# ipilter/RayTracerTest

Measured on AMD Instinct MI355X. Metric: Mray/s at 1920x1080x16spp, higher is better.
Workload: dtype f32

## Files before the change

### include/rt_mi355x.h

```cpp
#ifndef RT_MI355X_H
#define RT_MI355X_H

#include <stddef.h>
#include <stdint.h>

#ifdef __cplusplus
extern "C" {
#endif

#define RT_OK              0
#define RT_ERR_INVALID     1
#define RT_ERR_NO_DEVICE   2
#define RT_ERR_HIP         3
#define RT_ERR_STATE       4

#define RT_MATH_FMA        0u
#define RT_MATH_STRICT     1u

#define RT_FLAG_NO_FILTER  1u
#define RT_FLAG_NO_BINNING 2u

#define RT_FLAG_NEAREST_HIT 4u

#define RT_FLAG_NO_MACRO_BINS 16u
#define RT_FLAG_NO_SUPER_BINS 64u
#define RT_FLAG_NO_SURE_HIT 32u
#define RT_FLAG_SMOOTH_NORMALS 8u

#define RT_BUF_RENDER      0
#define RT_BUF_COUNTS      1
#define RT_BUF_IMAGE       2
#define RT_BUF_RNG         3
#define RT_BUF_FRAME       4
#define RT_GROUP_ID_BYTES  128

typedef struct rt_tracer rt_tracer;
typedef struct rt_float4 { float x, y, z, w; } rt_float4;

typedef void (*rt_callback_fn)(uint32_t* imageBuffer, size_t size, void* user);

typedef struct rt_options {
  uint32_t struct_size;
  int32_t  device;
  uint32_t full_height;
  uint32_t row_begin;
  uint32_t use_time_seed;
  uint32_t math_mode;
  uint64_t seed;
  uint32_t flags;
  uint32_t samples_in_flight;
  uint32_t lds_chunk;
  uint32_t bin_list;
  uint32_t transport;
} rt_options;

#define RT_TRANSPORT_RCCL  0u
#define RT_TRANSPORT_PEER  1u


int  rt_tracer_create(const uint32_t imageSize[2], const float cameraPosition[3],
                      const float cameraAngles[2], float fov, float focalLength, float aperture,
                      rt_tracer** out);
int  rt_tracer_create_ex(const uint32_t imageSize[2], const float cameraPosition[3],
                         const float cameraAngles[2], float fov, float focalLength, float aperture,
                         const rt_options* options, rt_tracer** out);
void rt_tracer_destroy(rt_tracer* t);
int  rt_tracer_trace(rt_tracer* t, uint32_t iterationCount, uint32_t samplesPerIteration,
                     uint32_t updateInterval);
void rt_tracer_stop(rt_tracer* t);
int  rt_tracer_resize(rt_tracer* t, const uint32_t size[2]);
void rt_tracer_set_camera_parameters(rt_tracer* t, float fov, float focalLength, float aperture);
void rt_tracer_rotate_camera(rt_tracer* t, const float angles[2]);
int  rt_tracer_upload_scene(rt_tracer* t, const rt_float4* hostData, size_t count);
int  rt_tracer_upload_scene_edges(rt_tracer* t, const rt_float4* hostData, size_t count);
float rt_pack_normal(const float n[3]);
void  rt_unpack_normal(float packed, float n[3]);
void rt_tracer_set_update_callback(rt_tracer* t, rt_callback_fn fn, void* user);
void rt_tracer_set_finished_callback(rt_tracer* t, rt_callback_fn fn, void* user);


int  rt_tracer_wait(rt_tracer* t);
int  rt_tracer_set_seed(rt_tracer* t, uint64_t seed);
int  rt_tracer_upload_spheres(rt_tracer* t, const rt_float4* spheres, size_t count);
int  rt_tracer_trace_enqueue(rt_tracer* t, uint32_t iterationCount, uint32_t samplesPerIteration);
int  rt_tracer_trace_enqueue_n(rt_tracer* t, uint32_t iterationCount, uint32_t samplesPerIteration, uint32_t n_steps);
int  rt_tracer_sync(rt_tracer* t);
int  rt_tracer_launch(rt_tracer* t, uint32_t samples, int clear_first, int emit_image);
int  rt_tracer_launch_iterations(rt_tracer* t, uint32_t samples, uint32_t iterations, int clear_first, int emit_image);
int  rt_tracer_fused_iterations(rt_tracer* t, uint32_t samples);
int  rt_tracer_set_list_reuse(rt_tracer* t, int across_traces);
int  rt_tracer_set_image_mirror(rt_tracer* t, void* device_visible_image);
int  rt_tracer_kernel_time(rt_tracer* t, double* total_ms, uint64_t* launches, int reset_after);
int  rt_tracer_launch_time(rt_tracer* t, double* total_ms, uint64_t* launches, int reset_after);
int  rt_tracer_trace_stats(rt_tracer* t, uint32_t samples, uint64_t out[16]);
int  rt_tracer_read_buffer(rt_tracer* t, int which, void* dst, size_t bytes);
int  rt_tracer_copy_buffer_to_device(rt_tracer* t, int which, void* dst_device, size_t bytes);
int  rt_tracer_copy_buffer_to_device_async(rt_tracer* t, int which, void* dst_device, size_t bytes);
void* rt_tracer_stream(rt_tracer* t);
void* rt_tracer_stream_b(rt_tracer* t);
void* rt_tracer_device_pointer(rt_tracer* t, int which);
size_t rt_tracer_buffer_bytes(rt_tracer* t, int which);
int  rt_tracer_info(rt_tracer* t, uint32_t out[8]);
const char* rt_tracer_last_error(rt_tracer* t);
const char* rt_last_error(void);
int  rt_device_count(void);
const char* rt_version(void);


int  rt_tracer_create_multi(const uint32_t imageSize[2], const float cameraPosition[3],
                            const float cameraAngles[2], float fov, float focalLength, float aperture,
                            const rt_options* options, const int32_t* devices, uint32_t n_bands,
                            rt_tracer** out);
int  rt_group_unique_id(uint8_t id[RT_GROUP_ID_BYTES]);
int  rt_tracer_join_group(rt_tracer* t, uint32_t n_ranks, uint32_t rank, const uint8_t id[RT_GROUP_ID_BYTES]);
int  rt_tracer_leave_group(rt_tracer* t);
int  rt_tracer_join_group_bands(rt_tracer* t, uint32_t n_ranks, uint32_t rank, const uint8_t id[RT_GROUP_ID_BYTES],
                                const uint32_t* row_begin);
int  rt_balance_rows(uint32_t n_bands, const uint32_t* row_begin, const double* cost, uint32_t granule,
                     uint32_t* new_row_begin);
int  rt_tracer_rebalance(rt_tracer* t);
int  rt_tracer_set_band(rt_tracer* t, uint32_t row_begin, uint32_t rows);
int  rt_tracer_gather_time(rt_tracer* t, double* total_ms, uint64_t* gathers, int reset_after);
int  rt_tracer_gather_only(rt_tracer* t);
int  rt_tracer_group_info(rt_tracer* t, char* json, size_t capacity);
int  rt_tracer_band_count(rt_tracer* t);
int  rt_tracer_band_info(rt_tracer* t, uint32_t band, uint32_t out[4]);

int rt_dbg_hit_triangle(int device, uint32_t math_mode, uint32_t n, const float* rays,
                        const float* tris, int eps_mode, int32_t* hit, float* tuv, float* normal,
                        float* point);
int rt_dbg_sincos(int device, uint32_t n, const float* x, float* s, float* c);
int rt_dbg_trace_occupancy(int device, int samples_in_flight, uint32_t lds_bytes);
int rt_dbg_valu_peak(int device, double* lane_fma_per_s, double* clock_ghz);
int rt_dbg_check_midrange(int device, uint64_t out[4]);
int rt_dbg_wave_list_counts(rt_tracer* t, int half, uint32_t* dst, size_t capacity_tiles, uint32_t* n_tiles, uint32_t* capacity_per_tile);
int rt_dbg_read_tile_lists(rt_tracer* t, uint32_t* dst, size_t capacity_words, uint32_t* words_per_tile);
int rt_dbg_focal_boxes(rt_tracer* t, float curv_scale, float* boxes, size_t boxes_capacity, float* focal, size_t focal_capacity);
int rt_dbg_classify(rt_tracer* t, uint32_t level, uint32_t forms, uint32_t slack_milli, const uint32_t* regions, uint32_t n_regions,
                    float* out, size_t capacity_floats);
int rt_dbg_uniform(int device, uint32_t n, uint32_t m, uint32_t* states, float* out);
int rt_dbg_get_ray(rt_tracer* t, uint32_t n, const uint32_t* pixels, uint32_t* states, float* rays);
void rt_dbg_rng_init_host(uint64_t seed, uint64_t subsequence, uint32_t state[6]);

#ifdef __cplusplus
}
#endif
#endif
```

### raytracertest_amd/api.py

```python
import ctypes as C
import os
import threading
import weakref

import numpy as np

_HERE = os.path.dirname(os.path.abspath(__file__))
_LIB_PATH = os.environ.get("RT_MI355X_LIB") or os.path.join(_HERE, "lib", "librt_mi355x.so")

MATH_FMA, MATH_STRICT = 0, 1
FLAG_NO_FILTER = 1
FLAG_NO_BINNING = 2
FLAG_NEAREST_HIT = 4
FLAG_SMOOTH_NORMALS = 8
FLAG_NO_MACRO_BINS = 16
FLAG_NO_SUPER_BINS = 64
FLAG_NO_SURE_HIT = 32
BUF_RENDER, BUF_COUNTS, BUF_IMAGE, BUF_RNG, BUF_FRAME = 0, 1, 2, 3, 4
GROUP_ID_BYTES = 128
TRANSPORT_RCCL, TRANSPORT_PEER = 0, 1

ABI_SYMBOLS = [
    "rt_tracer_create", "rt_tracer_create_ex", "rt_tracer_destroy", "rt_tracer_trace",
    "rt_tracer_stop", "rt_tracer_resize", "rt_tracer_set_camera_parameters",
    "rt_tracer_rotate_camera", "rt_tracer_upload_scene", "rt_tracer_set_update_callback",
    "rt_tracer_set_finished_callback", "rt_tracer_wait", "rt_tracer_set_seed",
    "rt_tracer_upload_spheres", "rt_tracer_trace_enqueue", "rt_tracer_trace_enqueue_n", "rt_tracer_sync", "rt_tracer_trace_stats", "rt_tracer_launch", "rt_tracer_launch_iterations", "rt_tracer_fused_iterations", "rt_tracer_set_image_mirror", "rt_tracer_set_list_reuse", "rt_tracer_stream_b", "rt_tracer_upload_scene_edges", "rt_pack_normal",
    "rt_unpack_normal",
    "rt_tracer_kernel_time", "rt_tracer_launch_time", "rt_tracer_read_buffer", "rt_tracer_copy_buffer_to_device", "rt_tracer_copy_buffer_to_device_async",
    "rt_tracer_stream",
    "rt_tracer_device_pointer", "rt_tracer_buffer_bytes", "rt_tracer_info",
    "rt_tracer_last_error", "rt_last_error", "rt_device_count", "rt_version",
    "rt_dbg_hit_triangle", "rt_dbg_sincos", "rt_dbg_valu_peak", "rt_dbg_check_midrange", "rt_dbg_trace_occupancy", "rt_dbg_uniform", "rt_dbg_get_ray",
    "rt_dbg_rng_init_host",
    "rt_tracer_create_multi", "rt_group_unique_id", "rt_tracer_join_group", "rt_tracer_leave_group",
    "rt_tracer_gather_time", "rt_tracer_band_count", "rt_tracer_band_info",
    "rt_tracer_join_group_bands", "rt_balance_rows", "rt_tracer_rebalance", "rt_tracer_set_band", "rt_dbg_read_tile_lists", "rt_dbg_wave_list_counts", "rt_dbg_focal_boxes", "rt_dbg_classify",
    "rt_tracer_gather_only", "rt_tracer_group_info",
]


class RtError(RuntimeError):
    pass


class Options(C.Structure):
    _fields_ = [("struct_size", C.c_uint32), ("device", C.c_int32), ("full_height", C.c_uint32),
                ("row_begin", C.c_uint32), ("use_time_seed", C.c_uint32), ("math_mode", C.c_uint32),
                ("seed", C.c_uint64), ("flags", C.c_uint32), ("samples_in_flight", C.c_uint32),
                ("lds_chunk", C.c_uint32), ("bin_list", C.c_uint32), ("transport", C.c_uint32)]


CALLBACK = C.CFUNCTYPE(None, C.POINTER(C.c_uint32), C.c_size_t, C.c_void_p)

_lib = None
_lib_lock = threading.Lock()


def library_path():
    return _LIB_PATH


def _share_hip_runtime_with_torch():
    if os.environ.get("RT_MI355X_HIP_RUNTIME", "") == "system":
        return None
    try:
        import importlib.util
        spec = importlib.util.find_spec("torch")
        if spec is None or not spec.submodule_search_locations:
            return None
        cand = os.path.join(list(spec.submodule_search_locations)[0], "lib", "libamdhip64.so")
        if os.path.exists(cand):
            C.CDLL(cand, mode=C.RTLD_GLOBAL)
            return cand
    except (ImportError, OSError, ValueError):
        pass
    return None


HIP_RUNTIME = None


def load_library():
    global _lib, HIP_RUNTIME
    with _lib_lock:
        if _lib is not None:
            return _lib
        if not os.path.exists(_LIB_PATH):
            raise RtError("HIP extension not built: %s is missing (run `python -m raytracertest_amd.build` "
                          "or __graft_entry__.build()); there is no CPU fallback" % _LIB_PATH)
        HIP_RUNTIME = _share_hip_runtime_with_torch()
        L = C.CDLL(_LIB_PATH)
        vp, u32p, f32p = C.c_void_p, C.POINTER(C.c_uint32), C.POINTER(C.c_float)
        L.rt_tracer_create.argtypes = [u32p, f32p, f32p, C.c_float, C.c_float, C.c_float, C.POINTER(vp)]
        L.rt_tracer_create_ex.argtypes = [u32p, f32p, f32p, C.c_float, C.c_float, C.c_float,
                                          C.POINTER(Options), C.POINTER(vp)]
        L.rt_tracer_destroy.argtypes = [vp]
        L.rt_tracer_destroy.restype = None
        L.rt_tracer_trace.argtypes = [vp, C.c_uint32, C.c_uint32, C.c_uint32]
        L.rt_tracer_stop.argtypes = [vp]
        L.rt_tracer_stop.restype = None
        L.rt_tracer_resize.argtypes = [vp, u32p]
        L.rt_tracer_set_camera_parameters.argtypes = [vp, C.c_float, C.c_float, C.c_float]
        L.rt_tracer_set_camera_parameters.restype = None
        L.rt_tracer_rotate_camera.argtypes = [vp, f32p]
        L.rt_tracer_rotate_camera.restype = None
        L.rt_tracer_upload_scene.argtypes = [vp, vp, C.c_size_t]
        L.rt_tracer_upload_scene_edges.argtypes = [vp, vp, C.c_size_t]
        L.rt_pack_normal.argtypes = [f32p]
        L.rt_pack_normal.restype = C.c_float
        L.rt_unpack_normal.argtypes = [C.c_float, f32p]
        L.rt_unpack_normal.restype = None
        L.rt_tracer_set_update_callback.argtypes = [vp, CALLBACK, vp]
        L.rt_tracer_set_update_callback.restype = None
        L.rt_tracer_set_finished_callback.argtypes = [vp, CALLBACK, vp]
        L.rt_tracer_set_finished_callback.restype = None
        L.rt_tracer_wait.argtypes = [vp]
        L.rt_tracer_set_seed.argtypes = [vp, C.c_uint64]
        L.rt_tracer_upload_spheres.argtypes = [vp, vp, C.c_size_t]
        L.rt_tracer_trace_enqueue.argtypes = [vp, C.c_uint32, C.c_uint32]
        L.rt_tracer_trace_enqueue_n.argtypes = [vp, C.c_uint32, C.c_uint32, C.c_uint32]
        L.rt_tracer_sync.argtypes = [vp]
        L.rt_tracer_launch.argtypes = [vp, C.c_uint32, C.c_int, C.c_int]
        L.rt_tracer_launch_iterations.argtypes = [vp, C.c_uint32, C.c_uint32, C.c_int, C.c_int]
        L.rt_tracer_fused_iterations.argtypes = [vp, C.c_uint32]
        L.rt_tracer_set_image_mirror.argtypes = [vp, vp]
        L.rt_tracer_set_list_reuse.argtypes = [vp, C.c_int]
        L.rt_tracer_trace_stats.argtypes = [vp, C.c_uint32, C.POINTER(C.c_uint64)]
        L.rt_tracer_kernel_time.argtypes = [vp, C.POINTER(C.c_double), C.POINTER(C.c_uint64), C.c_int]
        L.rt_tracer_launch_time.argtypes = [vp, C.POINTER(C.c_double), C.POINTER(C.c_uint64), C.c_int]
        L.rt_tracer_read_buffer.argtypes = [vp, C.c_int, vp, C.c_size_t]
        L.rt_tracer_copy_buffer_to_device.argtypes = [vp, C.c_int, vp, C.c_size_t]
        L.rt_tracer_copy_buffer_to_device_async.argtypes = [vp, C.c_int, vp, C.c_size_t]
        L.rt_tracer_stream.argtypes = [vp]
        L.rt_tracer_stream.restype = vp
        L.rt_tracer_stream_b.argtypes = [vp]
        L.rt_tracer_stream_b.restype = vp
        L.rt_tracer_device_pointer.argtypes = [vp, C.c_int]
        L.rt_tracer_device_pointer.restype = vp
        L.rt_tracer_buffer_bytes.argtypes = [vp, C.c_int]
        L.rt_tracer_buffer_bytes.restype = C.c_size_t
        L.rt_tracer_info.argtypes = [vp, u32p]
        L.rt_tracer_last_error.argtypes = [vp]
        L.rt_tracer_last_error.restype = C.c_char_p
        L.rt_last_error.restype = C.c_char_p
        L.rt_device_count.restype = C.c_int
        L.rt_version.restype = C.c_char_p
        L.rt_dbg_hit_triangle.argtypes = [C.c_int, C.c_uint32, C.c_uint32, f32p, f32p, C.c_int,
                                          C.POINTER(C.c_int32), f32p, f32p, f32p]
        L.rt_dbg_sincos.argtypes = [C.c_int, C.c_uint32, f32p, f32p, f32p]
        L.rt_dbg_uniform.argtypes = [C.c_int, C.c_uint32, C.c_uint32, u32p, f32p]
        L.rt_dbg_valu_peak.argtypes = [C.c_int, C.POINTER(C.c_double), C.POINTER(C.c_double)]
        L.rt_dbg_trace_occupancy.argtypes = [C.c_int, C.c_int, C.c_uint32]
        L.rt_dbg_get_ray.argtypes = [vp, C.c_uint32, u32p, u32p, f32p]
        L.rt_dbg_rng_init_host.argtypes = [C.c_uint64, C.c_uint64, u32p]
        L.rt_dbg_rng_init_host.restype = None
        L.rt_tracer_create_multi.argtypes = [u32p, f32p, f32p, C.c_float, C.c_float, C.c_float, C.POINTER(Options),
                                             C.POINTER(C.c_int32), C.c_uint32, C.POINTER(vp)]
        L.rt_group_unique_id.argtypes = [C.c_char_p]
        L.rt_tracer_join_group.argtypes = [vp, C.c_uint32, C.c_uint32, C.c_char_p]
        L.rt_tracer_leave_group.argtypes = [vp]
        L.rt_tracer_gather_time.argtypes = [vp, C.POINTER(C.c_double), C.POINTER(C.c_uint64), C.c_int]
        L.rt_tracer_band_count.argtypes = [vp]
        L.rt_tracer_band_info.argtypes = [vp, C.c_uint32, u32p]
        L.rt_tracer_join_group_bands.argtypes = [vp, C.c_uint32, C.c_uint32, C.c_char_p, u32p]
        L.rt_balance_rows.argtypes = [C.c_uint32, u32p, C.POINTER(C.c_double), C.c_uint32, u32p]
        L.rt_tracer_rebalance.argtypes = [vp]
        L.rt_tracer_set_band.argtypes = [vp, C.c_uint32, C.c_uint32]
        L.rt_dbg_read_tile_lists.argtypes = [vp, u32p, C.c_size_t, u32p]
        L.rt_dbg_wave_list_counts.argtypes = [vp, C.c_int, u32p, C.c_size_t, u32p, u32p]
        L.rt_dbg_focal_boxes.argtypes = [vp, C.c_float, f32p, C.c_size_t, f32p, C.c_size_t]
        L.rt_tracer_gather_only.argtypes = [vp]
        L.rt_tracer_group_info.argtypes = [vp, C.c_char_p, C.c_size_t]
        L.rt_dbg_classify.argtypes = [vp, C.c_uint32, C.c_uint32, C.c_uint32, u32p, C.c_uint32, f32p, C.c_size_t]
        _lib = L
        return _lib


def device_count():
    return int(load_library().rt_device_count())


def balance_rows(row_begin, cost, granule=8):
    b = np.ascontiguousarray(row_begin, np.uint32)
    c = np.ascontiguousarray(cost, np.float64)
    out = np.zeros_like(b)
    rc = load_library().rt_balance_rows(c.size, _u32p(b), c.ctypes.data_as(C.POINTER(C.c_double)), granule, _u32p(out))
    if rc != 0:
        raise RtError("rt_balance_rows: invalid partition")
    return [int(x) for x in out]


def group_unique_id():
    buf = C.create_string_buffer(GROUP_ID_BYTES)
    rc = load_library().rt_group_unique_id(buf)
    if rc != 0:
        raise RtError("rt_group_unique_id failed (%d): %s" % (rc, load_library().rt_last_error().decode()))
    return buf.raw


def _f32p(a):
    return a.ctypes.data_as(C.POINTER(C.c_float))


def _u32p(a):
    return a.ctypes.data_as(C.POINTER(C.c_uint32))


class RayTracer:

    def __init__(self, imageSize, cameraPosition=(0.0, 0.0, 0.0), cameraAngles=(0.0, 0.0), fov=70.0,
                 focalLength=10.0, aperture=4.0, *, seed=None, device=0, math_mode=MATH_FMA,
                 full_height=0, row_begin=0, no_filter=False, no_binning=False, nearest_hit=False, smooth_normals=False, no_macro_bins=False, no_super_bins=False, samples_in_flight=0,
                 lds_chunk=0, bin_list=0, devices=None, no_sure_hit=False, transport="rccl"):
        self._lib = load_library()
        self._h = C.c_void_p()
        self._cbs = {}
        self._retired = []
        size = np.array(imageSize, np.uint32)
        opt = Options()
        opt.struct_size = C.sizeof(Options)
        opt.device = device
        opt.full_height, opt.row_begin = full_height, row_begin
        opt.use_time_seed = 1 if seed is None else 0
        opt.seed = 0 if seed is None else int(seed)
        opt.math_mode = math_mode
        opt.flags = ((FLAG_NO_FILTER if no_filter else 0) | (FLAG_NO_BINNING if no_binning else 0) |
                     (FLAG_NEAREST_HIT if nearest_hit else 0) | (FLAG_SMOOTH_NORMALS if smooth_normals else 0) | (FLAG_NO_MACRO_BINS if no_macro_bins else 0) | (FLAG_NO_SUPER_BINS if no_super_bins else 0) |
                     (FLAG_NO_SURE_HIT if no_sure_hit else 0))
        opt.samples_in_flight, opt.lds_chunk, opt.bin_list = samples_in_flight, lds_chunk, bin_list
        opt.transport = {"rccl": TRANSPORT_RCCL, "peer": TRANSPORT_PEER}[transport]
        if devices is not None:
            devs = np.ascontiguousarray(devices, np.int32)
            rc = self._lib.rt_tracer_create_multi(_u32p(size), _f32p(np.array(cameraPosition, np.float32)),
                                                  _f32p(np.array(cameraAngles, np.float32)), fov, focalLength, aperture,
                                                  C.byref(opt), devs.ctypes.data_as(C.POINTER(C.c_int32)), devs.size,
                                                  C.byref(self._h))
        else:
            rc = self._lib.rt_tracer_create_ex(_u32p(size), _f32p(np.array(cameraPosition, np.float32)),
                                               _f32p(np.array(cameraAngles, np.float32)), fov, focalLength,
                                               aperture, C.byref(opt), C.byref(self._h))
        if rc != 0 or not self._h:
            raise RtError("rt_tracer_create failed (%d): %s" % (rc, self._lib.rt_last_error().decode()))
        self.full_height = int(full_height) if full_height else int(size[1])
        self._band = bool(full_height) and devices is None
        self.width = int(size[0])
        self.rows = int(size[1])

    def Trace(self, iterationCount, samplesPerIteration, updateInterval):
        self._check(self._lib.rt_tracer_trace(self._h, iterationCount, samplesPerIteration, updateInterval))

    def Stop(self):
        self._lib.rt_tracer_stop(self._h)

    def Resize(self, size):
        s = np.array(size, np.uint32)
        self._check(self._lib.rt_tracer_resize(self._h, _u32p(s)))
        self.width, self.rows = int(s[0]), int(s[1])
        if not self._band:
            self.full_height = self.rows

    def SetCameraParameters(self, fov, focalLength, aperture):
        self._lib.rt_tracer_set_camera_parameters(self._h, fov, focalLength, aperture)

    def RotateCamera(self, angles):
        self._lib.rt_tracer_rotate_camera(self._h, _f32p(np.array(angles, np.float32)))

    def UploadScene(self, hostData):
        a = np.ascontiguousarray(hostData, np.float32).reshape(-1, 4)
        rc = self._lib.rt_tracer_upload_scene(self._h, a.ctypes.data, a.shape[0])
        if rc == 1:
            return False
        self._check(rc)
        return True

    def UploadSceneEdges(self, hostData):
        a = np.ascontiguousarray(hostData, np.float32).reshape(-1, 4)
        rc = self._lib.rt_tracer_upload_scene_edges(self._h, a.ctypes.data, a.shape[0])
        if rc == 1:
            return False
        self._check(rc)
        return True

    def SetUpdateCallback(self, callback):
        self._set_cb("update", callback, self._lib.rt_tracer_set_update_callback)

    def SetFinishedCallback(self, callback):
        self._set_cb("finished", callback, self._lib.rt_tracer_set_finished_callback)

    def Wait(self):
        ok = bool(self._lib.rt_tracer_wait(self._h))
        self._retired.clear()
        return ok

    def SetSeed(self, seed):
        self._check(self._lib.rt_tracer_set_seed(self._h, int(seed)))

    def UploadSpheres(self, spheres):
        a = np.ascontiguousarray(spheres, np.float32).reshape(-1, 4)
        self._check(self._lib.rt_tracer_upload_spheres(self._h, a.ctypes.data, a.shape[0]))

    def TraceEnqueue(self, iterationCount, samplesPerIteration):
        self._check(self._lib.rt_tracer_trace_enqueue(self._h, iterationCount, samplesPerIteration))

    def TraceEnqueueN(self, iterationCount, samplesPerIteration, n_steps):
        self._check(self._lib.rt_tracer_trace_enqueue_n(self._h, iterationCount, samplesPerIteration, n_steps))

    def Launch(self, samples, clear_first=False, emit_image=False, iterations=1):
        if iterations == 1:
            self._check(self._lib.rt_tracer_launch(self._h, samples, int(clear_first), int(emit_image)))
        else:
            self._check(self._lib.rt_tracer_launch_iterations(self._h, samples, iterations, int(clear_first), int(emit_image)))

    def SetListReuse(self, across_traces=True):
        self._check(self._lib.rt_tracer_set_list_reuse(self._h, 1 if across_traces else 0))

    def SetImageMirror(self, device_visible_ptr):
        self._check(self._lib.rt_tracer_set_image_mirror(self._h, C.c_void_p(device_visible_ptr or 0)))

    def FusedIterations(self, samples):
        return max(1, int(self._lib.rt_tracer_fused_iterations(self._h, samples)))

    def Sync(self):
        self._check(self._lib.rt_tracer_sync(self._h))

    def TraceStats(self, samples):
        out = (C.c_uint64 * 16)()
        self._check(self._lib.rt_tracer_trace_stats(self._h, samples, out))
        v = [int(x) for x in out]
        return {"exit_det": v[0], "exit_u": v[1], "exit_v": v[2], "exit_hit": v[3],
                "skip_a": v[4], "skip_b": v[5], "skip_c": v[6], "reach_d": v[7],
                "bin_candidates": v[8], "bin_rounds": v[9], "pretest_skips": v[10],
                "tiles_by_list": {"0": v[11], "1": v[12], "sure": v[13], "2": v[14], "more": v[15]}}

    def KernelTime(self, reset=True):
        ms, n = C.c_double(), C.c_uint64()
        self._lib.rt_tracer_kernel_time(self._h, C.byref(ms), C.byref(n), 1 if reset else 0)
        return ms.value, n.value

    def LaunchTime(self, reset=True):
        ms, n = C.c_double(), C.c_uint64()
        self._lib.rt_tracer_launch_time(self._h, C.byref(ms), C.byref(n), 1 if reset else 0)
        return ms.value, n.value

    def _read(self, which, dtype, shape):
        out = np.empty(shape, dtype)
        self._check(self._lib.rt_tracer_read_buffer(self._h, which, out.ctypes.data, out.nbytes))
        return out

    def RenderBuffer(self):
        return self._read(BUF_RENDER, np.float32, (self.rows, self.width, 4))

    def SampleCounts(self):
        return self._read(BUF_COUNTS, np.uint32, (self.rows, self.width))

    def Image(self):
        return self._read(BUF_IMAGE, np.uint32, (self.rows, self.width))

    def RngStates(self):
        planes = self._read(BUF_RNG, np.uint32, (6, self.rows, self.width))
        return np.ascontiguousarray(np.moveaxis(planes, 0, -1))

    def JoinGroup(self, n_ranks, rank, unique_id=None, row_begin=None):
        if row_begin is None:
            self._check(self._lib.rt_tracer_join_group(self._h, n_ranks, rank, unique_id))
        else:
            b = np.ascontiguousarray(row_begin, np.uint32)
            self._check(self._lib.rt_tracer_join_group_bands(self._h, n_ranks, rank, unique_id, _u32p(b)))

    def SetBand(self, row_begin, rows):
        self._check(self._lib.rt_tracer_set_band(self._h, row_begin, rows))
        self.rows = int(rows)

    def Rebalance(self):
        self._check(self._lib.rt_tracer_rebalance(self._h))

    def LeaveGroup(self):
        self._check(self._lib.rt_tracer_leave_group(self._h))

    def Frame(self):
        return self._read(BUF_FRAME, np.uint32, (self.full_height, self.width))

    def GatherTime(self, reset=True):
        ms, n = C.c_double(), C.c_uint64()
        self._lib.rt_tracer_gather_time(self._h, C.byref(ms), C.byref(n), 1 if reset else 0)
        return ms.value, n.value

    def GatherOnly(self):
        self._check(self._lib.rt_tracer_gather_only(self._h))

    def GroupInfo(self):
        import json
        buf = C.create_string_buffer(8192)
        self._check(self._lib.rt_tracer_group_info(self._h, buf, len(buf)))
        return json.loads(buf.value.decode())

    def Bands(self):
        out = []
        for k in range(int(self._lib.rt_tracer_band_count(self._h))):
            v = np.zeros(4, np.uint32)
            self._check(self._lib.rt_tracer_band_info(self._h, k, _u32p(v)))
            out.append({"device": int(v[0]), "row0": int(v[1]), "rows": int(v[2]), "rank": int(v[3])})
        return out

    def DevicePointer(self, which):
        return self._lib.rt_tracer_device_pointer(self._h, which)

    def CopyToDevice(self, which, dst_ptr, nbytes):
        self._check(self._lib.rt_tracer_copy_buffer_to_device(self._h, which, dst_ptr, nbytes))

    def CopyToDeviceAsync(self, which, dst_ptr, nbytes):
        self._check(self._lib.rt_tracer_copy_buffer_to_device_async(self._h, which, dst_ptr, nbytes))

    def Stream(self):
        return int(self._lib.rt_tracer_stream(self._h) or 0)

    def StreamB(self):
        return int(self._lib.rt_tracer_stream_b(self._h) or 0)

    def Info(self):
        out = np.zeros(8, np.uint32)
        self._lib.rt_tracer_info(self._h, _u32p(out))
        keys = ("samples_in_flight", "lds_chunk", "lds_bytes", "grid_x", "grid_y", "n_tris", "n_spheres", "device")
        return dict(zip(keys, (int(v) for v in out)))

    def LastError(self):
        return self._lib.rt_tracer_last_error(self._h).decode()

    def DebugTileLists(self):
        bx, by = (self.width + 31) // 32, (self.rows + 7) // 8
        wpt = np.zeros(1, np.uint32)
        buf = np.zeros(bx * (by + 1) * 4 * 1025, np.uint32)
        self._check(self._lib.rt_dbg_read_tile_lists(self._h, _u32p(buf), buf.size, _u32p(wpt)))
        w = int(wpt[0])
        words = buf[:bx * by * 4 * w].reshape(by, bx * 4, w)[:, :, 0]
        return (words & 0x3FF).astype(np.int32), ((words >> 10) & 0x3FF).astype(np.int32), (words >> 31).astype(bool)

    def DebugWaveListCounts(self, half=0):
        n, cap = np.zeros(1, np.uint32), np.zeros(1, np.uint32)
        buf = np.zeros(((self.width + 31) // 32) * ((self.rows + 7) // 8 + 1) * 4, np.uint32)
        self._check(self._lib.rt_dbg_wave_list_counts(self._h, half, _u32p(buf), buf.size, _u32p(n), _u32p(cap)))
        return buf[:int(n[0])].copy(), int(cap[0])

    def DebugTileListWords(self):
        bx, by = (self.width + 31) // 32, (self.rows + 7) // 8
        wpt = np.zeros(1, np.uint32)
        buf = np.zeros(bx * (by + 1) * 4 * 1025, np.uint32)
        self._check(self._lib.rt_dbg_read_tile_lists(self._h, _u32p(buf), buf.size, _u32p(wpt)))
        w = int(wpt[0])
        return buf[:bx * by * 4 * w].reshape(by, bx * 4, w).copy()

    def DebugFocalBoxes(self, curv_scale=1.0):
        bx, by = (self.width + 31) // 32, (self.rows + 7) // 8
        boxes = np.zeros((by, bx * 4, 8), np.float32)
        focal = np.zeros((self.rows, self.width, 3), np.float32)
        self._check(self._lib.rt_dbg_focal_boxes(self._h, float(curv_scale), _f32p(boxes), boxes.size, _f32p(focal), focal.size))
        return boxes, focal

    def DebugClassify(self, regions, level=0, forms=False, slack_milli=1000):
        reg = np.ascontiguousarray(regions, np.uint32).reshape(-1, 2)
        n_tris = self.Info()["n_tris"]
        per = 16 + n_tris * (32 if forms else 12)
        out = np.zeros((reg.shape[0], per), np.float32)
        self._check(self._lib.rt_dbg_classify(self._h, level, 1 if forms else 0, slack_milli, _u32p(reg), reg.shape[0], _f32p(out), out.size))
        return out[:, :16], out[:, 16:].reshape(reg.shape[0], n_tris, 32 if forms else 12)

    def DebugGetRay(self, pixels, states):
        pix = np.ascontiguousarray(pixels, np.uint32).reshape(-1, 2)
        st = np.ascontiguousarray(states, np.uint32).reshape(-1, 6).copy()
        rays = np.zeros((pix.shape[0], 6), np.float32)
        self._check(self._lib.rt_dbg_get_ray(self._h, pix.shape[0], _u32p(pix), _u32p(st), _f32p(rays)))
        return rays, st

    def close(self):
        if self._h:
            self._lib.rt_tracer_destroy(self._h)
            self._h = C.c_void_p()
            self._retired.clear()

    def __del__(self):
        try:
            self.close()
        except Exception:
            pass

    def __enter__(self):
        return self

    def __exit__(self, *a):
        self.close()

    def _check(self, rc):
        if rc != 0:
            raise RtError("librt_mi355x error %d: %s" % (rc, self.LastError()))

    def _set_cb(self, key, callback, setter):
        old = self._cbs.get(key)
        if old is not None:
            self._retired.append(old)
        if callback is None:
            self._cbs[key] = CALLBACK()
            setter(self._h, self._cbs[key], None)
            return

        me = weakref.ref(self)

        def tramp(ptr, size, _user):
            n = size // 4
            img = np.ctypeslib.as_array(ptr, shape=(n,))
            owner = me()
            rows, width = (owner.rows, owner.width) if owner is not None else (0, 0)
            callback(img.reshape(rows, width) if n == rows * width and n else img, size)
        self._cbs[key] = CALLBACK(tramp)
        setter(self._h, self._cbs[key], None)


def dbg_hit_triangle(rays, tris, math_mode=MATH_FMA, eps_mode=0, device=0):
    L = load_library()
    r = np.ascontiguousarray(rays, np.float32).reshape(-1, 6)
    t = np.ascontiguousarray(tris, np.float32).reshape(-1, 9)
    n = r.shape[0]
    hit = np.zeros(n, np.int32)
    tuv, nrm, pt = (np.zeros((n, 3), np.float32) for _ in range(3))
    rc = L.rt_dbg_hit_triangle(device, math_mode, n, _f32p(r), _f32p(t), eps_mode,
                               hit.ctypes.data_as(C.POINTER(C.c_int32)), _f32p(tuv), _f32p(nrm), _f32p(pt))
    if rc != 0:
        raise RtError("rt_dbg_hit_triangle failed (%d): %s" % (rc, L.rt_last_error().decode()))
    return hit.astype(bool), tuv, nrm, pt


def dbg_sincos(x, device=0):
    L = load_library()
    a = np.ascontiguousarray(x, np.float32).ravel()
    s, c = np.zeros_like(a), np.zeros_like(a)
    rc = L.rt_dbg_sincos(device, a.size, _f32p(a), _f32p(s), _f32p(c))
    if rc != 0:
        raise RtError("rt_dbg_sincos failed (%d): %s" % (rc, L.rt_last_error().decode()))
    return s, c


def dbg_valu_peak(device=0):
    L = load_library()
    r, g = C.c_double(), C.c_double()
    rc = L.rt_dbg_valu_peak(device, C.byref(r), C.byref(g))
    if rc != 0:
        raise RtError("rt_dbg_valu_peak failed (%d): %s" % (rc, L.rt_last_error().decode()))
    return r.value, g.value


def dbg_check_midrange(device=0):
    L = load_library()
    out = (C.c_uint64 * 4)()
    L.rt_dbg_check_midrange.argtypes = [C.c_int, C.POINTER(C.c_uint64)]
    rc = L.rt_dbg_check_midrange(device, out)
    if rc != 0:
        raise RtError("rt_dbg_check_midrange failed (%d): %s" % (rc, L.rt_last_error().decode()))
    return tuple(int(x) for x in out)


def dbg_uniform(states, m, device=0):
    L = load_library()
    st = np.ascontiguousarray(states, np.uint32).reshape(-1, 6).copy()
    out = np.zeros((st.shape[0], m), np.float32)
    rc = L.rt_dbg_uniform(device, st.shape[0], m, _u32p(st), _f32p(out))
    if rc != 0:
        raise RtError("rt_dbg_uniform failed (%d): %s" % (rc, L.rt_last_error().decode()))
    return out, st


def dbg_rng_init_host(seed, subsequence):
    s = np.zeros(6, np.uint32)
    load_library().rt_dbg_rng_init_host(int(seed), int(subsequence), _u32p(s))
    return s
```

### raytracertest_amd/csrc/rt_kernels.hpp

```cpp
#pragma once
#include <hip/hip_runtime.h>
#include <stdint.h>

namespace rtk {

constexpr uint32_t kSuperChunk = 1024u, kSuperMaxChunks = 64u;

struct TraceParams {
  float4*   render;
  uint32_t* counts;
  uint32_t* rng;
  uint32_t  W, H;
  uint32_t  row0, rows;
  uint32_t  npix;
  uint32_t  samples;
  float     cam[12];
  float     half_height, aspect, focal, aperture;
  float     tile_curv, tile_round;
  const float4* tri_a;
  const float*  tri_b;
  const float4* tri_color;
  uint32_t  n_tris;
  const float4* spheres;
  uint32_t  n_spheres;
  uint32_t  chunk;
  uint32_t  bin_list;
  uint32_t  block_list;
  unsigned long long* stats;
  uint32_t* image;
  const float4* tri_n;
#ifdef RT_TIMELINE
  unsigned long long* timeline;
#endif
  uint32_t* image_host;
  uint32_t  pretest_on;
  uint32_t  iters;
  uint32_t* macro_lists;
  uint32_t  macro_cap, macro_w, macro_h, macro_nx;
  uint32_t* super_lists;
  uint32_t  super_chunks, super_f, super_nx;
  float*    macro_bounds;
  uint32_t* tile_lists;
  uint32_t  row_il, row_phase;
  uint32_t* half_cost;
  uint32_t  cost_split_brow;
  const float4* sure_table;
  uint32_t* wave_lists;
  uint32_t  wave_cap;
  uint32_t  flags;
};

constexpr uint32_t TRACE_ZERO_ACC = 1u;
constexpr uint32_t TRACE_EMIT_IMAGE = 2u;
constexpr uint32_t TRACE_NEAREST_HIT = 4u;
constexpr uint32_t TRACE_PRETEST = 32u;
constexpr uint32_t TRACE_NO_SURE_HIT = 64u;

hipError_t launch_rng_init(uint32_t* rng, uint32_t npix, uint32_t p0, const uint32_t seeded[6],
                           const uint32_t* jump, const uint32_t* win, hipStream_t st);
hipError_t launch_prep_triangles(bool fma, bool edges, const float4* verts, uint32_t n, float4* tri_a, float* tri_b,
                                 float4* color, float4* normals, hipStream_t st);
uint32_t trace_lds_bytes(const TraceParams& p, bool bin);
hipError_t launch_trace(const TraceParams& p, bool fma, bool filter, bool bin, int K, hipStream_t st);
int trace_occupancy(int K, size_t lds);
hipError_t launch_convert(const float4* render, const uint32_t* counts, uint32_t* image, uint32_t npix,
                          hipStream_t st);

hipError_t launch_dbg_hit_triangle(bool fma, uint32_t n, const float* rays, const float* tris, int eps_mode,
                                   int* hit, float* tuv, float* normal, float* point, hipStream_t st);
bool trace_can_fuse(bool filter, bool bin);
hipError_t launch_macro_bin(const TraceParams& p, bool fma, hipStream_t st);
hipError_t launch_super_bin(const TraceParams& p, bool fma, hipStream_t st);
hipError_t launch_wave_lists(const TraceParams& p, bool fma, hipStream_t st);
hipError_t launch_delay(uint32_t us, hipStream_t st);
hipError_t launch_publish_half_cost(uint32_t* half_cost, unsigned long long* host_word, hipStream_t st);
hipError_t launch_sure_table(const float4* colors, uint32_t n_tris, uint32_t samples, float4* out, hipStream_t st);
hipError_t launch_tile_lists(const TraceParams& p, bool fma, hipStream_t st);
hipError_t launch_dbg_check_midrange(unsigned long long* out, hipStream_t st);
hipError_t launch_dbg_focal_boxes(bool fma, const TraceParams& p, float* boxes, float* focal, hipStream_t st);
hipError_t launch_dbg_classify(bool fma, bool forms, uint32_t slack_milli, const TraceParams& p, uint32_t level, uint32_t n_regions,
                               const uint32_t* regions, float* out, hipStream_t st);
hipError_t launch_dbg_valu_peak(uint32_t blocks, int iters, float* out, unsigned long long* clk, hipStream_t st);
hipError_t launch_dbg_sincos(uint32_t n, const float* x, float* s, float* c, hipStream_t st);
hipError_t launch_dbg_uniform(uint32_t n, uint32_t m, uint32_t* states, float* out, hipStream_t st);
hipError_t launch_dbg_get_ray(bool fma, const TraceParams& p, uint32_t n, const uint32_t* pixels,
                              uint32_t* states, float* rays, hipStream_t st);

}
```

### raytracertest_amd/csrc/rt_lists.hpp

```cpp
#pragma once
#include "rt_classify.hpp"

namespace rtk {

template <bool FMA, int WAVES>
__device__ __forceinline__ FocalBounds rect_focal_bounds(const TraceParams& p, uint32_t x0, uint32_t y0, uint32_t rw, uint32_t rh, float (*s_box)[8]) {
  const uint32_t lane = threadIdx.x & 63u, wave = threadIdx.x >> 6;
  const uint32_t x1 = (x0 + rw < p.W) ? x0 + rw : p.W;
  const uint32_t y1 = (y0 + rh < p.rows) ? y0 + rh : p.rows;
  const uint32_t w = x1 - x0, count_px = w * (y1 - y0);
  float lo[3] = {FLT_MAX, FLT_MAX, FLT_MAX}, hi[3] = {-FLT_MAX, -FLT_MAX, -FLT_MAX};
  bool finite = true;
  for (uint32_t i = threadIdx.x; i < count_px; i += 64u * WAVES) {
    const uint32_t px = x0 + i % w, ly = y0 + i / w;
    V3 po, pd;
    pinhole<FMA>(p, px, p.row0 + ly, po, pd);
    const V3 f = focal_point<FMA>(p, pd);
    const float fl[3] = {f.x, f.y, f.z};
#pragma unroll
    for (int c = 0; c < 3; ++c) {
      finite = finite && (__builtin_fabsf(fl[c]) <= FLT_MAX);
      lo[c] = fminf(lo[c], fl[c]);
      hi[c] = fmaxf(hi[c], fl[c]);
    }
  }
#pragma unroll
  for (int c = 0; c < 3; ++c) { lo[c] = uniform(wave_min(lo[c])); hi[c] = uniform(wave_max(hi[c])); }
  const bool wave_ok = __builtin_amdgcn_ballot_w64(!finite) == 0ull;
  if (lane == 0u) {
#pragma unroll
    for (int c = 0; c < 3; ++c) { s_box[wave][c] = lo[c]; s_box[wave][3 + c] = hi[c]; }
    s_box[wave][6] = wave_ok ? 1.0f : 0.0f;
  }
  __syncthreads();
  FocalBounds bb;
  bb.ok = true; bb.any = count_px != 0u;
#pragma unroll
  for (int c = 0; c < 3; ++c) { bb.lo[c] = FLT_MAX; bb.hi[c] = -FLT_MAX; }
  for (uint32_t v = 0; v < static_cast<uint32_t>(WAVES); ++v) {
#pragma unroll
    for (int c = 0; c < 3; ++c) {
      bb.lo[c] = fminf(bb.lo[c], s_box[v][c]);
      bb.hi[c] = fmaxf(bb.hi[c], s_box[v][3 + c]);
    }
    bb.ok = bb.ok && (s_box[v][6] != 0.0f);
  }
  return bb;
}

template <class Src>
__device__ __forceinline__ void bin_pass(const TraceParams& p, const TileFamily& fam, Src tri_of, uint32_t n, uint32_t* out, uint32_t cap,
                                         uint32_t (*s_cnt)[4]) {
  const uint32_t lane = threadIdx.x & 63u, wave = threadIdx.x >> 6;
  uint32_t total = 0, step = 0;
  bool overflow = false;
  for (uint32_t base = 0; base < n; base += 256u, ++step) {
    const uint32_t e = base + threadIdx.x;
    const bool valid = e < n;
    const uint32_t tri = tri_of(valid ? e : (n - 1u));
    const float4 A0 = p.tri_a[2u * tri], A1 = p.tri_a[2u * tri + 1u];
    const float bz = p.tri_b[tri];
    bool keep = valid;
    if (fam.usable)
      keep = valid && !tile_misses_triangle(fam, {A1.z, A1.w, bz}, {A0.w, A1.x, A1.y}, {A0.x, A0.y, A0.z});
    const unsigned long long m = __builtin_amdgcn_ballot_w64(keep);
    uint32_t* const slot = s_cnt[step & 1u];
    if (lane == 0u) slot[wave] = static_cast<uint32_t>(__builtin_popcountll(m));
    __syncthreads();
    const uint32_t c0 = slot[0], c1 = slot[1], c2 = slot[2], c3 = slot[3];
    const uint32_t before = (wave > 0u ? c0 : 0u) + (wave > 1u ? c1 : 0u) + (wave > 2u ? c2 : 0u);
    const uint32_t step_total = c0 + c1 + c2 + c3;
    if (total + step_total > cap) { overflow = true; break; }
    const uint32_t pos = total + before + __builtin_amdgcn_mbcnt_hi(static_cast<uint32_t>(m >> 32),
                                                                __builtin_amdgcn_mbcnt_lo(static_cast<uint32_t>(m), 0u));
    if (keep) out[1u + pos] = tri;
    total += step_total;
  }
  if (threadIdx.x == 0u) out[0] = overflow ? 0xFFFFFFFFu : total;
}


__device__ __forceinline__ FocalBounds load_bounds(const float* b) {
  FocalBounds r;
#pragma unroll
  for (int c = 0; c < 3; ++c) { r.lo[c] = uniform(b[c]); r.hi[c] = uniform(b[3 + c]); }
  r.ok = uniform(b[6]) != 0.0f; r.any = uniform(b[7]) != 0.0f;
  return r;
}

template <bool FMA>
__global__ __launch_bounds__(256) void macro_bounds_kernel(TraceParams p) {
  __shared__ float s_box[4][8];
  const FocalBounds bb = rect_focal_bounds<FMA, 4>(p, blockIdx.x * p.macro_w, blockIdx.y * p.macro_h, p.macro_w, p.macro_h, s_box);
  if (threadIdx.x == 0u) {
    float* const o = p.macro_bounds + (static_cast<size_t>(blockIdx.y) * gridDim.x + blockIdx.x) * 8u;
#pragma unroll
    for (int c = 0; c < 3; ++c) { o[c] = bb.lo[c]; o[3 + c] = bb.hi[c]; }
    o[6] = bb.ok ? 1.0f : 0.0f; o[7] = bb.any ? 1.0f : 0.0f;
  }
}

template <bool FMA>
__global__ __launch_bounds__(256) void super_bin_kernel(TraceParams p) {
  __shared__ uint32_t s_cnt[2][4];
  const uint32_t sx = blockIdx.x % p.super_nx, sy = blockIdx.x / p.super_nx;
  const uint32_t macro_ny = (p.rows + p.macro_h - 1u) / p.macro_h;
  FocalBounds bb;
  bb.ok = true; bb.any = false;
#pragma unroll
  for (int c = 0; c < 3; ++c) { bb.lo[c] = FLT_MAX; bb.hi[c] = -FLT_MAX; }
  for (uint32_t j = 0; j < p.super_f; ++j) {
    for (uint32_t i = 0; i < p.super_f; ++i) {
      const uint32_t mx = sx * p.super_f + i, my = sy * p.super_f + j;
      if (mx >= p.macro_nx || my >= macro_ny) continue;
      const FocalBounds mb = load_bounds(p.macro_bounds + (static_cast<size_t>(my) * p.macro_nx + mx) * 8u);
#pragma unroll
      for (int c = 0; c < 3; ++c) { bb.lo[c] = fminf(bb.lo[c], mb.lo[c]); bb.hi[c] = fmaxf(bb.hi[c], mb.hi[c]); }
      bb.ok = bb.ok && mb.ok; bb.any = bb.any || mb.any;
    }
  }
  const TileFamily fam = make_family(p, bb);
  const uint32_t first = blockIdx.y * kSuperChunk;
  const uint32_t n = p.n_tris - first < kSuperChunk ? p.n_tris - first : kSuperChunk;
  uint32_t* const out = p.super_lists + (static_cast<size_t>(blockIdx.x) * gridDim.y + blockIdx.y) * (kSuperChunk + 1u);
  bin_pass(p, fam, [&](uint32_t e) { return first + e; }, n, out, kSuperChunk, s_cnt);
}

template <bool FMA>
__global__ __launch_bounds__(256) void macro_bin_kernel(TraceParams p) {
  __shared__ float s_box[4][8];
  __shared__ uint32_t s_cnt[2][4];
  __shared__ uint32_t s_first[kSuperMaxChunks + 1u];
  FocalBounds bb;
  if (p.macro_bounds != nullptr) bb = load_bounds(p.macro_bounds + (static_cast<size_t>(blockIdx.y) * gridDim.x + blockIdx.x) * 8u);
  else bb = rect_focal_bounds<FMA, 4>(p, blockIdx.x * p.macro_w, blockIdx.y * p.macro_h, p.macro_w, p.macro_h, s_box);
  const TileFamily fam = make_family(p, bb);
  uint32_t* const out = p.macro_lists + (static_cast<size_t>(blockIdx.y) * gridDim.x + blockIdx.x) * (p.macro_cap + 1u);
  if (p.super_lists == nullptr) {
    bin_pass(p, fam, [](uint32_t e) { return e; }, p.n_tris, out, p.macro_cap, s_cnt);
    return;
  }
  const uint32_t S = p.super_chunks;
  const uint32_t* const sl = p.super_lists + static_cast<size_t>((blockIdx.y / p.super_f) * p.super_nx + blockIdx.x / p.super_f) * S * (kSuperChunk + 1u);
  if (threadIdx.x == 0u) {
    uint32_t acc = 0;
    for (uint32_t c = 0; c < S; ++c) { s_first[c] = acc; acc += sl[static_cast<size_t>(c) * (kSuperChunk + 1u)]; }
    s_first[S] = acc;
  }
  __syncthreads();
  const uint32_t n = s_first[S];
  bin_pass(p, fam, [&](uint32_t e) {
    uint32_t c = 0;
    for (uint32_t k = 1; k < S; ++k) c += (e >= s_first[k]) ? 1u : 0u;
    return sl[static_cast<size_t>(c) * (kSuperChunk + 1u) + 1u + (e - s_first[c])];
  }, n, out, p.macro_cap, s_cnt);
}

template <int CTRL>
__device__ __forceinline__ float dpp_f(float v) {
  return __builtin_bit_cast(float, __builtin_amdgcn_update_dpp(0, __builtin_bit_cast(int, v), CTRL, 0xF, 0xF, true));
}
#define RT_ROW_REDUCE(OP, v)                 \
  v = OP(v, dpp_f<0xB1>(v));                 \
  v = OP(v, dpp_f<0x4E>(v));                 \
  v = OP(v, dpp_f<0x124>(v));                \
  v = OP(v, dpp_f<0x128>(v));
template <int G>
__device__ __forceinline__ float group_max(float v) {
  RT_ROW_REDUCE(fmaxf, v)
#pragma unroll
  for (int off = G / 2; off >= 16; off >>= 1) v = fmaxf(v, __shfl_xor(v, off, 64));
  return v;
}
template <int G>
__device__ __forceinline__ float group_min(float v) {
  RT_ROW_REDUCE(fminf, v)
#pragma unroll
  for (int off = G / 2; off >= 16; off >>= 1) v = fminf(v, __shfl_xor(v, off, 64));
  return v;
}
#undef RT_ROW_REDUCE

template <bool FMA, int G, class SL>
__device__ __forceinline__ FocalBounds group_focal_bounds(const TraceParams& p, uint32_t x0, uint32_t y0, bool in_image, uint32_t gl, uint32_t gbase) {
  constexpr uint32_t T = 64u / G;
  const bool full = in_image && x0 + 8u <= p.W && y0 + 8u <= p.rows;
  FocalBounds b;
  const bool corners = p.tile_curv > 0.0f && full;
  const unsigned long long need_range = __builtin_amdgcn_ballot_w64(in_image && !corners);
  {
    const uint32_t cx = x0 + ((gl & 1u) ? 7u : 0u), cy = y0 + ((gl & 2u) ? 7u : 0u);
    V3 po, pd;
    pinhole<FMA>(p, cx < p.W ? cx : 0u, p.row0 + (cy < p.rows ? cy : 0u), po, pd);
    const V3 f = focal_point<FMA>(p, pd);
    const float fl[3] = {f.x, f.y, f.z};
    const float dev = p.tile_curv + RT_SLK(4e-6f) * p.tile_round;
    bool finite = true;
#pragma unroll
    for (int i = 0; i < 3; ++i) {
      const float c0 = __shfl(fl[i], static_cast<int>(gbase), 64), c1 = __shfl(fl[i], static_cast<int>(gbase + 1u), 64);
      const float c2 = __shfl(fl[i], static_cast<int>(gbase + 2u), 64), c3 = __shfl(fl[i], static_cast<int>(gbase + 3u), 64);
      b.lo[i] = fminf(fminf(c0, c1), fminf(c2, c3)) - dev;
      b.hi[i] = fmaxf(fmaxf(c0, c1), fmaxf(c2, c3)) + dev;
      finite = finite && (__builtin_fabsf(b.lo[i]) <= FLT_MAX) && (__builtin_fabsf(b.hi[i]) <= FLT_MAX);
    }
    b.ok = finite; b.any = true;
  }
  if (need_range != 0ull) {
    float lo[3] = {FLT_MAX, FLT_MAX, FLT_MAX}, hi[3] = {-FLT_MAX, -FLT_MAX, -FLT_MAX};
    bool finite = true, any = false;
#pragma unroll
    for (uint32_t i = 0; i < T; ++i) {
      const uint32_t pi = gl + i * G;
      const uint32_t px = x0 + (pi & 7u), py = y0 + (pi >> 3);
      const bool inside = in_image && px < p.W && py < p.rows;
      V3 po, pd;
      pinhole<FMA>(p, inside ? px : 0u, p.row0 + (inside ? py : 0u), po, pd);
      const V3 f = focal_point<FMA>(p, pd);
      const float fl[3] = {f.x, f.y, f.z};
#pragma unroll
      for (int c = 0; c < 3; ++c) {
        if (inside) { lo[c] = fminf(lo[c], fl[c]); hi[c] = fmaxf(hi[c], fl[c]); finite = finite && (__builtin_fabsf(fl[c]) <= FLT_MAX); }
      }
      any = any || inside;
    }
    const unsigned long long gmask = G == 64 ? ~0ull : (0xFFFFFFFFull << gbase);
    const bool g_ok = (__builtin_amdgcn_ballot_w64(!finite) & gmask) == 0ull;
    const bool g_any = (__builtin_amdgcn_ballot_w64(any) & gmask) != 0ull;
#pragma unroll
    for (int c = 0; c < 3; ++c) { lo[c] = group_min<G>(lo[c]); hi[c] = group_max<G>(hi[c]); }
    if (!corners) {
#pragma unroll
      for (int c = 0; c < 3; ++c) { b.lo[c] = lo[c]; b.hi[c] = hi[c]; }
      b.ok = g_ok; b.any = g_any;
    }
  }
  return b;
}

template <bool FMA, int G, class SL = SlackProduct>
__global__ __launch_bounds__(256, 5) void tile_lists_kernel(const TraceParams p) {
  static_assert(G == 32 || G == 64, "lanes per tile");
  constexpr uint32_t T = 64u / G;
  const uint32_t lane = threadIdx.x & 63u, wave = threadIdx.x >> 6;
  const uint32_t gl = lane & (G - 1u), gbase = lane & ~(G - 1u);
  const uint32_t gx = (p.W + 31u) / 32u, gy = (p.rows + 7u) / 8u;
  const uint32_t slots = gx * gy * 4u;
  const uint32_t slot = (blockIdx.x * 4u + wave) * T + lane / G;
  const bool live = slot < slots;
  const uint32_t sl = live ? slot : 0u;
  const uint32_t x0 = ((sl / 4u) % gx) * 32u + (sl % 4u) * 8u, y0 = ((sl / 4u) / gx) * 8u;
  const bool in_image = live && x0 < p.W;

  const FocalBounds b = group_focal_bounds<FMA, G, SL>(p, x0, y0, in_image, gl, gbase);
  const TileFamily fam = make_family<SL>(p, b);

  uint32_t* const saved = p.tile_lists + static_cast<size_t>(sl) * (1u + p.bin_list);
  const uint32_t n = p.n_tris;
  uint32_t count = 0;
  const float NEG = -__builtin_inff();
  bool haveA = false;
  float Q = NEG, M1 = NEG, M2 = NEG;
  uint32_t A = 0, I1 = 0xFFFFFFFFu;
  for (uint32_t base = 0; base < n; base += G) {
    const uint32_t tri = base + gl;
    const bool valid = in_image && tri < n;
    const uint32_t ti = tri < n ? tri : n - 1u;
    const float4 A0 = p.tri_a[2u * ti], A1 = p.tri_a[2u * ti + 1u];
    const float bz = p.tri_b[ti];
    bool keep = valid, sure = false;
    float q[2] = {0.0f, 0.0f};
    if (fam.usable) {
      const bool miss = tile_misses_triangle<false, true, SL>(fam, {A1.z, A1.w, bz}, {A0.w, A1.x, A1.y}, {A0.x, A0.y, A0.z}, nullptr, &sure, q);
      keep = valid && !miss;
    } else {
      sure = false;
    }
    const unsigned long long m = __builtin_amdgcn_ballot_w64(keep);
    const unsigned long long gm = G == 64 ? m : ((m >> gbase) & 0xFFFFFFFFull);
    const uint32_t pos = count + static_cast<uint32_t>(__builtin_popcountll(gm & ((1ull << gl) - 1ull)));
    if (keep) saved[1u + pos] = tri;
    count += static_cast<uint32_t>(__builtin_popcountll(gm));
    const bool cand = keep && sure && fam.usable;
    const float Qs = group_max<G>(cand ? q[0] : NEG);
    const unsigned long long bm = __builtin_amdgcn_ballot_w64(cand && q[0] == Qs);
    const unsigned long long gbm = G == 64 ? bm : ((bm >> gbase) & 0xFFFFFFFFull);
    if (gbm != 0ull && (!haveA || Qs > Q)) { haveA = true; Q = Qs; A = base + static_cast<uint32_t>(__builtin_ctzll(gbm)); }
    const float qh = keep ? ((q[1] == q[1]) ? q[1] : __builtin_inff()) : NEG;
    if (n <= G) {
      const uint32_t la = gbm != 0ull ? static_cast<uint32_t>(__builtin_ctzll(gbm)) : 0xFFFFFFFFu;
      M1 = group_max<G>((keep && gl != la) ? qh : NEG);
      I1 = 0xFFFFFFFEu;
      break;
    }
    const float m1s = group_max<G>(qh);
    const unsigned long long tm = __builtin_amdgcn_ballot_w64(keep && qh == m1s);
    const unsigned long long gtm = G == 64 ? tm : ((tm >> gbase) & 0xFFFFFFFFull);
    const uint32_t l1 = gtm != 0ull ? static_cast<uint32_t>(__builtin_ctzll(gtm)) : 0xFFFFFFFFu;
    const float m2s = group_max<G>((keep && gl != l1) ? qh : NEG);
    if (gtm != 0ull) {
      if (m1s > M1) { M2 = fmaxf(M1, m2s); M1 = m1s; I1 = base + l1; }
      else { M2 = fmaxf(M2, m1s); }
    }
  }
  bool sure_one = false;
  if (haveA) {
    const float R = (I1 == A) ? M2 : M1;
    sure_one = count <= 1u || (R < Q - 1e-4f * (__builtin_fabsf(R) + __builtin_fabsf(Q)));
  }
  if (live && gl == 0u) saved[0] = count | (A << 10) | (sure_one ? 0x80000000u : 0u);
}

template <class SL>
__device__ __forceinline__ float tile_dev(const TraceParams& p) { return p.tile_curv + RT_SLK(4e-6f) * p.tile_round; }

__device__ __forceinline__ void region_corner_pixel(const TraceParams& p, uint32_t rx, uint32_t ry, uint32_t tile, uint32_t corner,
                                                    uint32_t& px, uint32_t& py, bool& valid) {
  const uint32_t x0 = rx * 32u + (tile & 3u) * 8u, y0 = (ry * 2u + (tile >> 2)) * 8u;
  valid = x0 < p.W && y0 < p.rows;
  const uint32_t x1 = (x0 + 7u < p.W) ? x0 + 7u : p.W - 1u, y1 = (y0 + 7u < p.rows) ? y0 + 7u : p.rows - 1u;
  px = valid ? ((corner & 1u) ? x1 : x0) : 0u;
  py = valid ? ((corner & 2u) ? y1 : y0) : 0u;
}

template <bool FMA, class SL, bool PACK = false>
__device__ __forceinline__ void region_focal_bounds(const TraceParams& p, uint32_t rx, uint32_t ry, uint32_t lane,
                                                    FocalBounds& tile_b, FocalBounds& region_b) {
  const uint32_t l32 = lane & 31u;
  uint32_t px, py;
  bool valid;
  region_corner_pixel(p, rx, ry, l32 >> 2, l32 & 3u, px, py, valid);
  V3 po, pd;
  pinhole<FMA>(p, px, p.row0 + py, po, pd);
  const V3 f = focal_point<FMA>(p, pd);
  const float fl[3] = {f.x, f.y, f.z};
  const float dev = tile_dev<SL>(p);
  bool fin = true;
  float rlo[3], rhi[3];
#pragma unroll
  for (int i = 0; i < 3; ++i) {
    float lo = fl[i], hi = fl[i];
    lo = fminf(lo, dpp_f<0xB1>(lo)); lo = fminf(lo, dpp_f<0x4E>(lo));
    hi = fmaxf(hi, dpp_f<0xB1>(hi)); hi = fmaxf(hi, dpp_f<0x4E>(hi));
    tile_b.lo[i] = lo - dev;
    tile_b.hi[i] = hi + dev;
    fin = fin && (__builtin_fabsf(tile_b.lo[i]) <= FLT_MAX) && (__builtin_fabsf(tile_b.hi[i]) <= FLT_MAX) && (fl[i] == fl[i]);
    rlo[i] = valid ? tile_b.lo[i] : FLT_MAX;
    rhi[i] = valid ? tile_b.hi[i] : -FLT_MAX;
  }
  const unsigned long long badm = __builtin_amdgcn_ballot_w64(!fin);
  const uint32_t quad_bad = (static_cast<uint32_t>(badm >> (lane & (PACK ? 60u : 28u))) & 0xFu);
  tile_b.ok = quad_bad == 0u;
  tile_b.any = valid;
  const unsigned long long vm = __builtin_amdgcn_ballot_w64(valid);
  const uint32_t hs = PACK ? (lane & 32u) : 0u;
  region_b.any = ((vm >> hs) & 0xFFFFFFFFull) != 0ull;
  region_b.ok = (((badm & vm) >> hs) & 0xFFFFFFFFull) == 0ull;
#pragma unroll
  for (int i = 0; i < 3; ++i) {
    region_b.lo[i] = group_min<32>(rlo[i]);
    region_b.hi[i] = group_max<32>(rhi[i]);
  }
}


template <int G>
__device__ __forceinline__ float max_group(float v) {
  v = fmaxf(v, dpp_f<0xB1>(v));
  v = fmaxf(v, dpp_f<0x4E>(v));
  if constexpr (G == 8) v = fmaxf(v, dpp_f<0x141>(v));
  return v;
}

template <class SL, int G2>
__device__ __forceinline__ void region_level2(const TraceParams& p, uint32_t lane, const FocalBounds& mine, const uint32_t* cand, uint32_t cnt,
                                              uint32_t cnt_max, uint32_t tslot, bool slot_live, bool lower) {
  constexpr uint32_t GM = (1u << G2) - 1u;
  const uint32_t j = lane & (G2 - 1u), gsh = lane & ~static_cast<uint32_t>(G2 - 1);
  const bool tile_valid = mine.any;
  const TileFamily fam = make_family<SL>(p, mine);
  uint32_t* const saved = p.tile_lists + static_cast<size_t>(tile_valid ? tslot : 0u) * (1u + p.bin_list);
  const float NEG = -__builtin_inff();
  uint32_t count = 0;
  bool haveA = false;
  float Q = NEG, M1 = NEG, M2 = NEG;
  uint32_t A = 0, I1 = 0xFFFFFFFFu;
  const bool one_pass = cnt_max <= static_cast<uint32_t>(G2);
  bool others_ok = true;
  for (uint32_t c0 = 0; c0 < cnt_max; c0 += G2) {
    const bool has = tile_valid && c0 + j < cnt;
    const uint32_t tri = (c0 + j < cnt) ? cand[c0 + j] : 0u;
    const float4 A0 = p.tri_a[2u * tri], A1 = p.tri_a[2u * tri + 1u];
    const float bz = p.tri_b[tri];
    bool keep = has, sure = false;
    float q[2] = {0.0f, 0.0f};
    float pr[9] = {0.0f, 0.0f, 0.0f, 0.0f, 0.0f, 0.0f, 0.0f, 0.0f, 0.0f};
    if (fam.usable) {
      const bool miss = tile_misses_triangle<false, true, SL>(fam, {A1.z, A1.w, bz}, {A0.w, A1.x, A1.y}, {A0.x, A0.y, A0.z}, nullptr, &sure, q,
                                                              nullptr, pr);
      keep = has && !miss;
    }
    const uint32_t gm = static_cast<uint32_t>(__builtin_amdgcn_ballot_w64(keep) >> gsh) & GM;
    const uint32_t pos = count + static_cast<uint32_t>(__builtin_popcount(gm & ((1u << j) - 1u)));
    if (keep) saved[1u + pos] = tri;
    count += static_cast<uint32_t>(__builtin_popcount(gm));
    const bool cd = keep && sure && fam.usable;
    const float Qs = max_group<G2>(cd ? q[0] : NEG);
    const uint32_t gbm = static_cast<uint32_t>(__builtin_amdgcn_ballot_w64(cd && q[0] == Qs) >> gsh) & GM;
    if (gbm != 0u && (!haveA || Qs > Q)) { haveA = true; Q = Qs; A = cand[c0 + static_cast<uint32_t>(__builtin_ctz(gbm))]; }
    const float qh = keep ? ((q[1] == q[1]) ? q[1] : __builtin_inff()) : NEG;
    if (one_pass) {
      const uint32_t la = gbm != 0u ? static_cast<uint32_t>(__builtin_ctz(gbm)) : 0xFFFFFFFFu;
      bool lane_ok = !keep || j == la || (gbm != 0u && qh < Qs - 1e-4f * (__builtin_fabsf(qh) + __builtin_fabsf(Qs)));
      const bool need = gbm != 0u && !lane_ok;
      if (__builtin_amdgcn_ballot_w64(need) != 0ull) {
        float pa[9];
        const int src = static_cast<int>(gsh + (la & (G2 - 1u)));
#pragma unroll
        for (int i = 0; i < 9; ++i) pa[i] = __shfl(pr[i], src, 64);
        lane_ok = lane_ok || (need && pair_farther<SL>(fam, pa, pr));
      }
      others_ok = (static_cast<uint32_t>(__builtin_amdgcn_ballot_w64(!lane_ok) >> gsh) & GM) == 0u;
    }
    const float m1s = max_group<G2>(qh);
    const uint32_t gtm = static_cast<uint32_t>(__builtin_amdgcn_ballot_w64(keep && qh == m1s) >> gsh) & GM;
    const uint32_t l1 = gtm != 0u ? static_cast<uint32_t>(__builtin_ctz(gtm)) : 0xFFFFFFFFu;
    const float m2s = max_group<G2>((keep && j != l1) ? qh : NEG);
    if (gtm != 0u) {
      const uint32_t i1s = cand[c0 + l1];
      if (m1s > M1) { M2 = fmaxf(M1, m2s); M1 = m1s; I1 = i1s; }
      else { M2 = fmaxf(M2, m1s); }
    }
  }
  bool sure_one = false;
  if (haveA) {
    const float R = (I1 == A) ? M2 : M1;
    sure_one = count <= 1u || (R < Q - 1e-4f * (__builtin_fabsf(R) + __builtin_fabsf(Q)));
    if (one_pass) sure_one = sure_one || others_ok;
  }
  if (j == 0u) {
    if (tile_valid) saved[0] = count | (A << 10) | (sure_one ? 0x80000000u : 0u);
    else if (slot_live) p.tile_lists[static_cast<size_t>(tslot) * (1u + p.bin_list)] = 0u;
  }
  if (p.half_cost != nullptr) {
    const bool rays = j == 0u && tile_valid && !sure_one;
    const uint32_t nu = static_cast<uint32_t>(__builtin_popcountll(__builtin_amdgcn_ballot_w64(rays && !lower)));
    const uint32_t nl = static_cast<uint32_t>(__builtin_popcountll(__builtin_amdgcn_ballot_w64(rays && lower)));
    if (lane == 0u) {
      if (nu != 0u) atomicAdd(p.half_cost, nu);
      if (nl != 0u) atomicAdd(p.half_cost + 1, nl);
    }
  }
}

template <bool FMA, class SL = SlackProduct>
__global__ __launch_bounds__(256, RT_LISTS_WAVES) void region_lists_kernel(const TraceParams p) {
  __shared__ uint32_t s_cand[4][256];
  const uint32_t lane = threadIdx.x & 63u, wave = threadIdx.x >> 6;
  const uint32_t gx = (p.W + 31u) / 32u, gy = (p.rows + 7u) / 8u, gry = (gy + 1u) / 2u;
  const uint32_t region = blockIdx.x * 4u + wave;
  if (region >= gx * gry) return;
  const uint32_t rx = region % gx, ry = region / gx;
  FocalBounds tb, rb;
  region_focal_bounds<FMA, SL>(p, rx, ry, lane, tb, rb);
  const uint32_t n = p.n_tris;
  uint32_t* const cand = s_cand[wave];

  uint32_t cnt = 0;
  {
    const TileFamily rf = make_family<SL>(p, rb);
    for (uint32_t base = 0; base < n; base += 64u) {
      const uint32_t tri = base + lane;
      const bool valid = tri < n;
      const uint32_t ti = valid ? tri : n - 1u;
      const float4 A0 = p.tri_a[2u * ti], A1 = p.tri_a[2u * ti + 1u];
      const float bz = p.tri_b[ti];
      bool keep = valid;
      if (rf.usable) keep = valid && !tile_misses_triangle<false, false, SL>(rf, {A1.z, A1.w, bz}, {A0.w, A1.x, A1.y}, {A0.x, A0.y, A0.z});
      const unsigned long long m = __builtin_amdgcn_ballot_w64(keep);
      const uint32_t pos = cnt + __builtin_amdgcn_mbcnt_hi(static_cast<uint32_t>(m >> 32), __builtin_amdgcn_mbcnt_lo(static_cast<uint32_t>(m), 0u));
      if (keep) cand[pos] = tri;
      cnt += static_cast<uint32_t>(__builtin_popcountll(m));
    }
    __builtin_amdgcn_fence(__ATOMIC_RELEASE, "wavefront");
    __builtin_amdgcn_wave_barrier();
  }

  const uint32_t t8 = lane >> 3;
  FocalBounds mine;
#pragma unroll
  for (int i = 0; i < 3; ++i) {
    mine.lo[i] = __shfl(tb.lo[i], static_cast<int>(4u * t8), 64);
    mine.hi[i] = __shfl(tb.hi[i], static_cast<int>(4u * t8), 64);
  }
  const unsigned long long okm = __builtin_amdgcn_ballot_w64(tb.ok), anym = __builtin_amdgcn_ballot_w64(tb.any);
  mine.ok = ((okm >> (4u * t8)) & 1ull) != 0ull;
  mine.any = ((anym >> (4u * t8)) & 1ull) != 0ull;
  const uint32_t brow = ry * 2u + (t8 >> 2);
  region_level2<SL, 8>(p, lane, mine, cand, cnt, cnt, (brow * gx + rx) * 4u + (t8 & 3u), brow < gy, brow >= p.cost_split_brow);
}

template <bool FMA, class SL = SlackProduct>
__global__ __launch_bounds__(256, 4) void region_pair_lists_kernel(const TraceParams p) {
  __shared__ uint32_t s_cand[4][2][32];
  const uint32_t lane = threadIdx.x & 63u, wave = threadIdx.x >> 6, half = lane >> 5;
  const uint32_t gx = (p.W + 31u) / 32u, gy = (p.rows + 7u) / 8u, gry = (gy + 1u) / 2u, regions = gx * gry;
  const uint32_t first = (blockIdx.x * 4u + wave) * 2u;
  if (first >= regions) return;
  const bool live = first + half < regions;
  const uint32_t region = live ? first + half : first;
  const uint32_t rx = region % gx, ry = region / gx;
  FocalBounds tb, rb;
  region_focal_bounds<FMA, SL, true>(p, rx, ry, lane, tb, rb);
  const uint32_t n = p.n_tris;
  uint32_t* const cand = s_cand[wave][half];

  uint32_t cnt;
  {
    const TileFamily rf = make_family<SL>(p, rb);
    const uint32_t tri = lane & 31u;
    const bool valid = tri < n;
    const uint32_t ti = valid ? tri : n - 1u;
    const float4 A0 = p.tri_a[2u * ti], A1 = p.tri_a[2u * ti + 1u];
    const float bz = p.tri_b[ti];
    bool keep = valid;
    if (rf.usable) keep = valid && !tile_misses_triangle<false, false, SL>(rf, {A1.z, A1.w, bz}, {A0.w, A1.x, A1.y}, {A0.x, A0.y, A0.z});
    const uint32_t hm = static_cast<uint32_t>(__builtin_amdgcn_ballot_w64(keep) >> (lane & 32u));
    if (keep) cand[__builtin_popcount(hm & ((1u << tri) - 1u))] = tri;
    cnt = static_cast<uint32_t>(__builtin_popcount(hm));
    __builtin_amdgcn_fence(__ATOMIC_RELEASE, "wavefront");
    __builtin_amdgcn_wave_barrier();
  }
  const uint32_t cnt_a = static_cast<uint32_t>(__builtin_amdgcn_readlane(static_cast<int>(cnt), 0));
  const uint32_t cnt_b = static_cast<uint32_t>(__builtin_amdgcn_readlane(static_cast<int>(cnt), 32));
  const unsigned long long okm = __builtin_amdgcn_ballot_w64(tb.ok), anym = __builtin_amdgcn_ballot_w64(tb.any && live);

  if (cnt_a <= 4u && cnt_b <= 4u) {
    const uint32_t t8 = (lane >> 2) & 7u;
    FocalBounds mine = tb;
    mine.ok = ((okm >> (lane & 60u)) & 1ull) != 0ull;
    mine.any = ((anym >> (lane & 60u)) & 1ull) != 0ull;
    const uint32_t brow = ry * 2u + (t8 >> 2);
    region_level2<SL, 4>(p, lane, mine, cand, cnt, cnt_a > cnt_b ? cnt_a : cnt_b, (brow * gx + rx) * 4u + (t8 & 3u), live && brow < gy,
                         brow >= p.cost_split_brow);
  } else {
#pragma nounroll
    for (uint32_t h = 0; h < 2u; ++h) {
      if (first + h >= regions) break;
      const uint32_t t8 = lane >> 3, src = h * 32u + 4u * t8;
      FocalBounds mine;
#pragma unroll
      for (int i = 0; i < 3; ++i) {
        mine.lo[i] = __shfl(tb.lo[i], static_cast<int>(src), 64);
        mine.hi[i] = __shfl(tb.hi[i], static_cast<int>(src), 64);
      }
      mine.ok = ((okm >> src) & 1ull) != 0ull;
      mine.any = ((anym >> src) & 1ull) != 0ull;
      const uint32_t hrx = (first + h) % gx, hry = (first + h) / gx, brow = hry * 2u + (t8 >> 2);
      const uint32_t hc = h == 0u ? cnt_a : cnt_b;
      region_level2<SL, 8>(p, lane, mine, s_cand[wave][h], hc, hc, (brow * gx + hrx) * 4u + (t8 & 3u), brow < gy, brow >= p.cost_split_brow);
    }
  }
}


}
```

### raytracertest_amd/csrc/rt_trace.hpp

```cpp
#pragma once
#include "rt_lists.hpp"

namespace rtk {

#ifndef RT_TRACE_MIN_WAVES
#define RT_TRACE_MIN_WAVES 4
#endif
#ifndef RT_TRACE_WAVES
#define RT_TRACE_WAVES(K) RT_TRACE_MIN_WAVES
#endif
#ifndef RT_HBM_WAVES
#define RT_HBM_WAVES 4
#endif
#ifndef RT_SMALL_WG_WAVES
#define RT_SMALL_WG_WAVES 4
#endif

template <bool FMA, int K, bool FILTER, bool STATS, class GetB>
__device__ __forceinline__ void test_triangle(const float4 A0, const float4 A1, GetB get_v0z, int tri_index,
                                              const V3 (&o)[K], const V3 (&d)[K], float (&best_t)[K],
                                              int (&best_i)[K], bool nearest, bool counted_lane, uint32_t valid_k,
                                              unsigned long long (&st_exit)[4],
                                              unsigned long long (&st_skip)[4]) {
  using M = Math<FMA>;
  const V3 e2 = {A0.x, A0.y, A0.z}, e1 = {A0.w, A1.x, A1.y};

  if constexpr (!FILTER) {
    const V3 v0 = {A1.z, A1.w, get_v0z()};
#pragma unroll
    for (int k = 0; k < K; ++k) {
      float t = 0.0f, u = 0.0f, v = 0.0f;
      int stage;
      const bool h = hit_triangle_exact<FMA>(o[k], d[k], v0, e1, e2, RT_EPS, t, u, v, stage);
      if (h && (nearest ? (t > 0.0f && t < best_t[k]) : best_t[k] < t)) {
        best_t[k] = t;
        best_i[k] = tri_index;
      }
      if constexpr (STATS) {
        const bool counted = counted_lane && (static_cast<uint32_t>(k) < valid_k);
#pragma unroll
        for (int e = 0; e < 4; ++e)
          st_exit[e] += __builtin_popcountll(__builtin_amdgcn_ballot_w64(counted && stage == e));
      }
    }
  } else {
    V3 pv[K];
    float det[K];
    unsigned long long mk[K];
    unsigned long long live = 0ull;
#pragma unroll
    for (int k = 0; k < K; ++k) {
      pv[k] = M::cross(d[k], e2);
      det[k] = M::dot(e1, pv[k]);
      mk[k] = __builtin_amdgcn_ballot_w64(!(det[k] < RT_EPS));
      live |= mk[k];
    }
    if (live == 0ull) { if constexpr (STATS) st_skip[0]++; return; }

    const V3 v0 = {A1.z, A1.w, get_v0z()};
    V3 tv[K];
    float U[K], thi[K], tlo[K];
    live = 0ull;
#pragma unroll
    for (int k = 0; k < K; ++k) {
      tv[k] = rtd::sub(o[k], v0);
      U[k] = M::dot(tv[k], pv[k]);
      thi[k] = det[k] * 1.0001f;
      tlo[k] = det[k] * -1e-6f;
      mk[k] &= __builtin_amdgcn_ballot_w64(!(U[k] > thi[k])) & __builtin_amdgcn_ballot_w64(!(U[k] < tlo[k]));
      live |= mk[k];
    }
    if (live == 0ull) { if constexpr (STATS) st_skip[1]++; return; }

    V3 qv[K];
    float V[K];
    live = 0ull;
#pragma unroll
    for (int k = 0; k < K; ++k) {
      qv[k] = M::cross(tv[k], e1);
      V[k] = M::dot(d[k], qv[k]);
      mk[k] &= __builtin_amdgcn_ballot_w64(!(V[k] < tlo[k])) &
               __builtin_amdgcn_ballot_w64(!((U[k] + V[k]) > thi[k]));
      live |= mk[k];
    }
    if (live == 0ull) { if constexpr (STATS) st_skip[2]++; return; }
    if constexpr (STATS) st_skip[3]++;

#pragma unroll
    for (int k = 0; k < K; ++k) {
      if (mk[k] != 0ull) {
        const float inv = 1.0f / det[k];
        const float u = U[k] * inv;
        const float v = V[k] * inv;
        const float t = M::dot(e2, qv[k]) * inv;
        const bool miss = (det[k] < RT_EPS) | (u < 0.0f) | (u > 1.0f) | (v < 0.0f) | (u + v > 1.0f);
        const bool closer = nearest ? ((t > 0.0f) & (t < best_t[k])) : (best_t[k] < t);
        const bool upd = (!miss) & closer;
        best_t[k] = upd ? t : best_t[k];
        best_i[k] = upd ? tri_index : best_i[k];
      }
    }
  }
}


constexpr uint32_t kWaveRec = 16u;
constexpr uint32_t kWaveOverflow = 0xFFFFFFFFu;
template <bool FMA, int K, bool FILTER, bool STATS, bool BIN, bool ONEPASS, bool FUSE = false, bool PRE = false, bool HBM = false>
__global__ __launch_bounds__((BIN && ONEPASS) ? 64 * RT_SMALL_WG_WAVES : 256, (ONEPASS && K == 2) ? 5 : HBM ? RT_HBM_WAVES : RT_TRACE_WAVES(K)) void trace_kernel(const TraceParams p) {
  static_assert(!HBM || (PRE && BIN && !ONEPASS && FILTER && !STATS), "lists from HBM: the default dense-scene kernels only");
  using M = Math<FMA>;
  extern __shared__ float4 s_mem[];
  constexpr uint32_t WGW = (BIN && ONEPASS) ? RT_SMALL_WG_WAVES : 4u, WGS = 4u / WGW;

  const uint32_t lane = threadIdx.x & 63u, wl = threadIdx.x >> 6;
  const uint32_t wave = (blockIdx.x % WGS) * WGW + wl;
  const uint32_t bx = blockIdx.x / WGS;
  uint32_t by = blockIdx.y;
  const uint32_t gxb = gridDim.x / WGS;
  if constexpr (BIN && ONEPASS) {
    if (p.row_il != 0u) by = (blockIdx.y / p.row_il) * (2u * p.row_il) + p.row_phase * p.row_il + blockIdx.y % p.row_il;
  }
  const uint32_t px = bx * 32u + wave * 8u + (lane & 7u);
  const uint32_t ly = by * 8u + (lane >> 3);
  const bool inside = px < p.W && ly < p.rows;
  const uint32_t cxp = inside ? px : 0u, cyp = inside ? ly : 0u;
  const size_t pix = static_cast<size_t>(cxp) + static_cast<size_t>(cyp) * p.W;

#ifdef RT_TIMELINE
  const size_t tl_slot = ((static_cast<size_t>(by) * gxb + bx) * 4u + wave) * 16u;
  auto tl_mark = [&](uint32_t i) {
    __builtin_amdgcn_sched_barrier(0);
    if (p.timeline != nullptr && lane == 0u) p.timeline[tl_slot + i] = __builtin_amdgcn_s_memrealtime();
    __builtin_amdgcn_sched_barrier(0);
  };
  if (p.timeline != nullptr && lane == 0u) {
    uint32_t hw, xcc;
    asm volatile("s_getreg_b32 %0, hwreg(HW_REG_HW_ID)" : "=s"(hw));
    asm volatile("s_getreg_b32 %0, hwreg(HW_REG_XCC_ID)" : "=s"(xcc));
    p.timeline[tl_slot + 6] = hw;
    p.timeline[tl_slot + 7] = (static_cast<unsigned long long>(xcc) << 32) | (__builtin_amdgcn_s_memrealtime() & 0xffffffffull);
  }
  tl_mark(0);
#else
  auto tl_mark = [](uint32_t) {};
#endif
  Rng rng;
  auto load_rng = [&] {
    rng.d = p.rng[0 * static_cast<size_t>(p.npix) + pix];
    rng.v0 = p.rng[1 * static_cast<size_t>(p.npix) + pix];
    rng.v1 = p.rng[2 * static_cast<size_t>(p.npix) + pix];
    rng.v2 = p.rng[3 * static_cast<size_t>(p.npix) + pix];
    rng.v3 = p.rng[4 * static_cast<size_t>(p.npix) + pix];
    rng.v4 = p.rng[5 * static_cast<size_t>(p.npix) + pix];
  };
  constexpr bool RNG_LATE = PRE && BIN && !ONEPASS;
  constexpr bool THIRD_BLOCK = RT_TRACE_THIRD_BLOCK, THIRD_WAVE = RT_TRACE_THIRD_WAVE;
  if constexpr (!RNG_LATE) load_rng();


  const bool sure_ok = BIN && ONEPASS && (p.flags & (TRACE_NEAREST_HIT | TRACE_NO_SURE_HIT)) == 0u && p.n_spheres == 0u && p.tri_n == nullptr;
  bool loaded_sure = false;
  uint32_t list_word = 0u;
  if constexpr (BIN && ONEPASS) {
    if (p.tile_lists != nullptr) {
      const size_t slot0 = (static_cast<size_t>(by) * gxb + bx) * 4u + wave;
      list_word = static_cast<uint32_t>(__builtin_amdgcn_readfirstlane(static_cast<int>(p.tile_lists[slot0 * (1u + p.bin_list)])));
      loaded_sure = sure_ok && (list_word >> 31) != 0u;
    }
  }
  V3 po = {0.0f, 0.0f, 0.0f}, pd = {0.0f, 0.0f, 0.0f}, focal = {0.0f, 0.0f, 0.0f};
  if (!loaded_sure) {
    pinhole<FMA>(p, cxp, p.row0 + cyp, po, pd);
    focal = focal_point<FMA>(p, pd);
  }

  const uint32_t n = p.n_tris;
  const bool nearest = (p.flags & TRACE_NEAREST_HIT) != 0u;
  float ax = 0.0f, ay = 0.0f, az = 0.0f;
  unsigned long long st_exit[4] = {0, 0, 0, 0};
  unsigned long long st_skip[4] = {0, 0, 0, 0};
  unsigned long long st_bin[2] = {0, 0};
  unsigned long long st_pre = 0;

  const uint32_t cap = n < p.chunk ? n : p.chunk;
  float4* const sA = s_mem;
  float* const sB = reinterpret_cast<float*>(s_mem + 2u * cap);
  const bool single_chunk = n <= p.chunk;
  if constexpr (!BIN) {
    if (single_chunk) {
      for (uint32_t i = threadIdx.x; i < 2u * n; i += 256u) sA[i] = p.tri_a[i];
      for (uint32_t i = threadIdx.x; i < n; i += 256u) sB[i] = p.tri_b[i];
      __syncthreads();
    }
  }

  const uint32_t L = p.bin_list;
  float4* const cA = s_mem + static_cast<size_t>(wl) * (2u * L);
  float* const cB = reinterpret_cast<float*>(s_mem + WGW * 2u * L) + wl * L;
  int* const cI = reinterpret_cast<int*>(s_mem + WGW * 2u * L) + WGW * L + wl * L;
  constexpr bool PRETEST = PRE && BIN && !ONEPASS;
  const bool pretest = PRETEST && (p.flags & TRACE_PRETEST) != 0u;
  float4* const cP = s_mem + 4u * 2u * L + 2u * L + static_cast<size_t>(wave) * (4u * L);
  const uint32_t list_floats4 = pretest ? (4u * 2u * L + 2u * L + 16u * L) : (4u * 2u * L + 2u * L);
  float* const cC = reinterpret_cast<float*>(s_mem + list_floats4) + wave * (3u * L);

  TileFamily fam;
  bool list_complete = false;
  uint32_t list_count = 0;
  bool sure_hit_tile = false;
  uint32_t sure_winner = 0;
  const uint32_t Lb = p.block_list;
  uint32_t* const bI = reinterpret_cast<uint32_t*>(s_mem + list_floats4);
  uint32_t* const bcnt = bI + Lb;
  float* const bbox = reinterpret_cast<float*>(bcnt + 8);
  uint32_t src_count = n;
  bool src_is_block_list = false;
  const uint32_t* mI = nullptr;
  if constexpr (BIN && !ONEPASS) {
    if (p.macro_lists != nullptr) {
      const uint32_t mt = (blockIdx.y * 8u / p.macro_h) * p.macro_nx + (blockIdx.x * 32u / p.macro_w);
      const uint32_t* const ml = p.macro_lists + static_cast<size_t>(mt) * (p.macro_cap + 1u);
      const uint32_t mc = static_cast<uint32_t>(__builtin_amdgcn_readfirstlane(static_cast<int>(ml[0])));
      if (mc != 0xFFFFFFFFu) { mI = ml + 1; src_count = mc; }
    }
  }
  const uint32_t n_src = src_count;
  if constexpr (BIN && ONEPASS) fam.usable = false;
  bool hbm_overflow = false;
  if constexpr (HBM) {
    const size_t slot = (static_cast<size_t>(by) * gxb + bx) * 4u + wave;
    const float4* const rec = reinterpret_cast<const float4*>(p.wave_lists) + slot * (1u + p.wave_cap) * (kWaveRec / 4u);
    const float4 hdr = rec[0];
    const uint32_t count = static_cast<uint32_t>(__builtin_amdgcn_readfirstlane(__builtin_bit_cast(int, hdr.x)));
    hbm_overflow = count == kWaveOverflow;
    fam.usable = true;
    fam.fc[0] = uniform(hdr.y); fam.fc[1] = uniform(hdr.z); fam.fc[2] = uniform(hdr.w);
    list_count = hbm_overflow ? 0u : count;
    for (uint32_t e = lane; e < list_count; e += 64u) {
      const float4* const r = rec + (1u + e) * (kWaveRec / 4u);
      const float4 f0 = r[0], f1 = r[1], f2 = r[2], f3 = r[3];
      const uint32_t tri = __builtin_bit_cast(uint32_t, f3.z);
      const float4 a0 = p.tri_a[2u * tri], a1 = p.tri_a[2u * tri + 1u], c0 = p.tri_color[tri];
      const float bz = p.tri_b[tri];
      cP[4u * e] = f0; cP[4u * e + 1u] = f1; cP[4u * e + 2u] = f2; cP[4u * e + 3u] = make_float4(f3.x, f3.y, 0.0f, 0.0f);
      cA[2u * e] = a0; cA[2u * e + 1u] = a1;
      cB[e] = bz;
      cI[e] = static_cast<int>(tri);
      cC[3u * e] = c0.x; cC[3u * e + 1u] = c0.y; cC[3u * e + 2u] = c0.z;
    }
    __builtin_amdgcn_fence(__ATOMIC_RELEASE, "wavefront");
    __builtin_amdgcn_wave_barrier();
    list_complete = true;
  }
  if constexpr (BIN && !ONEPASS && !HBM) {
    tl_mark(8);
    const FocalBounds wb = focal_bounds(p, focal, inside);
    tl_mark(9);
    fam = make_family(p, wb);
    tl_mark(10);
    {
      if (Lb != 0u) {
        const FocalBounds bb = block_focal_union(wb, bbox, wave, lane);
        const TileFamily bfam = make_family(p, bb);
        uint32_t total = 0;
        bool overflow = false;
        uint32_t step = 0;
        for (uint32_t base = 0; base < n_src; base += 256u, ++step) {
          const uint32_t e = base + threadIdx.x;
          const bool valid = e < n_src;
          const uint32_t ei = valid ? e : (n_src - 1u);
          const uint32_t tri = mI != nullptr ? mI[ei] : ei;
          const uint32_t ti = tri;
          const float4 A0 = p.tri_a[2u * ti], A1 = p.tri_a[2u * ti + 1u];
          const float bz = p.tri_b[ti];
          bool keep = valid;
          if (bfam.usable)
            keep = valid && !tile_misses_triangle<false, false, SlackProduct, THIRD_BLOCK>(bfam, {A1.z, A1.w, bz}, {A0.w, A1.x, A1.y}, {A0.x, A0.y, A0.z});
          const unsigned long long m = __builtin_amdgcn_ballot_w64(keep);
          uint32_t* const slot = bcnt + (step & 1u) * 4u;
          if (lane == 0u) slot[wave] = static_cast<uint32_t>(__builtin_popcountll(m));
          __syncthreads();
          const uint32_t c0 = slot[0], c1 = slot[1], c2 = slot[2], c3 = slot[3];
          const uint32_t before = (wave > 0u ? c0 : 0u) + (wave > 1u ? c1 : 0u) + (wave > 2u ? c2 : 0u);
          const uint32_t step_total = c0 + c1 + c2 + c3;
          if (total + step_total > Lb) { overflow = true; break; }
          const uint32_t pos = total + before + __builtin_amdgcn_mbcnt_hi(static_cast<uint32_t>(m >> 32),
                                                                      __builtin_amdgcn_mbcnt_lo(static_cast<uint32_t>(m), 0u));
          if (keep) bI[pos] = tri;
          total += step_total;
        }
        __syncthreads();
        if (!overflow) { src_count = total; src_is_block_list = true; }
      }
    }
  }

  auto classify = [&](uint32_t from, auto with_forms) -> uint32_t {
    constexpr bool WF = decltype(with_forms)::value;
    uint32_t count = 0, base = from;
    while (base < src_count && count < L) {
      const uint32_t e = base + lane;
      const bool valid = e < src_count;
      const uint32_t ei = valid ? e : (src_count - 1u);
      const uint32_t tri = src_is_block_list ? bI[ei] : (mI != nullptr ? mI[ei] : ei);
      const uint32_t ti = tri;
      float4 A0, A1;
      float bz;
      A0 = p.tri_a[2u * ti]; A1 = p.tri_a[2u * ti + 1u];
      bz = p.tri_b[ti];
      bool keep = valid;
      float forms[18] = {0.0f, 0.0f, 0.0f, 0.0f, 0.0f, 0.0f, 0.0f, 0.0f, 0.0f,
                         0.0f, 0.0f, 0.0f, 0.0f, 0.0f, 0.0f, 0.0f, 0.0f, 0.0f};
      if (fam.usable) {
        if constexpr (PRETEST && WF) {
          if (pretest) {
            const bool miss3 = tile_misses_triangle<false, false, SlackProduct, true>(fam, {A1.z, A1.w, bz}, {A0.w, A1.x, A1.y}, {A0.x, A0.y, A0.z});
            asm volatile("" : "+v"(A0.x), "+v"(A0.y), "+v"(A0.z), "+v"(A0.w), "+v"(A1.x), "+v"(A1.y), "+v"(A1.z), "+v"(A1.w), "+v"(bz));
            keep = valid && !miss3 && !tile_misses_triangle<true>(fam, {A1.z, A1.w, bz}, {A0.w, A1.x, A1.y}, {A0.x, A0.y, A0.z}, forms);
          }
          else keep = valid && !tile_misses_triangle<false, false, SlackProduct, THIRD_WAVE>(fam, {A1.z, A1.w, bz}, {A0.w, A1.x, A1.y}, {A0.x, A0.y, A0.z});
        } else {
          keep = valid && !tile_misses_triangle<false, false, SlackProduct, THIRD_WAVE>(fam, {A1.z, A1.w, bz}, {A0.w, A1.x, A1.y}, {A0.x, A0.y, A0.z});
        }
      }
      const unsigned long long m = __builtin_amdgcn_ballot_w64(keep);
      if (count + static_cast<uint32_t>(__builtin_popcountll(m)) > L) break;
      const uint32_t pos = count + __builtin_amdgcn_mbcnt_hi(static_cast<uint32_t>(m >> 32),
                                                             __builtin_amdgcn_mbcnt_lo(static_cast<uint32_t>(m), 0u));
      if (keep) {
        cA[2u * pos] = A0;
        cA[2u * pos + 1u] = A1;
        cB[pos] = bz;
        cI[pos] = static_cast<int>(tri);
        if constexpr (PRETEST && WF) {
          if (pretest) {
            auto pk = [&](float hi, float lo) {
              const uint32_t h = __builtin_bit_cast(uint16_t, static_cast<_Float16>(hi)), l = __builtin_bit_cast(uint16_t, static_cast<_Float16>(lo));
              return __builtin_bit_cast(float, (h << 16) | l);
            };
            cP[4u * pos] = make_float4(forms[0], forms[1], forms[2], forms[3]);
            cP[4u * pos + 1u] = make_float4(forms[4], forms[5], forms[6], forms[7]);
            cP[4u * pos + 2u] = make_float4(forms[8], pk(forms[9], forms[10]), pk(forms[11], forms[12]), pk(forms[13], forms[14]));
            cP[4u * pos + 3u] = make_float4(pk(forms[15], forms[16]), pk(forms[17], 0.0f), 0.0f, 0.0f);
          }
        }
      }
      count += static_cast<uint32_t>(__builtin_popcountll(m));
      base += 64u;
    }
    __builtin_amdgcn_fence(__ATOMIC_RELEASE, "wavefront");
    __builtin_amdgcn_wave_barrier();
    list_count = count;
    if constexpr (STATS) { st_bin[0] += count; st_bin[1] += 1; }
    return base < src_count ? base : src_count;
  };

  if constexpr (BIN && ONEPASS) {
    const size_t slot = (static_cast<size_t>(by) * gxb + bx) * 4u + wave;
    const uint32_t count = list_word & 0x3FFu;
    sure_hit_tile = loaded_sure;
    sure_winner = (list_word >> 10) & 0x3FFu;
    if (p.tile_lists != nullptr) {
      const uint32_t* const saved = p.tile_lists + slot * (1u + L);
      for (uint32_t base = 0; base < (sure_hit_tile ? 0u : count); base += 64u) {
        const uint32_t e = base + lane;
        if (e < count) {
          const uint32_t tri = saved[1u + e];
          cA[2u * e] = p.tri_a[2u * tri];
          cA[2u * e + 1u] = p.tri_a[2u * tri + 1u];
          cB[e] = p.tri_b[tri];
          cI[e] = static_cast<int>(tri);
        }
      }
    }
    __builtin_amdgcn_fence(__ATOMIC_RELEASE, "wavefront");
    __builtin_amdgcn_wave_barrier();
    list_count = count;
    if constexpr (STATS) { st_bin[0] += count; st_bin[1] += 1; }
    list_complete = true;
  }
  bool forms_ready = false;
  if constexpr (PRETEST && !HBM) {
    const uint32_t next0 = classify(0u, std::true_type{});
    list_complete = next0 >= src_count;
    forms_ready = pretest && list_complete;
  }
  if constexpr (HBM) forms_ready = true;
  if constexpr (RNG_LATE) load_rng();
  tl_mark(1);
  float4 sure_col = make_float4(0.0f, 0.0f, 0.0f, 0.0f);
  const bool sure_sums = BIN && ONEPASS && p.sure_table != nullptr;
  if constexpr (BIN && ONEPASS) { if (sure_hit_tile) sure_col = sure_sums ? p.sure_table[sure_winner] : p.tri_color[sure_winner]; }
  if constexpr (STATS && BIN && ONEPASS) {
    if (lane == 0u && p.stats != nullptr)
      atomicAdd(p.stats + (sure_hit_tile ? 13 : list_count == 0u ? 11 : list_count == 1u ? 12 : list_count == 2u ? 14 : 15), 1ull);
  }
  const uint32_t iters = FUSE ? p.iters : 1u;
  float rx = 0.0f, ry = 0.0f, rz = 0.0f, rw = 0.0f;
  uint32_t cnt_first = 0u;
  for (uint32_t it = 0; it < iters; ++it) {
  if constexpr (FUSE) { ax = 0.0f; ay = 0.0f; az = 0.0f; }
  uint32_t traced_samples = p.samples;
  if constexpr (BIN && ONEPASS) {
    if (sure_hit_tile) {
      rtd::rng_discard(rng, 3u * p.samples);
      if (sure_sums) { ax = sure_col.x; ay = sure_col.y; az = sure_col.z; }
      else for (uint32_t s = 0; s < p.samples; ++s) { ax += sure_col.x; ay += sure_col.y; az += sure_col.z; }
      if constexpr (STATS) st_pre += (p.samples + static_cast<uint32_t>(K) - 1u) / static_cast<uint32_t>(K);
      traced_samples = 0u;
    }
  }
  for (uint32_t s0 = 0; s0 < traced_samples; s0 += K) {
    if (s0 == static_cast<uint32_t>(K)) tl_mark(2);
    const uint32_t valid_k = (p.samples - s0 < static_cast<uint32_t>(K)) ? p.samples - s0 : static_cast<uint32_t>(K);
    V3 o[K], d[K];
    float best_t[K];
    int best_i[K];
#pragma unroll
    for (int k = 0; k < K; ++k) {
      if (static_cast<uint32_t>(k) < valid_k) get_ray<FMA>(p, focal, rng, o[k], d[k]);
      else { o[k] = {0.0f, 0.0f, 0.0f}; d[k] = {0.0f, 0.0f, -1.0f}; }
      best_t[k] = nearest ? FLT_MAX : -FLT_MAX;
      best_i[k] = -1;
    }

    const unsigned long long lanes_in = __builtin_amdgcn_ballot_w64(inside);
    unsigned long long pad_mask[K];
#pragma unroll
    for (int k = 0; k < K; ++k) pad_mask[k] = (static_cast<uint32_t>(k) < valid_k) ? 0ull : ~0ull;
    float dox[K], doy[K];
    float dFx = 0.0f, dFy = 0.0f, dFz = 0.0f;
    if constexpr (PRETEST) {
#pragma unroll
      for (int k = 0; k < K; ++k) { dox[k] = o[k].x - p.cam[9]; doy[k] = o[k].y - p.cam[10]; }
      dFx = focal.x - fam.fc[0]; dFy = focal.y - fam.fc[1]; dFz = focal.z - fam.fc[2];
    }
    if constexpr (BIN && ONEPASS) {
      for (uint32_t j = 0; j < list_count; ++j) {
        const float4 A0 = cA[2u * j], A1 = cA[2u * j + 1u];
        test_triangle<FMA, K, FILTER, STATS>(A0, A1, [&] { return cB[j]; }, cI[j], o, d, best_t, best_i,
                                             nearest, inside, valid_k, st_exit, st_skip);
      }
    } else if constexpr (BIN) {
      uint32_t base = 0;
      do {
        uint32_t next = src_count;
        if constexpr (!HBM) {
          if (!list_complete) {
            next = classify(base, std::false_type{});
            if (base == 0u && next >= src_count) list_complete = true;
          }
        }
        auto forms_eval = [&](const float4 f0, const float4 f1, const float4 q2, const float4 q3) -> bool {
          const float f2 = q2.x;
          typedef _Float16 h2 __attribute__((ext_vector_type(2)));
          const h2 w0 = __builtin_bit_cast(h2, q2.y), w1 = __builtin_bit_cast(h2, q2.z), w2 = __builtin_bit_cast(h2, q2.w),
                   w3 = __builtin_bit_cast(h2, q3.x), w4 = __builtin_bit_cast(h2, q3.y);
          const float b1 = __builtin_fmaf(static_cast<float>(w1.y), dFz, __builtin_fmaf(static_cast<float>(w0.x), dFy, __builtin_fmaf(static_cast<float>(w0.y), dFx, f0.x)));
          const float b2 = __builtin_fmaf(static_cast<float>(w2.x), dFz, __builtin_fmaf(static_cast<float>(w2.y), dFy, __builtin_fmaf(static_cast<float>(w1.x), dFx, f0.w)));
          const float b3 = __builtin_fmaf(static_cast<float>(w4.y), dFz, __builtin_fmaf(static_cast<float>(w3.x), dFy, __builtin_fmaf(static_cast<float>(w3.y), dFx, f1.z)));
          unsigned long long all_neg = ~0ull;
#pragma unroll
          for (int k = 0; k < K; ++k) {
            const float F1 = __builtin_fmaf(f0.z, doy[k], __builtin_fmaf(f0.y, dox[k], b1));
            const float F2 = __builtin_fmaf(f1.y, doy[k], __builtin_fmaf(f1.x, dox[k], b2));
            const float F3 = __builtin_fmaf(f2, doy[k], __builtin_fmaf(f1.w, dox[k], b3));
            const float worst = __builtin_fminf(__builtin_fminf(F1, F2), F3);
            all_neg &= __builtin_amdgcn_ballot_w64(worst < 0.0f) | pad_mask[k];
          }
          const bool alive = (~all_neg & lanes_in) != 0ull;
          if constexpr (STATS) { if (!alive) st_pre += 1; }
          return alive;
        };
        auto forms_alive = [&](uint32_t j) -> bool { return forms_eval(cP[4u * j], cP[4u * j + 1u], cP[4u * j + 2u], cP[4u * j + 3u]); };
        auto run_tests = [&](uint32_t j) {
          const float4 A0 = cA[2u * j], A1 = cA[2u * j + 1u];
          test_triangle<FMA, K, FILTER, STATS>(A0, A1, [&] { return cB[j]; }, HBM ? static_cast<int>(j) : cI[j], o, d, best_t, best_i,
                                               nearest, inside, valid_k, st_exit, st_skip);
        };
        if (forms_ready) {
          uint32_t j = 0;
          for (; j + 1u < list_count; j += 2u) {
            const bool a0 = forms_alive(j), a1 = forms_alive(j + 1u);
            if (a0) run_tests(j);
            if (a1) run_tests(j + 1u);
          }
          if (j < list_count && forms_alive(j)) run_tests(j);
        } else {
          for (uint32_t j = 0; j < list_count; ++j) run_tests(j);
        }
        base = next;
        if (!list_complete) __builtin_amdgcn_wave_barrier();
      } while (!list_complete && base < src_count);
      if constexpr (HBM) {
        if (hbm_overflow) {
          for (uint32_t e = 0; e < n_src; ++e) {
            const uint32_t tri = mI != nullptr ? static_cast<uint32_t>(__builtin_amdgcn_readfirstlane(static_cast<int>(mI[e]))) : e;
            const float4 A0 = p.tri_a[2u * tri], A1 = p.tri_a[2u * tri + 1u];
            const float bz = p.tri_b[tri];
            test_triangle<FMA, K, FILTER, STATS>(A0, A1, [&] { return bz; }, static_cast<int>(tri), o, d, best_t, best_i,
                                                 nearest, inside, valid_k, st_exit, st_skip);
          }
        }
      }
    } else {
      for (uint32_t c0 = 0; c0 < n; c0 += p.chunk) {
        const uint32_t cn = (n - c0 < p.chunk) ? n - c0 : p.chunk;
        if (!single_chunk) {
          __syncthreads();
          for (uint32_t i = threadIdx.x; i < 2u * cn; i += 256u) sA[i] = p.tri_a[2u * c0 + i];
          for (uint32_t i = threadIdx.x; i < cn; i += 256u) sB[i] = p.tri_b[c0 + i];
          __syncthreads();
        }
        for (uint32_t j = 0; j < cn; ++j) {
          const float4 A0 = sA[2u * j], A1 = sA[2u * j + 1u];
          test_triangle<FMA, K, FILTER, STATS>(A0, A1, [&] { return sB[j]; }, static_cast<int>(c0 + j), o, d,
                                               best_t, best_i, nearest, inside, valid_k, st_exit, st_skip);
        }
      }
    }
// ... 132 lines not shown
```

### raytracertest_amd/csrc/rt_tracer.hip

```cpp
#include <hip/hip_runtime.h>

#include <atomic>
#include <chrono>
#include <condition_variable>
#include <functional>
#include <cmath>
#include <cstdarg>
#include <cstdio>
#include <cstring>
#include <ctime>
#include <map>
#include <mutex>
#include <string>
#include <thread>
#include <vector>

#include "../../include/rt_mi355x.h"
#include "rt_device_math.hpp"
#include "rt_kernels.hpp"
#include "rt_rng_host.hpp"

namespace {

std::mutex g_err_mu;
std::string g_last_error;

struct Env {
  bool log;
  bool no_split;
  bool no_pretest;
  bool no_sure_table;
  int row_interleave;
  long macro_cap;
  static bool on(const char* name) { const char* e = getenv(name); return e && e[0] == '1'; }
  Env() {
    log = getenv("RT_MI355X_LOG") != nullptr;
    no_split = on("RT_MI355X_NO_SPLIT");
    no_pretest = on("RT_MI355X_NO_PRETEST");
    no_sure_table = on("RT_MI355X_NO_SURE_TABLE");
    const char* ri = getenv("RT_MI355X_ROW_INTERLEAVE");
    row_interleave = (ri && (ri[0] == '0' || ri[0] == '1') && ri[1] == 0) ? ri[0] - '0' : -1;
    const char* mc = getenv("RT_MI355X_MACRO_CAP");
    macro_cap = mc ? strtol(mc, nullptr, 10) : 0;
  }
};
inline Env read_env() { return Env(); }

void set_global_error(const std::string& s) {
  std::lock_guard<std::mutex> lk(g_err_mu);
  g_last_error = s;
  static const bool log = getenv("RT_MI355X_LOG") != nullptr;
  if (log) fprintf(stderr, "[rt_mi355x] %s\n", s.c_str());
}

std::string fmt(const char* f, ...) {
  char buf[512];
  va_list ap;
  va_start(ap, f);
  vsnprintf(buf, sizeof buf, f, ap);
  va_end(ap);
  return buf;
}

struct HipFail { std::string what; };
#define HIP_CHECK(expr)                                                                   \
  do {                                                                                    \
    hipError_t e_ = (expr);                                                               \
    if (e_ != hipSuccess) throw HipFail{fmt("%s failed: %s", #expr, hipGetErrorString(e_))}; \
  } while (0)

std::mutex g_jump_mu;
std::vector<uint32_t> g_jump_host;
std::map<int, uint32_t*> g_jump_dev;

const std::vector<uint32_t>& jump_host() {
  std::lock_guard<std::mutex> lk(g_jump_mu);
  if (g_jump_host.empty()) g_jump_host = rth::build_jump_table();
  return g_jump_host;
}

constexpr size_t kJumpWords = 32u * 160u * 8u;

uint32_t* jump_device(int device) {
  const std::vector<uint32_t>& h = jump_host();
  std::lock_guard<std::mutex> lk(g_jump_mu);
  auto it = g_jump_dev.find(device);
  if (it != g_jump_dev.end()) return it->second;
  static const std::vector<uint32_t> win = rth::build_window_tables(h);
  uint32_t* d = nullptr;
  HIP_CHECK(hipMalloc(&d, (h.size() + win.size()) * sizeof(uint32_t)));
  HIP_CHECK(hipMemcpy(d, h.data(), h.size() * sizeof(uint32_t), hipMemcpyHostToDevice));
  HIP_CHECK(hipMemcpy(d + h.size(), win.data(), win.size() * sizeof(uint32_t), hipMemcpyHostToDevice));
  g_jump_dev[device] = d;
  return d;
}

struct Camera {
  float position[3];
  float angles[2];
  float fov;
  float focal, aperture;
  float M[16];

  static float radians(float deg) { return deg * 0.01745329251994329576923690768489f; }

  void transform() {
    float sx, cx, sy, cy;
    rtd::sincos_spec(angles[0] * 0.5f, sx, cx);
    rtd::sincos_spec(angles[1] * 0.5f, sy, cy);
    const float Xw = cx, Xx = 1.0f * sx, Xy = 0.0f * sx, Xz = 0.0f * sx;
    const float Yw = cy, Yx = 0.0f * sy, Yy = 1.0f * sy, Yz = 0.0f * sy;
    const float w = Yw * Xw - Yx * Xx - Yy * Xy - Yz * Xz;
    const float x = Yw * Xx + Yx * Xw + Yy * Xz - Yz * Xy;
    const float y = Yw * Xy + Yy * Xw + Yz * Xx - Yx * Xz;
    const float z = Yw * Xz + Yz * Xw + Yx * Xy - Yy * Xx;
    const float qxx = x * x, qyy = y * y, qzz = z * z, qxz = x * z, qxy = x * y, qyz = y * z;
    const float qwx = w * x, qwy = w * y, qwz = w * z;
    memset(M, 0, sizeof M);
    M[0] = 1.0f - 2.0f * (qyy + qzz); M[1] = 2.0f * (qxy + qwz);        M[2] = 2.0f * (qxz - qwy);
    M[4] = 2.0f * (qxy - qwz);        M[5] = 1.0f - 2.0f * (qxx + qzz); M[6] = 2.0f * (qyz + qwx);
    M[8] = 2.0f * (qxz + qwy);        M[9] = 2.0f * (qyz - qwx);        M[10] = 1.0f - 2.0f * (qxx + qyy);
    M[15] = 1.0f;
  }
  float tan_half_fov() const {
    float s, c;
    rtd::sincos_spec(fov / 2.0f, s, c);
    return s / c;
  }
};

#ifndef RT_EVENT_STRIDE
#define RT_EVENT_STRIDE 16
#endif
#ifndef RT_PRETEST_LIST
#define RT_PRETEST_LIST 84u
#endif
struct EventPair { hipEvent_t a, b, c; uint32_t launches; bool split; uint64_t seq; };

class RenderThread {
 public:
  ~RenderThread() { shutdown(); }
  bool busy() const { return busy_.load(std::memory_order_acquire); }
  void run(std::function<void()> job) {
    std::unique_lock<std::mutex> lk(mu_);
    done_cv_.wait(lk, [&] { return !busy_.load(); });
    if (!th_.joinable()) th_ = std::thread([this] { loop(); });
    job_ = std::move(job);
    busy_.store(true, std::memory_order_release);
    posted_.store(true, std::memory_order_release);
    lk.unlock();
    cv_.notify_one();
  }
  void wait_idle() {
    if (!busy()) return;
    for (int i = 0; i < 2000 && busy(); ++i) spin_pause();
    std::unique_lock<std::mutex> lk(mu_);
    done_cv_.wait(lk, [&] { return !busy_.load(); });
  }
  void shutdown() {
    {
      std::unique_lock<std::mutex> lk(mu_);
      done_cv_.wait(lk, [&] { return !busy_.load(); });
      quit_ = true;
    }
    cv_.notify_one();
    if (th_.joinable()) th_.join();
  }

 private:
  static void spin_pause() {
#if defined(__x86_64__) || defined(__i386__)
    __builtin_ia32_pause();
#endif
  }
  void loop() {
    for (;;) {
      const auto t0 = std::chrono::steady_clock::now();
      while (!posted_.load(std::memory_order_acquire) &&
             std::chrono::steady_clock::now() - t0 < std::chrono::microseconds(50)) spin_pause();
      std::function<void()> job;
      {
        std::unique_lock<std::mutex> lk(mu_);
        cv_.wait(lk, [&] { return posted_.load() || quit_; });
        if (!posted_.load()) return;
        posted_.store(false);
        job = std::move(job_);
        job_ = nullptr;
      }
      job();
      {
        std::lock_guard<std::mutex> lk(mu_);
        busy_.store(false, std::memory_order_release);
      }
      done_cv_.notify_all();
    }
  }
// ... 50 lines not shown
    a_dirty = false;
  }
  void mark_b_dirty() { std::lock_guard<std::mutex> lk(order_mu); b_dirty = true; }
  float4* d_render = nullptr;
  uint32_t* d_counts = nullptr;
  uint32_t* d_image = nullptr;
  uint32_t* d_rng = nullptr;
  uint32_t* h_image = nullptr;
  uint32_t* h_image_alt = nullptr;
  uint32_t* image_mirror = nullptr;
  hipEvent_t handoff_event = nullptr;
  int handoff_next = 0;
  float4* d_tri = nullptr;
  float* d_tri_b = nullptr;
  float4* d_tri_color = nullptr;
  uint32_t n_tris = 0;
  float4* d_spheres = nullptr;
  uint32_t n_spheres = 0;

  std::mutex state_mu;
  Camera cam;
  rt_callback_fn update_cb = nullptr; void* update_user = nullptr;
  rt_callback_fn finished_cb = nullptr; void* finished_user = nullptr;

  std::mutex api_mu;
  RenderThread render;
  std::atomic<bool> stopped{false};
  std::atomic<bool> completed{false};

  std::mutex time_mu;
  std::vector<EventPair> pending;
  std::vector<EventPair> free_events;
  uint64_t next_event_seq = 0;
  double kernel_ms = 0.0;
  double span_ms = 0.0;
  uint64_t kernel_launches = 0;

  std::mutex err_mu;
  std::string last_error;
  uint32_t last_k = 0, last_chunk = 0, last_lds = 0;

  void set_error(const std::string& s) {
    { std::lock_guard<std::mutex> lk(err_mu); last_error = s; }
    set_global_error(s);
  }
  uint32_t npix() const { return W * rows; }
  void use_device() { HIP_CHECK(hipSetDevice(device)); }

  void cancel_and_join() {
    if (render.busy()) {
      stopped = true;
      render.wait_idle();
      stopped = false;
    }
  }

  void release_buffers() {
    if (d_render) (void)hipFree(d_render);
    if (d_counts) (void)hipFree(d_counts);
    if (d_image) (void)hipFree(d_image);
    if (d_rng) (void)hipFree(d_rng);
    if (h_image) (void)hipHostFree(h_image);
    if (h_image_alt) (void)hipHostFree(h_image_alt);
    h_image_alt = nullptr;
    d_render = nullptr; d_counts = nullptr; d_image = nullptr; d_rng = nullptr; h_image = nullptr;
  }

  void create_states() {
    uint32_t seeded[6];
    rth::seed_state(seed, seeded);
    const uint32_t p0 = row0 * W;
    if (static_cast<uint64_t>(W) * H > 0xFFFFFFFFull) throw HipFail{"frames above 2^32 pixels are not supported (32-bit pixel index, Kernels.cuh:128)"};
    uint32_t* const tables = jump_device(device);
    HIP_CHECK(rtk::launch_rng_init(d_rng, npix(), p0, seeded, tables, tables + kJumpWords, main_stream()));
  }

  void create_buffers() {
    const size_t n = npix();
    if (n == 0) throw HipFail{"image has no pixels"};
    HIP_CHECK(hipMalloc(&d_rng, n * 6 * sizeof(uint32_t)));
    HIP_CHECK(hipMalloc(&d_render, n * sizeof(float4)));
    HIP_CHECK(hipMalloc(&d_counts, n * sizeof(uint32_t)));
    HIP_CHECK(hipMalloc(&d_image, n * sizeof(uint32_t)));
    HIP_CHECK(hipHostMalloc(&h_image, n * sizeof(uint32_t), hipHostMallocDefault));
    HIP_CHECK(hipHostMalloc(&h_image_alt, n * sizeof(uint32_t), hipHostMallocDefault));
    memset(h_image, 0, n * sizeof(uint32_t));
    memset(h_image_alt, 0, n * sizeof(uint32_t));
    HIP_CHECK(hipMemsetAsync(d_render, 0, n * sizeof(float4), main_stream()));
    HIP_CHECK(hipMemsetAsync(d_counts, 0, n * sizeof(uint32_t), main_stream()));
    HIP_CHECK(hipMemsetAsync(d_image, 0, n * sizeof(uint32_t), main_stream()));
    create_states();
    HIP_CHECK(hipStreamSynchronize(main_stream()));
  }

  void reshape(uint32_t w, uint32_t h, uint32_t r0, uint32_t n) {
    HIP_CHECK(hipStreamSynchronize(main_stream()));
    sync_list_stream();
    release_buffers();
    W = w; H = h; row0 = r0; rows = n;
    list_key_valid = false;
    create_buffers();
  }

  void copy_image_to(uint32_t* target) {
    HIP_CHECK(hipMemcpyAsync(target, d_image, static_cast<size_t>(npix()) * sizeof(uint32_t), hipMemcpyDeviceToDevice, main_stream()));
  }

  void tile_corner_bound(rtk::TraceParams& p) const {
    p.tile_curv = -1.0f; p.tile_round = 0.0f;
    double G[3][3];
    for (int i = 0; i < 3; ++i)
      for (int j = 0; j < 3; ++j) {
        G[i][j] = 0.0;
        for (int r = 0; r < 3; ++r) G[i][j] += static_cast<double>(p.cam[i * 3 + r]) * static_cast<double>(p.cam[j * 3 + r]);
      }
    double lmax = 0.0, lmin = 1e300;
    for (int i = 0; i < 3; ++i) {
      const double off = std::fabs(G[i][(i + 1) % 3]) + std::fabs(G[i][(i + 2) % 3]);
      lmax = std::max(lmax, G[i][i] + off);
      lmin = std::min(lmin, G[i][i] - off);
    }
    if (!(lmin > 0.25) || !(lmax < 4.0)) return;
    const double hh = std::fabs(static_cast<double>(p.half_height)), asp = std::fabs(static_cast<double>(p.aspect));
    const double a = 7.0 * 2.0 * hh * asp / static_cast<double>(W), b = 7.0 * 2.0 * hh / static_cast<double>(H);
    if (!(0.5 * (a * a + b * b) * (lmax / lmin) <= 0.1 * std::min(a, b))) return;
    const double foc = std::fabs(static_cast<double>(p.focal));
#ifndef RT_TILE_CURV_SCALE
#define RT_TILE_CURV_SCALE 1.0
#endif
    const double curv = foc * 0.5 * (a * a + b * b) * (lmax / lmin) * 1.001 * RT_TILE_CURV_SCALE + 1e-30;
    const double pos = std::max(std::fabs(p.cam[9]), std::max(std::fabs(p.cam[10]), std::fabs(p.cam[11])));
    const double round = foc * (1.0 + hh * asp + hh) + pos;
    if (!(curv <= 1e30) || !(round <= 1e30)) return;
    p.tile_curv = std::nextafter(static_cast<float>(curv), 3.0e38f);
    p.tile_round = std::nextafter(static_cast<float>(round), 3.0e38f);
  }

  rtk::TraceParams params(uint32_t samples) {
    rtk::TraceParams p;
    memset(&p, 0, sizeof p);
    Camera c;
    { std::lock_guard<std::mutex> lk(state_mu); c = cam; }
    p.render = d_render; p.counts = d_counts; p.rng = d_rng;
    p.W = W; p.H = H; p.row0 = row0; p.rows = rows; p.npix = npix(); p.samples = samples;
    for (int col = 0; col < 4; ++col)
      for (int r = 0; r < 3; ++r) p.cam[col * 3 + r] = c.M[col * 4 + r];
    p.half_height = c.tan_half_fov();
    p.aspect = static_cast<float>(W) / static_cast<float>(H);
    p.focal = c.focal; p.aperture = c.aperture;
    tile_corner_bound(p);
    p.tri_a = d_tri; p.tri_b = d_tri_b; p.tri_color = d_tri_color; p.n_tris = n_tris;
    p.tri_n = smooth_normals ? d_tri_n : nullptr;
    p.stats = nullptr;
    p.spheres = d_spheres; p.n_spheres = n_spheres;
    p.chunk = chunk_req ? chunk_req : 1024u;
    if (p.chunk > 4096u) p.chunk = 4096u;
    uint32_t want = bin_list_req ? bin_list_req : ((n_tris + 31u) / 32u) * 32u;
    want = ((want + 31u) / 32u) * 32u;
    p.bin_list = want < 32u ? 32u : want > (bin_list_req ? 960u : 256u) ? (bin_list_req ? 960u : 256u) : want;
    p.block_list = n_tris > p.bin_list ? 1024u : 0u;
    if (p.block_list != 0u && !bin_list_req) p.bin_list = 192u;
    if (pretest && filter && bin && n_tris >= kPretestMinTris && n_tris <= 50000u) {
      p.pretest_on = 1u;
      if (!bin_list_req) p.bin_list = RT_PRETEST_LIST;
      else p.bin_list = (p.bin_list + 1u) & ~1u;
      if (p.block_list != 0u) p.block_list = 448u;
    }
    return p;
  }

  uint32_t mode_flags(const rtk::TraceParams& p) const {
    return (nearest_hit ? rtk::TRACE_NEAREST_HIT : 0u) | (p.pretest_on ? rtk::TRACE_PRETEST : 0u) |
           (sure_hit ? 0u : rtk::TRACE_NO_SURE_HIT);
  }

  int pick_k(uint32_t samples) const {
    if (k_req == 1 || k_req == 2 || k_req == 4) return static_cast<int>(k_req);
    const uint32_t want = (n_tris <= 128u) ? 2u : 4u;
    return samples >= want ? static_cast<int>(want) : samples >= 2 ? 2 : 1;
  }

  EventPair take_events() {
    std::lock_guard<std::mutex> lk(time_mu);
    if (!free_events.empty()) { EventPair e = free_events.back(); free_events.pop_back(); return e; }
    EventPair e{};
    HIP_CHECK(hipEventCreate(&e.a));
    HIP_CHECK(hipEventCreate(&e.b));
    HIP_CHECK(hipEventCreate(&e.c));
    return e;
  }

  void enqueue_trace_launch(uint32_t samples, uint32_t flags, int sync_after, uint32_t iters = 1,
                            uint32_t* host_image = nullptr, bool allow_split = true) {
    const int K = pick_k(samples);
    rtk::TraceParams p = params(samples);
    p.iters = iters;
    p.image_host = host_image;
    p.flags = flags | mode_flags(p);
    p.image = d_image;
    bool have_lists = false;
    const bool build_lists = prepare_tile_lists(p, (flags & rtk::TRACE_ZERO_ACC) != 0u, have_lists);
    attach_sure_table(p, have_lists);
    last_k = K; last_chunk = p.chunk;
    last_lds = rtk::trace_lds_bytes(p, bin);
    const bool timed = sync_after == 1 || (launch_counter++ % kEventStride) == 0u;
    const uint32_t r0 = allow_split ? split_row(p.rows) : 0u;
    EventPair e{};
    if (timed) { e = take_events(); e.launches = 1; e.split = r0 != 0u; }
    if (r0 == 0u) {
      (void)main_stream();
      if (build_lists) build_tile_lists_ahead(p);
      attach_tile_lists(p, have_lists);
      if (timed) HIP_CHECK(hipEventRecord(e.a, stream));
      if (have_lists) wait_for_lists(stream, list_waited_a);
      attach_macro_lists(p, 0, stream, (flags & rtk::TRACE_ZERO_ACC) != 0u);
      HIP_CHECK(rtk::launch_trace(p, fma, filter, bin, K, stream));
      if (timed) HIP_CHECK(hipEventRecord(e.b, stream));
    } else {
      fork_b();
      if (build_lists) build_tile_lists_ahead(p);
      const bool stagger = stagger_next.exchange(false);
      const bool interleave = have_lists && want_interleave();
      if (have_lists && interleave != rows_interleaved) {
        (void)main_stream();
        fork_b();
        rows_interleaved = interleave;
        if (env.log) fprintf(stderr, "[rt_mi355x] split launches: halves by %s\n", interleave ? "even / odd block rows" : "rows");
      }
      rtk::TraceParams half[2] = {sub_band(p, 0u, r0), sub_band(p, r0, p.rows - r0)};
      if (interleave) { half[0] = p; half[1] = p; half[0].row_il = half[1].row_il = 1u; half[1].row_phase = 1u; }
      hipStream_t st[2] = {stream, stream_b};
      if (timed) HIP_CHECK(hipEventRecord(e.a, stream));
      for (int h = 0; h < 2; ++h) {
        attach_tile_lists(half[h], have_lists);
        if (have_lists) wait_for_lists(st[h], h == 0 ? list_waited_a : list_waited_b);
        if (h == 1 && stagger) {
          const uint32_t us = static_cast<uint32_t>(last_half_ms.load() * 450.0f);
          if (us >= 5u) HIP_CHECK(rtk::launch_delay(us, stream_b));
          else HIP_CHECK(hipStreamWaitEvent(stream_b, stagger_event, 0));
        }
        attach_macro_lists(half[h], h, st[h], (flags & rtk::TRACE_ZERO_ACC) != 0u);
        HIP_CHECK(rtk::launch_trace(half[h], fma, filter, bin, K, st[h]));
        if (h == 0 && stagger) HIP_CHECK(hipEventRecord(stagger_event, stream));
      }
      if (timed) { HIP_CHECK(hipEventRecord(e.b, stream)); HIP_CHECK(hipEventRecord(e.c, stream_b)); }
      mark_b_dirty();
    }
    if (!timed) return;
    const EventPair* wait_for = nullptr;
    EventPair waited{};
    size_t back = 2;
    {
      std::lock_guard<std::mutex> lk(time_mu);
      if (sync_after == 0) reap_finished_locked();
      e.seq = next_event_seq++;
      pending.push_back(e);
      const size_t stride = kEventStride;
      back = (static_cast<size_t>(sync_after > 1 ? sync_after : 2) + stride - 1u) / stride;
      if (back < 2u) back = 2u;
      if (sync_after == 1) { waited = e; wait_for = &waited; }
      else if (sync_after > 1 && pending.size() >= back) { waited = pending[pending.size() - back]; wait_for = &waited; }
    }
    if (wait_for) {
      HIP_CHECK(hipEventSynchronize(wait_for->b));
      if (wait_for->split) HIP_CHECK(hipEventSynchronize(wait_for->c));
      if (sync_after > 1) drain_events(back - 1u);
    }
  }

  static rtk::TraceParams sub_band(const rtk::TraceParams& p, uint32_t off, uint32_t n) {
    rtk::TraceParams q = p;
    const size_t px = static_cast<size_t>(off) * p.W;
    q.row0 = p.row0 + off; q.rows = n;
    q.render = p.render + px; q.counts = p.counts + px; q.rng = p.rng + px;
    q.image = p.image + px;
    if (p.image_host != nullptr) q.image_host = p.image_host + px;
    return q;
  }

  void recycle_locked(size_t n_done) {
    for (size_t i = 0; i < n_done; ++i) {
      EventPair& e = pending[i];
      float ms = 0.0f;
      if (hipEventElapsedTime(&ms, e.a, e.b) == hipSuccess) {
        kernel_ms += ms; kernel_launches += e.launches;
        if (e.split && e.launches == 1) last_half_ms = ms;
        float lower = 0.0f;
        if (e.split && hipEventElapsedTime(&lower, e.a, e.c) == hipSuccess && lower > ms) ms = lower;
        span_ms += ms;
      }
      free_events.push_back(e);
    }
    pending.erase(pending.begin(), pending.begin() + static_cast<std::ptrdiff_t>(n_done));
  }
  void drain_events(size_t keep_last = 0) {
    std::lock_guard<std::mutex> lk(time_mu);
    if (pending.size() > keep_last) recycle_locked(pending.size() - keep_last);
  }
  void drain_events_before(uint64_t seq_end) {
    std::lock_guard<std::mutex> lk(time_mu);
    size_t n = 0;
    while (n < pending.size() && pending[n].seq < seq_end) ++n;
    recycle_locked(n);
  }
  void reap_finished_locked() {
    size_t n = 0;
    while (n < pending.size() && hipEventQuery(pending[n].b) == hipSuccess &&
           (!pending[n].split || hipEventQuery(pending[n].c) == hipSuccess)) ++n;
    (void)hipGetLastError();
    recycle_locked(n);
  }
  uint64_t event_seq_now() { std::lock_guard<std::mutex> lk(time_mu); return next_event_seq; }

  void clear_accumulators() {
    HIP_CHECK(hipMemsetAsync(d_render, 0, static_cast<size_t>(npix()) * sizeof(float4), main_stream()));
    HIP_CHECK(hipMemsetAsync(d_counts, 0, static_cast<size_t>(npix()) * sizeof(uint32_t), main_stream()));
  }

  void convert() {
    HIP_CHECK(rtk::launch_convert(d_render, d_counts, d_image, npix(), main_stream()));
  }

  static void sync_polling(hipStream_t st) {
    const auto t0 = std::chrono::steady_clock::now();
    for (;;) {
      const hipError_t e = hipStreamQuery(st);
      if (e == hipSuccess) return;
      if (e != hipErrorNotReady) HIP_CHECK(e);
      if (std::chrono::steady_clock::now() - t0 > std::chrono::milliseconds(2)) break;
    }
    (void)hipGetLastError();
    HIP_CHECK(hipStreamSynchronize(st));
  }

  void fetch_image() {
    HIP_CHECK(hipMemcpyAsync(h_image, d_image, static_cast<size_t>(npix()) * sizeof(uint32_t),
                             hipMemcpyDeviceToHost, main_stream()));
    HIP_CHECK(hipStreamSynchronize(main_stream()));
  }

  struct ListKey {
    float cam[12], half_height, aspect, focal, aperture;
    uint32_t W, H, row0, rows, bin_list, n_tris, scene_generation;
    bool fma;
  };
  static constexpr int kListRing = 8, kFreeEvents = 10;
  int ring_n = 8, kFreeStride = 4;
  uint32_t* d_list_ring[kListRing] = {};
  hipEvent_t list_ready[kListRing] = {};
  hipEvent_t list_free_a[kFreeEvents] = {}, list_free_b[kFreeEvents] = {};
  uint64_t list_free_build[kFreeEvents] = {};
  uint64_t list_alloc_build = 0;
  uint64_t list_free_waited = 0;
  int list_cur = 0;
  uint64_t list_builds = 0;
  uint64_t list_waited_a = 0, list_waited_b = 0;
  hipStream_t stream_l = nullptr;
  std::atomic<bool> stagger_next{true};
  hipEvent_t stagger_event = nullptr;
  std::atomic<float> last_half_ms{0.0f};
  size_t tile_lists_words = 0;
  uint32_t* tile_lists_now() const { return d_list_ring[list_cur]; }
  uint32_t* d_half_cost = nullptr;
  unsigned long long* h_half_cost = nullptr;
  bool rows_interleaved = false;
  bool want_interleave() {
    if (env.row_interleave >= 0) return env.row_interleave != 0;
    if (h_half_cost == nullptr) return false;
    const unsigned long long w = *reinterpret_cast<volatile unsigned long long*>(h_half_cost);
    const double u = static_cast<double>(w & 0xFFFFFFFFull), l = static_cast<double>(w >> 32);
    if (u + l < 16.0) return rows_interleaved;
    const double ratio = (u > l ? u : l) / ((u > l ? l : u) + 1.0);
    return rows_interleaved ? ratio > 1.15 : ratio > 1.25;
  }
  uint32_t split_row(uint32_t band_rows) const {
    return (split_launches && band_rows >= 128u) ? ((band_rows / 2u + 7u) / 8u) * 8u : 0u;
  }
  void release_tile_lists() {
    for (int r = 0; r < kListRing; ++r) { if (d_list_ring[r]) (void)hipFree(d_list_ring[r]); d_list_ring[r] = nullptr; }
    tile_lists_words = 0; list_key_valid = false; list_cur = 0; list_alloc_build = list_builds;
  }
  void sync_list_stream() { if (stream_l) HIP_CHECK(hipStreamSynchronize(stream_l)); }
  ListKey list_key{};
  bool list_key_valid = false;
  uint32_t scene_generation = 0;

  bool prepare_tile_lists(const rtk::TraceParams& p, bool first_launch_of_trace, bool& have) {
    have = false;
    if (!bin || p.n_tris == 0u || p.n_tris > p.bin_list) return false;
    have = true;
    const size_t tiles = static_cast<size_t>((W + 31u) / 32u) * ((rows + 7u) / 8u + 1u) * 4u;
    const size_t words = tiles * (1u + p.bin_list);
    if (words > tile_lists_words) {
      HIP_CHECK(hipStreamSynchronize(main_stream()));
      sync_list_stream();
      release_tile_lists();
      {
        const bool big = words * sizeof(uint32_t) > (size_t(128) << 20);
        ring_n = big ? 4 : 8; kFreeStride = big ? 2 : 4;
      }
      for (int r = 0; r < ring_n; ++r) {
        HIP_CHECK(hipMalloc(&d_list_ring[r], words * sizeof(uint32_t)));
        HIP_CHECK(hipMemsetAsync(d_list_ring[r], 0, words * sizeof(uint32_t), stream_l));
      }
      tile_lists_words = words;
    }
    ListKey k;
    memset(&k, 0, sizeof k);
    memcpy(k.cam, p.cam, sizeof k.cam);
    k.half_height = p.half_height; k.aspect = p.aspect; k.focal = p.focal; k.aperture = p.aperture;
    k.W = p.W; k.H = p.H; k.row0 = p.row0; k.rows = p.rows; k.bin_list = p.bin_list; k.n_tris = p.n_tris;
    k.scene_generation = scene_generation; k.fma = fma;
    const bool same = list_key_valid && memcmp(&k, &list_key, sizeof k) == 0 && !(first_launch_of_trace && !reuse_across_traces);
    if (same) return false;
    list_key = k;
    list_key_valid = true;
    return true;
  }

  void attach_tile_lists(rtk::TraceParams& p, bool have) {
    p.tile_lists = nullptr;
    if (!have) return;
    const size_t slot_base = static_cast<size_t>((W + 31u) / 32u) * ((p.row0 - row0) / 8u) * 4u;
    p.tile_lists = tile_lists_now() + slot_base * (1u + p.bin_list);
  }

  float4* d_sure_table = nullptr;
  uint32_t sure_table_cap = 0, sure_table_samples = 0;
  uint64_t sure_table_scene = ~0ull;
  void attach_sure_table(rtk::TraceParams& p, bool have) {
    p.sure_table = nullptr;
    if (!have || env.no_sure_table || p.n_tris == 0u) return;
    if (sure_table_samples != p.samples || sure_table_scene != scene_generation || sure_table_cap < p.n_tris) {
      hipStream_t st = main_stream();
      if (sure_table_cap < p.n_tris) {
        HIP_CHECK(hipStreamSynchronize(st));
        if (d_sure_table) { HIP_CHECK(hipFree(d_sure_table)); d_sure_table = nullptr; }
        HIP_CHECK(hipMalloc(&d_sure_table, static_cast<size_t>(p.n_tris) * sizeof(float4)));
        sure_table_cap = p.n_tris;
      }
      HIP_CHECK(rtk::launch_sure_table(p.tri_color, p.n_tris, p.samples, d_sure_table, st));
      sure_table_samples = p.samples; sure_table_scene = scene_generation;
    }
    p.sure_table = d_sure_table;
  }

  void build_tile_lists_ahead(const rtk::TraceParams& p_band) {
    const uint64_t m = list_builds;
    if (m > 0 && m % kFreeStride == 0) {
      const int i = static_cast<int>((m / kFreeStride) % kFreeEvents);
      HIP_CHECK(hipEventRecord(list_free_a[i], stream));
      HIP_CHECK(hipEventRecord(list_free_b[i], stream_b));
      list_free_build[i] = m;
    }
    const int r = static_cast<int>(m % ring_n);
    if (m >= list_alloc_build + ring_n) {
      const uint64_t e = ((m - ring_n + 1 + kFreeStride - 1) / kFreeStride) * kFreeStride;
      const int i = static_cast<int>((e / kFreeStride) % kFreeEvents);
      if (list_free_build[i] != e) throw HipFail{"list ring: the free event of the slot's readers is missing"};
      if (e != list_free_waited) {
        HIP_CHECK(hipStreamWaitEvent(stream_l, list_free_a[i], 0));
        HIP_CHECK(hipStreamWaitEvent(stream_l, list_free_b[i], 0));
        list_free_waited = e;
      }
    }
    list_cur = r;
    rtk::TraceParams q = p_band;
    attach_tile_lists(q, true);
    const uint32_t sr = split_row(rows);
    if (sr != 0u && d_half_cost != nullptr && env.row_interleave < 0 && (m % 32u) == 0u) { q.half_cost = d_half_cost; q.cost_split_brow = sr / 8u; }
    HIP_CHECK(rtk::launch_tile_lists(q, fma, stream_l));
    HIP_CHECK(hipEventRecord(list_ready[r], stream_l));
    if (q.half_cost != nullptr) HIP_CHECK(rtk::launch_publish_half_cost(d_half_cost, h_half_cost, stream_l));
    ++list_builds;
  }
  void wait_for_lists(hipStream_t st, uint64_t& waited) {
    if (waited == list_builds) return;
    HIP_CHECK(hipStreamWaitEvent(st, list_ready[list_cur], 0));
    waited = list_builds;
  }

  static constexpr uint32_t kEventStride = RT_EVENT_STRIDE;
  std::atomic<uint32_t> launch_counter{0};
  uint32_t* d_macro_lists[2] = {nullptr, nullptr};
  size_t macro_lists_words[2] = {0, 0};
  bool macro = true;
  bool pretest = true;
  bool sure_hit = true;
  bool reuse_across_traces = true;
  static constexpr uint32_t kPretestMinTris = 4096;
  static constexpr uint32_t kMacroW = 128, kMacroH = 64, kMacroCapMax = 65536;
#ifndef RT_SUPER_F
#define RT_SUPER_F 4
#endif
  static constexpr uint32_t kSuperF = RT_SUPER_F, kSuperMinTris = 2048;
  bool super_level = true;
  uint32_t* d_super_lists[2] = {nullptr, nullptr};
  size_t super_lists_words[2] = {0, 0};

  ListKey macro_key[2] = {};
  bool macro_key_valid[2] = {false, false};
  void attach_macro_lists(rtk::TraceParams& p, int half, hipStream_t st, bool first_launch_of_trace = true) {
    p.macro_lists = nullptr;
    if (!bin || !macro || p.n_tris <= p.bin_list) return;
    p.macro_w = kMacroW; p.macro_h = kMacroH;
    p.macro_nx = (p.W + p.macro_w - 1u) / p.macro_w;
    const uint32_t ny = (p.rows + p.macro_h - 1u) / p.macro_h;
    p.macro_cap = p.n_tris < kMacroCapMax ? p.n_tris : kMacroCapMax;
    if (env.macro_cap > 0 && static_cast<uint32_t>(env.macro_cap) < p.macro_cap) p.macro_cap = static_cast<uint32_t>(env.macro_cap);
    const size_t words = static_cast<size_t>(p.macro_nx) * ny * (p.macro_cap + 1u);
    if (words > macro_lists_words[half]) {
      if (d_macro_lists[half]) (void)hipFree(d_macro_lists[half]);
      d_macro_lists[half] = nullptr; macro_lists_words[half] = 0; macro_key_valid[half] = false;
      HIP_CHECK(hipMalloc(&d_macro_lists[half], words * sizeof(uint32_t)));
      macro_lists_words[half] = words;
    }
    p.macro_lists = d_macro_lists[half];
    p.super_lists = nullptr; p.macro_bounds = nullptr; p.super_f = 0u; p.super_chunks = 0u; p.super_nx = 0u;
    const uint32_t chunks = (p.n_tris + rtk::kSuperChunk - 1u) / rtk::kSuperChunk;
    if (super_level && p.n_tris >= kSuperMinTris && chunks <= rtk::kSuperMaxChunks && p.macro_nx * ny > kSuperF * kSuperF) {
      p.super_f = kSuperF; p.super_chunks = chunks;
      p.super_nx = (p.macro_nx + kSuperF - 1u) / kSuperF;
      const size_t sw = static_cast<size_t>(p.super_nx) * ((ny + kSuperF - 1u) / kSuperF) * chunks * (rtk::kSuperChunk + 1u) +
                        static_cast<size_t>(p.macro_nx) * ny * 8u;
      if (sw > super_lists_words[half]) {
        if (d_super_lists[half]) (void)hipFree(d_super_lists[half]);
        d_super_lists[half] = nullptr; super_lists_words[half] = 0; macro_key_valid[half] = false;
        HIP_CHECK(hipMalloc(&d_super_lists[half], sw * sizeof(uint32_t)));
        super_lists_words[half] = sw;
      }
      p.super_lists = d_super_lists[half];
      p.macro_bounds = reinterpret_cast<float*>(d_super_lists[half] + (sw - static_cast<size_t>(p.macro_nx) * ny * 8u));
    }
    ListKey k;
    memset(&k, 0, sizeof k);
    memcpy(k.cam, p.cam, sizeof k.cam);
    k.half_height = p.half_height; k.aspect = p.aspect; k.focal = p.focal; k.aperture = p.aperture;
    k.W = p.W; k.H = p.H; k.row0 = p.row0; k.rows = p.rows; k.bin_list = p.macro_cap * 65536u + p.macro_w * 256u + p.macro_h; k.n_tris = p.n_tris;
    k.scene_generation = scene_generation; k.fma = fma;
    const bool same = macro_key_valid[half] && memcmp(&k, &macro_key[half], sizeof k) == 0 && !(first_launch_of_trace && !reuse_across_traces);
    if (!same) {
      macro_key[half] = k;
      macro_key_valid[half] = true;
      if (p.super_lists != nullptr) HIP_CHECK(rtk::launch_super_bin(p, fma, st));
      HIP_CHECK(rtk::launch_macro_bin(p, fma, st));
    }
    attach_wave_lists(p, half, st, !same);
  }

  static constexpr size_t kWaveListsMaxBytes = size_t(6) << 30;
  uint32_t* d_wave_lists[2] = {nullptr, nullptr};
  size_t wave_lists_words[2] = {0, 0};
  bool wave_lists_valid[2] = {false, false};
  void attach_wave_lists(rtk::TraceParams& p, int half, hipStream_t st, bool macro_rebuilt) {
    p.wave_lists = nullptr; p.wave_cap = 0u;
    if (macro_rebuilt) wave_lists_valid[half] = false;
    if (!p.pretest_on || p.stats != nullptr || p.macro_lists == nullptr) return;
    const size_t tiles = static_cast<size_t>((p.W + 31u) / 32u) * ((p.rows + 7u) / 8u) * 4u;
    const size_t words = tiles * (1u + p.bin_list) * 16u;
    if (words * sizeof(uint32_t) > kWaveListsMaxBytes) return;
    if (words > wave_lists_words[half]) {
      if (d_wave_lists[half]) (void)hipFree(d_wave_lists[half]);
      d_wave_lists[half] = nullptr; wave_lists_words[half] = 0; wave_lists_valid[half] = false;
      HIP_CHECK(hipMalloc(&d_wave_lists[half], words * sizeof(uint32_t)));
      wave_lists_words[half] = words;
    }
    p.wave_lists = d_wave_lists[half]; p.wave_cap = p.bin_list;
    if (!wave_lists_valid[half]) {
      HIP_CHECK(rtk::launch_wave_lists(p, fma, st));
      wave_lists_valid[half] = true;
    }
  }

  static constexpr int kWindow = 4;

  void trace_enqueue_body(uint32_t iterationCount, uint32_t samplesPerIteration, uint32_t* target) {
    use_device();
    if (iterationCount == 0) {
      clear_accumulators();
      convert();
      if (target) copy_image_to(target);
      return;
    }
    const uint32_t group = fused_iterations(samplesPerIteration);
    for (uint32_t i = 0; i < iterationCount;) {
      const uint32_t n = iterationCount - i < group ? iterationCount - i : group;
      const bool last = i + n == iterationCount;
      enqueue_trace_launch(samplesPerIteration, (i == 0 ? rtk::TRACE_ZERO_ACC : 0u) | (last ? rtk::TRACE_EMIT_IMAGE : 0u),
                           0, n, last ? target : nullptr);
      i += n;
    }
  }

  uint32_t fused_iterations(uint32_t samplesPerIteration) const {
    if (!rtk::trace_can_fuse(filter, bin) || samplesPerIteration == 0u) return 1u;
    const uint32_t n = 64u / samplesPerIteration;
    return n < 1u ? 1u : n;
  }

  void trace_funct(uint32_t iterationCount, uint32_t samplesPerIteration, uint32_t updateInterval) {
    try {
      use_device();
      bool cleared = false;
      struct { bool due = false; uint32_t* image = nullptr; rt_callback_fn cb = nullptr; void* user = nullptr; } pend;
      auto deliver = [&] {
        if (!pend.due) return;
        HIP_CHECK(hipEventSynchronize(handoff_event));
        pend.cb(pend.image, static_cast<size_t>(npix()) * sizeof(uint32_t), pend.user);
        pend.due = false;
      };
      uint32_t* final_image = h_image;
      uint32_t i = 0;
      while (!stopped && i < iterationCount) {
        rt_callback_fn cb; void* user;
        { std::lock_guard<std::mutex> lk(state_mu); cb = update_cb; user = update_user; }
        auto is_update = [&](uint32_t k) { return cb != nullptr && k > 0 && updateInterval > 0 && k % updateInterval == 0; };
        const uint32_t last_allowed = iterationCount - 1u - i < fused_iterations(samplesPerIteration) - 1u
                                          ? iterationCount - 1u : i + fused_iterations(samplesPerIteration) - 1u;
        uint32_t e = i;
        while (e < last_allowed && !is_update(e)) ++e;
        const bool update = is_update(e);
        const bool emit = update || e + 1 == iterationCount;
        const uint32_t flags = (cleared ? 0u : rtk::TRACE_ZERO_ACC) | (emit ? rtk::TRACE_EMIT_IMAGE : 0u);
        uint32_t* const target = emit ? (handoff_next ? h_image_alt : h_image) : nullptr;
        if (emit && pend.due && pend.image == target) deliver();
        enqueue_trace_launch(samplesPerIteration, flags, kWindow, e - i + 1u, target, false);
        cleared = true;
        deliver();
        if (emit) { final_image = target; handoff_next ^= 1; }
        if (update) {
          HIP_CHECK(hipEventRecord(handoff_event, main_stream()));
          pend.due = true; pend.image = target; pend.cb = cb; pend.user = user;
        }
        i = e + 1u;
      }
      deliver();
      drain_events();
      if (!cleared) {
        clear_accumulators();
        if (!stopped) convert();
      }
      if (stopped) { HIP_CHECK(hipStreamSynchronize(main_stream())); return; }
      if (cleared && i == iterationCount) {
        sync_polling(main_stream());
      } else {
        fetch_image();
        final_image = h_image;
      }
      completed = true;
      rt_callback_fn cb; void* user;
      { std::lock_guard<std::mutex> lk(state_mu); cb = finished_cb; user = finished_user; }
      if (cb != nullptr) cb(final_image, static_cast<size_t>(npix()) * sizeof(uint32_t), user);
    } catch (const HipFail& f) {
      set_error(f.what);
    } catch (...) {
      set_error("unknown failure in the render thread");
    }
  }
};

#include "rt_multi.hpp"

namespace {

size_t buffer_bytes(rt_tracer* t, int which) {
  const size_t n = t->npix();
  switch (which) {
    case RT_BUF_RENDER: return n * sizeof(float4);
    case RT_BUF_COUNTS: return n * sizeof(uint32_t);
    case RT_BUF_IMAGE: return n * sizeof(uint32_t);
    case RT_BUF_RNG: return n * 6 * sizeof(uint32_t);
    case RT_BUF_FRAME: {
      const Group* g = t->mg ? &t->mg->group : t->grp;
      return (g && g->has_root) ? g->frame_bytes() : 0;
    }
    default: return 0;
  }
}

void* buffer_ptr(rt_tracer* t, int which) {
  if (which == RT_BUF_FRAME || (t->mg && which == RT_BUF_IMAGE)) {
    Group* g = t->mg ? &t->mg->group : t->grp;
    return (g && g->has_root) ? g->d_frame[g->last_b < 0 ? 0 : g->last_b] : nullptr;
  }
  if (t->mg) return nullptr;
  switch (which) {
    case RT_BUF_RENDER: return t->d_render;
    case RT_BUF_COUNTS: return t->d_counts;
    case RT_BUF_IMAGE: return t->d_image;
    case RT_BUF_RNG: return t->d_rng;
    default: return nullptr;
  }
}

template <class F>
int guarded(rt_tracer* t, F&& f) {
  try {
    f();
    return RT_OK;
  } catch (const HipFail& e) {
    if (t) t->set_error(e.what); else set_global_error(e.what);
    return RT_ERR_HIP;
  } catch (const std::exception& e) {
    if (t) t->set_error(e.what()); else set_global_error(e.what());
    return RT_ERR_STATE;
  } catch (...) {
    if (t) t->set_error("unknown failure"); else set_global_error("unknown failure");
    return RT_ERR_STATE;
  }
}

struct DevBuf {
  void* p = nullptr;
  explicit DevBuf(size_t bytes) { HIP_CHECK(hipMalloc(&p, bytes ? bytes : 1)); }
  ~DevBuf() { if (p) (void)hipFree(p); }
  template <class T> T* as() { return static_cast<T*>(p); }
};

int require_device(int device) {
  int n = 0;
  hipError_t e = hipGetDeviceCount(&n);
  if (e != hipSuccess || n <= 0) {
    set_global_error(fmt("no HIP device available (%s); librt_mi355x has no CPU fallback",
                         e == hipSuccess ? "device count 0" : hipGetErrorString(e)));
    return RT_ERR_NO_DEVICE;
  }
  if (device < 0 || device >= n) {
    set_global_error(fmt("device %d out of range (%d devices)", device, n));
    return RT_ERR_INVALID;
  }
  return RT_OK;
}

}

#include "rt_multi_api.hpp"

extern "C" {

#ifndef RT_KERNEL_SOURCE_HASH
#define RT_KERNEL_SOURCE_HASH "unknown"
#endif
const char* rt_version(void) { return "rt_mi355x 0.2 (gfx950, kernels=" RT_KERNEL_SOURCE_HASH ")"; }

int rt_device_count(void) {
  int n = 0;
  if (hipGetDeviceCount(&n) != hipSuccess) return 0;
  return n;
}

const char* rt_last_error(void) {
  static thread_local std::string copy;
  std::lock_guard<std::mutex> lk(g_err_mu);
  copy = g_last_error;
  return copy.c_str();
}

const char* rt_tracer_last_error(rt_tracer* t) {
  static thread_local std::string copy;
  if (!t) return rt_last_error();
  std::lock_guard<std::mutex> lk(t->err_mu);
  copy = t->last_error;
  return copy.c_str();
}

int rt_tracer_create_ex(const uint32_t imageSize[2], const float cameraPosition[3],
                        const float cameraAngles[2], float fov, float focalLength, float aperture,
                        const rt_options* options, rt_tracer** out) {
  if (!out) return RT_ERR_INVALID;
  *out = nullptr;
  if (!imageSize || !cameraAngles || imageSize[0] == 0 || imageSize[1] == 0) {
    set_global_error("rt_tracer_create: invalid image size or camera angles");
    return RT_ERR_INVALID;
  }
  rt_options opt;
  memset(&opt, 0, sizeof opt);
  opt.use_time_seed = 1;
  if (options) {
    const size_t n = options->struct_size < sizeof(opt) ? options->struct_size : sizeof(opt);
    if (n < 8) { set_global_error("rt_options.struct_size not set"); return RT_ERR_INVALID; }
    opt.use_time_seed = 0;
    memcpy(&opt, options, n);
  }
  int rc = require_device(opt.device);
  if (rc != RT_OK) return rc;

  rt_tracer* t = new rt_tracer();
  t->device = opt.device;
  t->W = imageSize[0];
  if (opt.full_height) {
    t->band_mode = true;
    t->H = opt.full_height; t->row0 = opt.row_begin; t->rows = imageSize[1];
    if (static_cast<uint64_t>(t->row0) + t->rows > t->H) {
      delete t;
      set_global_error("row band exceeds full_height");
      return RT_ERR_INVALID;
    }
  } else {
    t->H = imageSize[1]; t->row0 = 0; t->rows = imageSize[1];
  }
  t->seed = opt.use_time_seed ? static_cast<uint64_t>(static_cast<uint32_t>(time(nullptr))) : opt.seed;
  t->fma = opt.math_mode != RT_MATH_STRICT;
  t->filter = (opt.flags & RT_FLAG_NO_FILTER) == 0;
  t->bin = (opt.flags & RT_FLAG_NO_BINNING) == 0;
  t->nearest_hit = (opt.flags & RT_FLAG_NEAREST_HIT) != 0;
  t->smooth_normals = (opt.flags & RT_FLAG_SMOOTH_NORMALS) != 0;
  t->env = read_env();
  t->pretest = !t->env.no_pretest;
  t->sure_hit = (opt.flags & RT_FLAG_NO_SURE_HIT) == 0;
  t->split_launches = !t->env.no_split;
  t->macro = (opt.flags & RT_FLAG_NO_MACRO_BINS) == 0;
  t->super_level = (opt.flags & RT_FLAG_NO_SUPER_BINS) == 0;
  t->k_req = opt.samples_in_flight;
  t->chunk_req = opt.lds_chunk;
  t->bin_list_req = opt.bin_list;
  Camera& c = t->cam;
  for (int i = 0; i < 3; ++i) c.position[i] = cameraPosition ? cameraPosition[i] : 0.0f;
  c.angles[0] = cameraAngles[0]; c.angles[1] = cameraAngles[1];
  c.fov = Camera::radians(fov);
  c.focal = focalLength; c.aperture = aperture;
  c.transform();
  rc = guarded(t, [&] {
    t->use_device();
    HIP_CHECK(hipStreamCreateWithFlags(&t->stream, hipStreamNonBlocking));
    HIP_CHECK(hipStreamCreateWithFlags(&t->stream_b, hipStreamNonBlocking));
    {
      int lo = 0, hi = 0;
      if (hipDeviceGetStreamPriorityRange(&lo, &hi) == hipSuccess && hi != lo)
        HIP_CHECK(hipStreamCreateWithPriority(&t->stream_l, hipStreamNonBlocking, hi));
      else
        HIP_CHECK(hipStreamCreateWithFlags(&t->stream_l, hipStreamNonBlocking));
      HIP_CHECK(hipEventCreateWithFlags(&t->stagger_event, hipEventDisableTiming));
      HIP_CHECK(hipMalloc(&t->d_half_cost, 2 * sizeof(uint32_t)));
      HIP_CHECK(hipMemset(t->d_half_cost, 0, 2 * sizeof(uint32_t)));
      HIP_CHECK(hipDeviceSynchronize());
      HIP_CHECK(hipHostMalloc(&t->h_half_cost, sizeof(unsigned long long), hipHostMallocDefault));
      *t->h_half_cost = 0ull;
      for (int r = 0; r < rt_tracer::kListRing; ++r) HIP_CHECK(hipEventCreateWithFlags(&t->list_ready[r], hipEventDisableTiming));
      for (int r = 0; r < rt_tracer::kFreeEvents; ++r) {
        HIP_CHECK(hipEventCreateWithFlags(&t->list_free_a[r], hipEventDisableTiming));
        HIP_CHECK(hipEventCreateWithFlags(&t->list_free_b[r], hipEventDisableTiming));
      }
    }
    HIP_CHECK(hipEventCreateWithFlags(&t->handoff_event, hipEventDisableTiming));
    HIP_CHECK(hipEventCreateWithFlags(&t->join_event, hipEventDisableTiming));
    HIP_CHECK(hipEventCreateWithFlags(&t->fork_event, hipEventDisableTiming));
    t->create_buffers();
  });
  if (rc != RT_OK) {
    std::string why = t->last_error;
    t->release_buffers();
    if (t->handoff_event) (void)hipEventDestroy(t->handoff_event);
    if (t->join_event) (void)hipEventDestroy(t->join_event);
    if (t->fork_event) (void)hipEventDestroy(t->fork_event);
    if (t->stream_b) (void)hipStreamDestroy(t->stream_b);
    if (t->stream) (void)hipStreamDestroy(t->stream);
    delete t;
    set_global_error("rt_tracer_create: " + why);
    return rc;
  }
  *out = t;
  return RT_OK;
}

int rt_tracer_create(const uint32_t imageSize[2], const float cameraPosition[3],
                     const float cameraAngles[2], float fov, float focalLength, float aperture,
                     rt_tracer** out) {
  return rt_tracer_create_ex(imageSize, cameraPosition, cameraAngles, fov, focalLength, aperture,
                             nullptr, out);
}

void rt_tracer_destroy(rt_tracer* t) {
  if (!t) return;
  t->stopped = true;
  t->render.shutdown();
  if (t->mg) {
    multi_destroy(t);
    delete t;
    return;
  }
  member_leave(t);
  (void)hipSetDevice(t->device);
  if (t->stream_b) (void)hipStreamSynchronize(t->stream_b);
  if (t->stream) (void)hipStreamSynchronize(t->stream);
  t->drain_events();
  for (EventPair& e : t->free_events) { (void)hipEventDestroy(e.a); (void)hipEventDestroy(e.b); (void)hipEventDestroy(e.c); }
  if (t->stream_l) (void)hipStreamSynchronize(t->stream_l);
  t->release_tile_lists();
  for (int r = 0; r < rt_tracer::kListRing; ++r)
    if (t->list_ready[r]) (void)hipEventDestroy(t->list_ready[r]);
  for (int r = 0; r < rt_tracer::kFreeEvents; ++r) {
    if (t->list_free_a[r]) (void)hipEventDestroy(t->list_free_a[r]);
    if (t->list_free_b[r]) (void)hipEventDestroy(t->list_free_b[r]);
  }
  if (t->stream_l) (void)hipStreamDestroy(t->stream_l);
  if (t->stagger_event) (void)hipEventDestroy(t->stagger_event);
  if (t->d_half_cost) (void)hipFree(t->d_half_cost);
  if (t->h_half_cost) (void)hipHostFree(t->h_half_cost);
  for (int h = 0; h < 2; ++h) if (t->d_macro_lists[h]) (void)hipFree(t->d_macro_lists[h]);
  for (int h = 0; h < 2; ++h) if (t->d_super_lists[h]) (void)hipFree(t->d_super_lists[h]);
  for (int h = 0; h < 2; ++h) if (t->d_wave_lists[h]) (void)hipFree(t->d_wave_lists[h]);
  if (t->d_tri_n) (void)hipFree(t->d_tri_n);
  if (t->d_tri) (void)hipFree(t->d_tri);
  if (t->d_tri_b) (void)hipFree(t->d_tri_b);
  if (t->d_tri_color) (void)hipFree(t->d_tri_color);
  if (t->d_sure_table) (void)hipFree(t->d_sure_table);
  if (t->d_spheres) (void)hipFree(t->d_spheres);
  t->release_buffers();
  if (t->handoff_event) (void)hipEventDestroy(t->handoff_event);
  if (t->join_event) (void)hipEventDestroy(t->join_event);
  if (t->fork_event) (void)hipEventDestroy(t->fork_event);
  if (t->stream_b) (void)hipStreamDestroy(t->stream_b);
  if (t->stream) (void)hipStreamDestroy(t->stream);
  delete t;
}

int rt_tracer_trace(rt_tracer* t, uint32_t iterationCount, uint32_t samplesPerIteration,
                    uint32_t updateInterval) {
  if (!t) return RT_ERR_INVALID;
  std::lock_guard<std::mutex> lk(t->api_mu);
  return guarded(t, [&] {
    t->cancel_and_join();
    t->completed = false;
    if (t->mg) t->render.run([=] { multi_trace_funct(t, iterationCount, samplesPerIteration, updateInterval); });
    else t->render.run([=] { t->trace_funct(iterationCount, samplesPerIteration, updateInterval); });
  });
}

void rt_tracer_stop(rt_tracer* t) {
  if (t) t->stopped = true;
}

int rt_tracer_wait(rt_tracer* t) {
  if (!t) return 0;
  std::lock_guard<std::mutex> lk(t->api_mu);
  t->render.wait_idle();
  t->stopped = false;
  return t->completed ? 1 : 0;
}

int rt_tracer_resize(rt_tracer* t, const uint32_t size[2]) {
  if (!t || !size || size[0] == 0 || size[1] == 0) return RT_ERR_INVALID;
  std::lock_guard<std::mutex> lk(t->api_mu);
  return guarded(t, [&] {
    t->cancel_and_join();
    if (t->mg) { multi_resize(t, size[0], size[1]); return; }
    if (t->grp) throw HipFail{"Resize: the tracer is a member of a multi-process group (leave and re-join with the new bands)"};
    t->use_device();
    HIP_CHECK(hipStreamSynchronize(t->main_stream()));
    t->release_buffers();
    t->W = size[0];
    if (t->band_mode) {
      if (static_cast<uint64_t>(t->row0) + size[1] > t->H) throw HipFail{"row band exceeds full_height"};
      t->rows = size[1];
    } else {
      t->H = size[1]; t->rows = size[1];
    }
    t->create_buffers();
  });
}

void rt_tracer_set_camera_parameters(rt_tracer* t, float fov, float focalLength, float aperture) {
  if (!t) return;
  std::lock_guard<std::mutex> lk(t->state_mu);
  t->cam.fov = Camera::radians(fov);
  t->cam.focal = focalLength;
  t->cam.aperture = aperture;
}

void rt_tracer_rotate_camera(rt_tracer* t, const float angles[2]) {
  if (!t || !angles) return;
  std::lock_guard<std::mutex> lk(t->state_mu);
  t->cam.angles[0] += angles[0];
  t->cam.angles[1] += angles[1];
  t->cam.transform();
}

static int upload_scene_impl(rt_tracer* t, const rt_float4* hostData, size_t count, bool edges) {
  if (!t) return RT_ERR_INVALID;
  if (!hostData || count < 3 || count % 3 != 0) {
    t->set_error(fmt("UploadScene got invalid triangle list. Size = %zu", count));
    return RT_ERR_INVALID;
  }
  std::lock_guard<std::mutex> lk(t->api_mu);
  if (t->mg) {
    int rc = guarded(t, [&] { t->cancel_and_join(); multi_sync_all(t); });
    for (rt_tracer* b : t->mg->bands) {
      if (rc != RT_OK) break;
      rc = upload_scene_impl(b, hostData, count, edges);
      if (rc != RT_OK) t->set_error(b->last_error);
    }
    if (rc == RT_OK) { t->n_tris = static_cast<uint32_t>(count / 3); t->scene_generation++; }
    return rc;
  }
  return guarded(t, [&] {
    t->cancel_and_join();
    t->use_device();
    HIP_CHECK(hipStreamSynchronize(t->main_stream()));
    t->sync_list_stream();
    if (t->d_tri) { (void)hipFree(t->d_tri); t->d_tri = nullptr; }
    if (t->d_tri_b) { (void)hipFree(t->d_tri_b); t->d_tri_b = nullptr; }
    if (t->d_tri_color) { (void)hipFree(t->d_tri_color); t->d_tri_color = nullptr; }
    if (t->d_tri_n) { (void)hipFree(t->d_tri_n); t->d_tri_n = nullptr; }
    t->n_tris = 0;
    const uint32_t n = static_cast<uint32_t>(count / 3);
    DevBuf verts(count * sizeof(float4));
    HIP_CHECK(hipMalloc(&t->d_tri, static_cast<size_t>(n) * 2 * sizeof(float4)));
    HIP_CHECK(hipMalloc(&t->d_tri_b, static_cast<size_t>(n) * sizeof(float)));
    HIP_CHECK(hipMalloc(&t->d_tri_color, static_cast<size_t>(n) * sizeof(float4)));
    if (edges) HIP_CHECK(hipMalloc(&t->d_tri_n, static_cast<size_t>(n) * 3 * sizeof(float4)));
    HIP_CHECK(hipMemcpyAsync(verts.p, hostData, count * sizeof(float4), hipMemcpyHostToDevice, t->main_stream()));
    HIP_CHECK(rtk::launch_prep_triangles(t->fma, edges, verts.as<float4>(), n, t->d_tri, t->d_tri_b,
                                         t->d_tri_color, t->d_tri_n, t->main_stream()));
    HIP_CHECK(hipStreamSynchronize(t->main_stream()));
    t->n_tris = n;
    t->scene_generation++;
  });
}

int rt_tracer_upload_scene(rt_tracer* t, const rt_float4* hostData, size_t count) {
  return upload_scene_impl(t, hostData, count, false);
}

int rt_tracer_upload_scene_edges(rt_tracer* t, const rt_float4* hostData, size_t count) {
  return upload_scene_impl(t, hostData, count, true);
}

float rt_pack_normal(const float n[3]) {
  return floorf(n[0] * 127.0f + 127.5f) / 256.0f + floorf(n[1] * 127.0f + 127.5f) / 65536.0f +
         floorf(n[2] * 127.0f + 127.5f) / 16777216.0f;
}

void rt_unpack_normal(float packed, float n[3]) {
  const float m[3] = {1.0f, 256.0f, 65536.0f};
  for (int i = 0; i < 3; ++i) {
    const float s = packed * m[i];
    const float frac = s - floorf(s);
    n[i] = floorf(frac * 256.0f) / 127.0f - 1.0f;
  }
}

int rt_tracer_upload_spheres(rt_tracer* t, const rt_float4* spheres, size_t count) {
  if (!t || (count && !spheres)) return RT_ERR_INVALID;
  std::lock_guard<std::mutex> lk(t->api_mu);
  if (t->mg) {
    int rc = guarded(t, [&] { t->cancel_and_join(); multi_sync_all(t); });
    for (rt_tracer* b : t->mg->bands) {
      if (rc != RT_OK) break;
      rc = rt_tracer_upload_spheres(b, spheres, count);
      if (rc != RT_OK) t->set_error(b->last_error);
// ... 26 lines not shown
  t->finished_cb = fn; t->finished_user = user;
}

int rt_tracer_set_seed(rt_tracer* t, uint64_t seed) {
  if (!t) return RT_ERR_INVALID;
  std::lock_guard<std::mutex> lk(t->api_mu);
  return guarded(t, [&] {
    t->cancel_and_join();
    t->seed = seed;
    if (t->mg) {
      t->mg->opt.seed = seed;
      for (rt_tracer* b : t->mg->bands)
        if (rt_tracer_set_seed(b, seed) != RT_OK) throw HipFail{b->last_error};
      return;
    }
    t->use_device();
    t->create_states();
    HIP_CHECK(hipStreamSynchronize(t->main_stream()));
  });
}

static void trace_enqueue_once(rt_tracer* t, uint32_t iterationCount, uint32_t samplesPerIteration) {
  if (t->mg) { multi_trace_enqueue(t, iterationCount, samplesPerIteration); return; }
  if (t->grp) {
    const size_t k = member_band_index(t);
    const int b = t->grp->begin_frame();
    t->trace_enqueue_body(iterationCount, samplesPerIteration, t->grp->tile_target(k, b));
    t->grp->tile_written(k);
    t->grp->gather(b);
    return;
  }
  t->trace_enqueue_body(iterationCount, samplesPerIteration, t->image_mirror);
}

int rt_tracer_trace_enqueue(rt_tracer* t, uint32_t iterationCount, uint32_t samplesPerIteration) {
  if (!t) return RT_ERR_INVALID;
  std::lock_guard<std::mutex> lk(t->api_mu);
  return guarded(t, [&] {
    t->cancel_and_join();
    trace_enqueue_once(t, iterationCount, samplesPerIteration);
  });
}

int rt_tracer_trace_enqueue_n(rt_tracer* t, uint32_t iterationCount, uint32_t samplesPerIteration, uint32_t n_steps) {
  if (!t) return RT_ERR_INVALID;
  std::lock_guard<std::mutex> lk(t->api_mu);
  return guarded(t, [&] {
    t->cancel_and_join();
    for (uint32_t s = 0; s < n_steps; ++s) trace_enqueue_once(t, iterationCount, samplesPerIteration);
  });
}

int rt_tracer_set_list_reuse(rt_tracer* t, int across_traces) {
  if (!t) return RT_ERR_INVALID;
  std::lock_guard<std::mutex> lk(t->api_mu);
  t->cancel_and_join();
  if (t->mg) for (rt_tracer* b : t->mg->bands) (void)rt_tracer_set_list_reuse(b, across_traces);
  t->reuse_across_traces = across_traces != 0;
  t->list_key_valid = false;
  return RT_OK;
}

int rt_tracer_set_image_mirror(rt_tracer* t, void* device_visible_image) {
  if (!t) return RT_ERR_INVALID;
  std::lock_guard<std::mutex> lk(t->api_mu);
  if (t->mg || t->grp) { t->set_error("rt_tracer_set_image_mirror: the gather owns the second image target of a sharded frame"); return RT_ERR_STATE; }
  t->image_mirror = static_cast<uint32_t*>(device_visible_image);
  return RT_OK;
}

int rt_tracer_fused_iterations(rt_tracer* t, uint32_t samples) {
  if (t && t->mg) return static_cast<int>(t->mg->bands[0]->fused_iterations(samples));
  return t ? static_cast<int>(t->fused_iterations(samples)) : 0;
}

static void launch_impl(rt_tracer* t, uint32_t samples, uint32_t iterations, bool clear_first, bool emit) {
  t->cancel_and_join();
  if (t->mg) { multi_launch(t, samples, iterations, clear_first, emit); return; }
  t->use_device();
  const uint32_t flags = (clear_first ? rtk::TRACE_ZERO_ACC : 0u) | (emit ? rtk::TRACE_EMIT_IMAGE : 0u);
  if (t->grp && emit) {
    const size_t k = member_band_index(t);
    const int b = t->grp->begin_frame();
    t->enqueue_trace_launch(samples, flags, 0, iterations, t->grp->tile_target(k, b));
    t->grp->tile_written(k);
    t->grp->gather(b);
    return;
  }
  t->enqueue_trace_launch(samples, flags, 0, iterations, emit ? t->image_mirror : nullptr);
}

int rt_tracer_launch_iterations(rt_tracer* t, uint32_t samples, uint32_t iterations, int clear_first, int emit_image) {
  if (!t || iterations == 0u) return RT_ERR_INVALID;
  if (iterations > static_cast<uint32_t>(rt_tracer_fused_iterations(t, samples))) {
    t->set_error(fmt("rt_tracer_launch_iterations: %u iterations of %u samples exceed rt_tracer_fused_iterations", iterations, samples));
    return RT_ERR_INVALID;
  }
  std::lock_guard<std::mutex> lk(t->api_mu);
  return guarded(t, [&] { launch_impl(t, samples, iterations, clear_first != 0, emit_image != 0); });
}

int rt_tracer_launch(rt_tracer* t, uint32_t samples, int clear_first, int emit_image) {
  if (!t) return RT_ERR_INVALID;
  std::lock_guard<std::mutex> lk(t->api_mu);
  return guarded(t, [&] { launch_impl(t, samples, 1u, clear_first != 0, emit_image != 0); });
}

int rt_tracer_trace_stats(rt_tracer* t, uint32_t samples, uint64_t out[16]) {
  if (!t || !out) return RT_ERR_INVALID;
  std::lock_guard<std::mutex> lk(t->api_mu);
  if (t->mg) {
    memset(out, 0, 16 * sizeof(uint64_t));
    t->cancel_and_join();
    multi_push_camera(t);
    for (rt_tracer* b : t->mg->bands) {
      uint64_t part[16];
      const int rc = rt_tracer_trace_stats(b, samples, part);
      if (rc != RT_OK) { t->set_error(b->last_error); return rc; }
      for (int i = 0; i < 16; ++i) out[i] += part[i];
    }
    return RT_OK;
  }
  return guarded(t, [&] {
    t->cancel_and_join();
    t->use_device();
    DevBuf counters(16 * sizeof(unsigned long long));
    HIP_CHECK(hipMemsetAsync(counters.p, 0, 16 * sizeof(unsigned long long), t->main_stream()));
    t->clear_accumulators();
    rtk::TraceParams p = t->params(samples);
    p.stats = counters.as<unsigned long long>();
    p.flags = t->mode_flags(p);
    bool have_lists = false;
    const bool build_lists = t->prepare_tile_lists(p, true, have_lists);
    t->sync_list_stream();
    t->attach_tile_lists(p, have_lists);
    if (have_lists) HIP_CHECK(rtk::launch_tile_lists(p, t->fma, t->main_stream()));
    (void)build_lists;
    t->attach_macro_lists(p, 0, t->main_stream());
    HIP_CHECK(rtk::launch_trace(p, t->fma, t->filter, t->bin, t->pick_k(samples), t->main_stream()));
    HIP_CHECK(hipStreamSynchronize(t->main_stream()));
    HIP_CHECK(hipMemcpy(out, counters.p, 16 * sizeof(uint64_t), hipMemcpyDeviceToHost));
  });
}

int rt_tracer_sync(rt_tracer* t) {
  if (!t) return RT_ERR_INVALID;
  if (t->mg) return guarded(t, [&] { multi_sync_all(t); });
  return guarded(t, [&] {
    t->use_device();
    const uint64_t seen = t->event_seq_now();
    HIP_CHECK(hipStreamSynchronize(t->main_stream()));
    t->sync_list_stream();
    t->stagger_next = true;
    t->drain_events_before(seen);
    if (t->grp) t->grp->sync();
  });
}

int rt_tracer_kernel_time(rt_tracer* t, double* total_ms, uint64_t* launches, int reset_after) {
  if (!t) return RT_ERR_INVALID;
  if (t->mg) {
    const int rc = rt_tracer_kernel_time(t->mg->bands[0], total_ms, launches, reset_after);
    if (reset_after) for (size_t k = 1; k < t->mg->bands.size(); ++k) (void)rt_tracer_kernel_time(t->mg->bands[k], nullptr, nullptr, 1);
    return rc;
  }
  std::lock_guard<std::mutex> lk(t->time_mu);
  if (total_ms) *total_ms = t->kernel_ms;
  if (launches) *launches = t->kernel_launches;
  if (reset_after) { t->kernel_ms = 0.0; t->span_ms = 0.0; t->kernel_launches = 0; t->launch_counter = 0; }
  return RT_OK;
}

int rt_tracer_launch_time(rt_tracer* t, double* total_ms, uint64_t* launches, int reset_after) {
  if (!t) return RT_ERR_INVALID;
  if (t->mg) {
    const int rc = rt_tracer_launch_time(t->mg->bands[0], total_ms, launches, reset_after);
    if (reset_after) for (size_t k = 1; k < t->mg->bands.size(); ++k) (void)rt_tracer_launch_time(t->mg->bands[k], nullptr, nullptr, 1);
    return rc;
  }
  std::lock_guard<std::mutex> lk(t->time_mu);
  if (total_ms) *total_ms = t->span_ms;
  if (launches) *launches = t->kernel_launches;
  if (reset_after) { t->kernel_ms = 0.0; t->span_ms = 0.0; t->kernel_launches = 0; t->launch_counter = 0; }
  return RT_OK;
}

size_t rt_tracer_buffer_bytes(rt_tracer* t, int which) { return t ? buffer_bytes(t, which) : 0; }
void* rt_tracer_device_pointer(rt_tracer* t, int which) { return t ? buffer_ptr(t, which) : nullptr; }

int rt_tracer_read_buffer(rt_tracer* t, int which, void* dst, size_t bytes) {
  if (!t || !dst) return RT_ERR_INVALID;
  if (t->mg) {
    if (bytes > buffer_bytes(t, which) || buffer_bytes(t, which) == 0) return RT_ERR_INVALID;
    return guarded(t, [&] { multi_read_buffer(t, which, dst, bytes); });
  }
  if (buffer_ptr(t, which) == nullptr || bytes > buffer_bytes(t, which)) return RT_ERR_INVALID;
  return guarded(t, [&] {
    t->use_device();
    HIP_CHECK(hipStreamSynchronize(t->main_stream()));
    if (t->grp) t->grp->sync();
    HIP_CHECK(hipMemcpy(dst, buffer_ptr(t, which), bytes, hipMemcpyDeviceToHost));
  });
}

int rt_tracer_copy_buffer_to_device(rt_tracer* t, int which, void* dst_device, size_t bytes) {
  if (!t || !dst_device || buffer_ptr(t, which) == nullptr || bytes > buffer_bytes(t, which)) return RT_ERR_INVALID;
  if (t->mg) return guarded(t, [&] {
    multi_sync_all(t);
    HIP_CHECK(hipSetDevice(t->mg->group.local[0].device));
    HIP_CHECK(hipMemcpy(dst_device, buffer_ptr(t, which), bytes, hipMemcpyDeviceToDevice));
  });
  return guarded(t, [&] {
    t->use_device();
    if (t->grp && which == RT_BUF_FRAME) t->grp->sync();
    HIP_CHECK(hipMemcpyAsync(dst_device, buffer_ptr(t, which), bytes, hipMemcpyDeviceToDevice, t->main_stream()));
    HIP_CHECK(hipStreamSynchronize(t->main_stream()));
  });
}

int rt_tracer_copy_buffer_to_device_async(rt_tracer* t, int which, void* dst_device, size_t bytes) {
  if (!t || !dst_device || buffer_ptr(t, which) == nullptr || bytes > buffer_bytes(t, which)) return RT_ERR_INVALID;
  if (t->mg || which == RT_BUF_FRAME) { t->set_error("rt_tracer_copy_buffer_to_device_async: per-stream copies are for plain tracers' own buffers"); return RT_ERR_STATE; }
  return guarded(t, [&] {
    t->use_device();
    HIP_CHECK(hipMemcpyAsync(dst_device, buffer_ptr(t, which), bytes, hipMemcpyDeviceToDevice, t->main_stream()));
  });
}

void* rt_tracer_stream(rt_tracer* t) { return (t && !t->mg) ? static_cast<void*>(t->stream) : nullptr; }
void* rt_tracer_stream_b(rt_tracer* t) { return (t && !t->mg) ? static_cast<void*>(t->stream_b) : nullptr; }

int rt_tracer_info(rt_tracer* t, uint32_t out[8]) {
  if (!t || !out) return RT_ERR_INVALID;
  if (t->mg) {
    (void)rt_tracer_info(t->mg->bands[0], out);
    out[3] = (t->W + 31) / 32; out[4] = (t->H + 7) / 8;
    out[7] = static_cast<uint32_t>(t->device);
    return RT_OK;
  }
  out[0] = t->last_k; out[1] = t->last_chunk; out[2] = t->last_lds;
  out[3] = (t->W + 31) / 32; out[4] = (t->rows + 7) / 8;
  out[5] = t->n_tris; out[6] = t->n_spheres; out[7] = static_cast<uint32_t>(t->device);
  return RT_OK;
}


int rt_tracer_create_multi(const uint32_t imageSize[2], const float cameraPosition[3], const float cameraAngles[2],
                           float fov, float focalLength, float aperture, const rt_options* options,
                           const int32_t* devices, uint32_t n_bands, rt_tracer** out) {
  return multi_create(imageSize, cameraPosition, cameraAngles, fov, focalLength, aperture, options, devices, n_bands, out);
}

int rt_group_unique_id(uint8_t id[RT_GROUP_ID_BYTES]) {
  if (!id) return RT_ERR_INVALID;
  return guarded(nullptr, [&] {
    ncclUniqueId uid;
    RCCL_CHECK(need_rccl().GetUniqueId(&uid));
    memcpy(id, uid.internal, RT_GROUP_ID_BYTES);
  });
}

int rt_tracer_join_group(rt_tracer* t, uint32_t n_ranks, uint32_t rank, const uint8_t id[RT_GROUP_ID_BYTES]) {
  if (!t || t->mg || n_ranks == 0u || rank >= n_ranks || (!id && n_ranks > 1u)) return RT_ERR_INVALID;
  static const uint8_t zero_id[RT_GROUP_ID_BYTES] = {0};
  std::lock_guard<std::mutex> lk(t->api_mu);
  return guarded(t, [&] {
    t->cancel_and_join();
    member_join(t, n_ranks, rank, id ? id : zero_id, nullptr);
  });
}

int rt_tracer_join_group_bands(rt_tracer* t, uint32_t n_ranks, uint32_t rank, const uint8_t id[RT_GROUP_ID_BYTES],
                               const uint32_t* row_begin) {
  if (!t || t->mg || n_ranks == 0u || rank >= n_ranks || (!id && n_ranks > 1u) || !row_begin) return RT_ERR_INVALID;
  static const uint8_t zero_id[RT_GROUP_ID_BYTES] = {0};
  std::lock_guard<std::mutex> lk(t->api_mu);
  return guarded(t, [&] {
    t->cancel_and_join();
    member_join(t, n_ranks, rank, id ? id : zero_id, row_begin);
  });
}

int rt_balance_rows(uint32_t n_bands, const uint32_t* row_begin, const double* cost, uint32_t granule, uint32_t* new_row_begin) {
  if (n_bands == 0u || !row_begin || !cost || !new_row_begin) return RT_ERR_INVALID;
  for (uint32_t k = 0; k < n_bands; ++k) if (row_begin[k + 1] <= row_begin[k]) return RT_ERR_INVALID;
  balance_rows(n_bands, row_begin, cost, granule, new_row_begin);
  return RT_OK;
}

int rt_tracer_set_band(rt_tracer* t, uint32_t row_begin, uint32_t rows) {
  if (!t || t->mg || rows == 0u) return RT_ERR_INVALID;
  std::lock_guard<std::mutex> lk(t->api_mu);
  return guarded(t, [&] {
    t->cancel_and_join();
    if (t->grp) throw HipFail{"rt_tracer_set_band: leave the group first"};
    if (!t->band_mode) throw HipFail{"rt_tracer_set_band: the tracer owns a whole image, not a band (rt_options.full_height)"};
    if (static_cast<uint64_t>(row_begin) + rows > t->H) throw HipFail{"row band exceeds full_height"};
    t->use_device();
    t->reshape(t->W, t->H, row_begin, rows);
  });
}

int rt_tracer_rebalance(rt_tracer* t) {
  if (!t || !t->mg) return RT_ERR_INVALID;
  std::lock_guard<std::mutex> lk(t->api_mu);
  return guarded(t, [&] {
// ... 24 lines not shown
    member_leave(t);
  });
}

int rt_tracer_gather_time(rt_tracer* t, double* total_ms, uint64_t* gathers, int reset_after) {
  if (!t) return RT_ERR_INVALID;
  Group* g = t->mg ? &t->mg->group : t->grp;
  if (total_ms) *total_ms = 0.0;
  if (gathers) *gathers = 0u;
  if (g) g->read_time(total_ms, gathers, reset_after != 0);
  return RT_OK;
}

int rt_tracer_gather_only(rt_tracer* t) {
  if (!t || (!t->mg && !t->grp)) return RT_ERR_INVALID;
  std::lock_guard<std::mutex> lk(t->api_mu);
  return guarded(t, [&] {
    t->cancel_and_join();
    group_gather_only(t);
  });
}

int rt_tracer_group_info(rt_tracer* t, char* json, size_t capacity) {
  if (!t || !json || capacity == 0) return RT_ERR_INVALID;
  const std::string s = group_info_json(t);
  if (s.size() + 1 > capacity) return RT_ERR_INVALID;
  memcpy(json, s.c_str(), s.size() + 1);
  return RT_OK;
}

int rt_tracer_band_count(rt_tracer* t) {
  if (!t) return 0;
  return t->mg ? static_cast<int>(t->mg->bands.size()) : 1;
}

int rt_tracer_band_info(rt_tracer* t, uint32_t band, uint32_t out[4]) {
  if (!t || !out) return RT_ERR_INVALID;
  if (t->mg) {
    if (band >= t->mg->bands.size()) return RT_ERR_INVALID;
    const GroupBand& b = t->mg->group.bands[band];
    out[0] = static_cast<uint32_t>(t->mg->band_device[band]); out[1] = b.row0; out[2] = b.rows; out[3] = static_cast<uint32_t>(b.rank);
    return RT_OK;
  }
  if (band != 0u) return RT_ERR_INVALID;
  out[0] = static_cast<uint32_t>(t->device); out[1] = t->row0; out[2] = t->rows;
  out[3] = t->grp ? static_cast<uint32_t>(t->grp->local[0].rank) : 0u;
  return RT_OK;
}


int rt_dbg_hit_triangle(int device, uint32_t math_mode, uint32_t n, const float* rays, const float* tris,
                        int eps_mode, int32_t* hit, float* tuv, float* normal, float* point) {
  int rc = require_device(device);
  if (rc != RT_OK) return rc;
  return guarded(nullptr, [&] {
    HIP_CHECK(hipSetDevice(device));
    DevBuf dr(n * 6 * sizeof(float)), dt(n * 9 * sizeof(float)), dh(n * sizeof(int)),
        duv(n * 3 * sizeof(float)), dn(n * 3 * sizeof(float)), dp(n * 3 * sizeof(float));
    HIP_CHECK(hipMemcpy(dr.p, rays, n * 6 * sizeof(float), hipMemcpyHostToDevice));
    HIP_CHECK(hipMemcpy(dt.p, tris, n * 9 * sizeof(float), hipMemcpyHostToDevice));
    HIP_CHECK(rtk::launch_dbg_hit_triangle(math_mode != RT_MATH_STRICT, n, dr.as<float>(), dt.as<float>(),
                                           eps_mode, dh.as<int>(), duv.as<float>(), dn.as<float>(),
                                           dp.as<float>(), nullptr));
    HIP_CHECK(hipDeviceSynchronize());
    HIP_CHECK(hipMemcpy(hit, dh.p, n * sizeof(int), hipMemcpyDeviceToHost));
    HIP_CHECK(hipMemcpy(tuv, duv.p, n * 3 * sizeof(float), hipMemcpyDeviceToHost));
    HIP_CHECK(hipMemcpy(normal, dn.p, n * 3 * sizeof(float), hipMemcpyDeviceToHost));
    HIP_CHECK(hipMemcpy(point, dp.p, n * 3 * sizeof(float), hipMemcpyDeviceToHost));
  });
}

int rt_dbg_check_midrange(int device, uint64_t out[4]) {
  if (!out) return RT_ERR_INVALID;
  int rc = require_device(device);
  if (rc != RT_OK) return rc;
  return guarded(nullptr, [&] {
    HIP_CHECK(hipSetDevice(device));
    DevBuf d(4 * sizeof(unsigned long long));
    HIP_CHECK(hipMemset(d.p, 0, 4 * sizeof(unsigned long long)));
    HIP_CHECK(rtk::launch_dbg_check_midrange(d.as<unsigned long long>(), nullptr));
    HIP_CHECK(hipDeviceSynchronize());
    HIP_CHECK(hipMemcpy(out, d.p, 4 * sizeof(uint64_t), hipMemcpyDeviceToHost));
  });
}

int rt_dbg_valu_peak(int device, double* lane_fma_per_s, double* clock_ghz) {
  int rc = require_device(device);
  if (rc != RT_OK) return rc;
  return guarded(nullptr, [&] {
    HIP_CHECK(hipSetDevice(device));
    hipDeviceProp_t prop;
    HIP_CHECK(hipGetDeviceProperties(&prop, device));
    const uint32_t blocks = static_cast<uint32_t>(prop.multiProcessorCount) * 8u;
    const int iters = 20000;
    DevBuf out(static_cast<size_t>(blocks) * 256 * sizeof(float)), clk(2 * sizeof(unsigned long long));
    hipEvent_t e0, e1;
    HIP_CHECK(hipEventCreate(&e0));
    HIP_CHECK(hipEventCreate(&e1));
    HIP_CHECK(rtk::launch_dbg_valu_peak(blocks, iters, out.as<float>(), clk.as<unsigned long long>(), nullptr));
    HIP_CHECK(hipEventRecord(e0, nullptr));
    HIP_CHECK(rtk::launch_dbg_valu_peak(blocks, iters, out.as<float>(), clk.as<unsigned long long>(), nullptr));
    HIP_CHECK(hipEventRecord(e1, nullptr));
    HIP_CHECK(hipEventSynchronize(e1));
    float ms = 0.0f;
    HIP_CHECK(hipEventElapsedTime(&ms, e0, e1));
    unsigned long long c[2];
    HIP_CHECK(hipMemcpy(c, clk.p, sizeof c, hipMemcpyDeviceToHost));
    (void)hipEventDestroy(e0); (void)hipEventDestroy(e1);
    if (lane_fma_per_s) *lane_fma_per_s = static_cast<double>(blocks) * 256.0 * iters * 8.0 / (ms * 1e-3);
    if (clock_ghz) *clock_ghz = c[1] ? static_cast<double>(c[0]) / static_cast<double>(c[1]) * 0.1 : 0.0;
  });
}

#ifdef RT_TIMELINE
extern "C" int rt_dbg_trace_timeline(rt_tracer* t, uint32_t samples, unsigned long long* out, size_t capacity_words) {
  if (!t || !out) return RT_ERR_INVALID;
  std::lock_guard<std::mutex> lk(t->api_mu);
  return guarded(t, [&] {
    t->cancel_and_join();
    t->use_device();
    const size_t words = static_cast<size_t>((t->W + 31u) / 32u) * ((t->rows + 7u) / 8u) * 4u * 16u;
    if (words > capacity_words) throw HipFail{fmt("timeline needs %zu words", words)};
    DevBuf buf(words * sizeof(unsigned long long));
    HIP_CHECK(hipMemsetAsync(buf.p, 0, words * sizeof(unsigned long long), t->main_stream()));
    rtk::TraceParams p = t->params(samples);
    p.flags = rtk::TRACE_ZERO_ACC | rtk::TRACE_EMIT_IMAGE | t->mode_flags(p);
    p.image = t->d_image;
    p.timeline = buf.as<unsigned long long>();
    bool have_lists = false;
    const bool build_lists = t->prepare_tile_lists(p, true, have_lists);
    t->sync_list_stream();
    t->attach_tile_lists(p, have_lists);
    if (have_lists) HIP_CHECK(rtk::launch_tile_lists(p, t->fma, t->main_stream()));
    (void)build_lists;
    t->attach_macro_lists(p, 0, t->main_stream());
    HIP_CHECK(rtk::launch_trace(p, t->fma, t->filter, t->bin, t->pick_k(samples), t->main_stream()));
    HIP_CHECK(hipStreamSynchronize(t->main_stream()));
    HIP_CHECK(hipMemcpy(out, buf.p, words * sizeof(unsigned long long), hipMemcpyDeviceToHost));
  });
}
#endif

int rt_dbg_read_tile_lists(rt_tracer* t, uint32_t* dst, size_t capacity_words, uint32_t* words_per_tile) {
  if (!t || t->mg || !dst) return RT_ERR_INVALID;
  std::lock_guard<std::mutex> lk(t->api_mu);
  return guarded(t, [&] {
    t->cancel_and_join();
    t->use_device();
    HIP_CHECK(hipStreamSynchronize(t->main_stream()));
    t->sync_list_stream();
    if (!t->tile_lists_now() || !t->list_key_valid) throw HipFail{"no tile lists (small scenes build them ahead of their first trace launch)"};
    const size_t n = t->tile_lists_words < capacity_words ? t->tile_lists_words : capacity_words;
    HIP_CHECK(hipMemcpy(dst, t->tile_lists_now(), n * sizeof(uint32_t), hipMemcpyDeviceToHost));
    if (words_per_tile) *words_per_tile = 1u + t->list_key.bin_list;
  });
}

int rt_dbg_wave_list_counts(rt_tracer* t, int half, uint32_t* dst, size_t capacity_tiles, uint32_t* n_tiles, uint32_t* capacity_per_tile) {
  if (!t || t->mg || !dst || half < 0 || half > 1) return RT_ERR_INVALID;
  std::lock_guard<std::mutex> lk(t->api_mu);
  return guarded(t, [&] {
    t->cancel_and_join();
    t->use_device();
    HIP_CHECK(hipStreamSynchronize(t->main_stream()));
    if (!t->d_wave_lists[half] || !t->wave_lists_valid[half]) throw HipFail{"no wave lists (dense scenes build them ahead of their first trace launch)"};
    const rt_tracer::ListKey& k = t->macro_key[half];
    const size_t tiles = static_cast<size_t>((k.W + 31u) / 32u) * ((k.rows + 7u) / 8u) * 4u;
    const uint32_t cap = t->params(1).bin_list;
    const size_t n = tiles < capacity_tiles ? tiles : capacity_tiles;
    HIP_CHECK(hipMemcpy2D(dst, sizeof(uint32_t), t->d_wave_lists[half], static_cast<size_t>(1u + cap) * 64u, sizeof(uint32_t), n, hipMemcpyDeviceToHost));
    if (n_tiles) *n_tiles = static_cast<uint32_t>(tiles);
    if (capacity_per_tile) *capacity_per_tile = cap;
  });
}

int rt_dbg_trace_occupancy(int device, int samples_in_flight, uint32_t lds_bytes) {
  if (require_device(device) != RT_OK) return -1;
  if (hipSetDevice(device) != hipSuccess) return -1;
  return rtk::trace_occupancy(samples_in_flight, lds_bytes);
}

int rt_dbg_sincos(int device, uint32_t n, const float* x, float* s, float* c) {
  int rc = require_device(device);
  if (rc != RT_OK) return rc;
  return guarded(nullptr, [&] {
    HIP_CHECK(hipSetDevice(device));
    DevBuf dx(n * sizeof(float)), ds(n * sizeof(float)), dc(n * sizeof(float));
    HIP_CHECK(hipMemcpy(dx.p, x, n * sizeof(float), hipMemcpyHostToDevice));
    HIP_CHECK(rtk::launch_dbg_sincos(n, dx.as<float>(), ds.as<float>(), dc.as<float>(), nullptr));
    HIP_CHECK(hipDeviceSynchronize());
    HIP_CHECK(hipMemcpy(s, ds.p, n * sizeof(float), hipMemcpyDeviceToHost));
    HIP_CHECK(hipMemcpy(c, dc.p, n * sizeof(float), hipMemcpyDeviceToHost));
  });
}

int rt_dbg_uniform(int device, uint32_t n, uint32_t m, uint32_t* states, float* out) {
  int rc = require_device(device);
  if (rc != RT_OK) return rc;
  return guarded(nullptr, [&] {
    HIP_CHECK(hipSetDevice(device));
    DevBuf ds(n * 6 * sizeof(uint32_t)), dout(static_cast<size_t>(n) * m * sizeof(float));
    HIP_CHECK(hipMemcpy(ds.p, states, n * 6 * sizeof(uint32_t), hipMemcpyHostToDevice));
    HIP_CHECK(rtk::launch_dbg_uniform(n, m, ds.as<uint32_t>(), dout.as<float>(), nullptr));
    HIP_CHECK(hipDeviceSynchronize());
    HIP_CHECK(hipMemcpy(states, ds.p, n * 6 * sizeof(uint32_t), hipMemcpyDeviceToHost));
    HIP_CHECK(hipMemcpy(out, dout.p, static_cast<size_t>(n) * m * sizeof(float), hipMemcpyDeviceToHost));
  });
}

int rt_dbg_get_ray(rt_tracer* t, uint32_t n, const uint32_t* pixels, uint32_t* states, float* rays) {
  if (!t) return RT_ERR_INVALID;
  if (t->mg) { multi_push_camera(t); return rt_dbg_get_ray(t->mg->bands[0], n, pixels, states, rays); }
  return guarded(t, [&] {
    t->use_device();
    rtk::TraceParams p = t->params(1);
    DevBuf dpix(n * 2 * sizeof(uint32_t)), ds(n * 6 * sizeof(uint32_t)), dr(n * 6 * sizeof(float));
    HIP_CHECK(hipMemcpy(dpix.p, pixels, n * 2 * sizeof(uint32_t), hipMemcpyHostToDevice));
    HIP_CHECK(hipMemcpy(ds.p, states, n * 6 * sizeof(uint32_t), hipMemcpyHostToDevice));
    HIP_CHECK(rtk::launch_dbg_get_ray(t->fma, p, n, dpix.as<uint32_t>(), ds.as<uint32_t>(), dr.as<float>(),
                                      t->main_stream()));
    HIP_CHECK(hipStreamSynchronize(t->main_stream()));
    HIP_CHECK(hipMemcpy(states, ds.p, n * 6 * sizeof(uint32_t), hipMemcpyDeviceToHost));
    HIP_CHECK(hipMemcpy(rays, dr.p, n * 6 * sizeof(float), hipMemcpyDeviceToHost));
  });
}

int rt_dbg_focal_boxes(rt_tracer* t, float curv_scale, float* boxes, size_t boxes_capacity, float* focal, size_t focal_capacity) {
  if (!t || t->mg || !boxes || !focal) return RT_ERR_INVALID;
  std::lock_guard<std::mutex> lk(t->api_mu);
  return guarded(t, [&] {
    t->cancel_and_join();
    t->use_device();
    rtk::TraceParams p = t->params(1);
    if (p.tile_curv > 0.0f) p.tile_curv = std::max(p.tile_curv * curv_scale, 1e-30f);
    const size_t tiles = static_cast<size_t>((t->W + 31u) / 32u) * ((t->rows + 7u) / 8u) * 4u;
    const size_t nb = tiles * 8u, nf = static_cast<size_t>(t->npix()) * 3u;
    if (nb > boxes_capacity || nf > focal_capacity) throw HipFail{fmt("focal boxes need %zu + %zu floats", nb, nf)};
    DevBuf db(nb * sizeof(float)), df(nf * sizeof(float));
    HIP_CHECK(hipMemsetAsync(db.p, 0, nb * sizeof(float), t->main_stream()));
    HIP_CHECK(rtk::launch_dbg_focal_boxes(t->fma, p, db.as<float>(), df.as<float>(), t->main_stream()));
    HIP_CHECK(hipStreamSynchronize(t->main_stream()));
    HIP_CHECK(hipMemcpy(boxes, db.p, nb * sizeof(float), hipMemcpyDeviceToHost));
    HIP_CHECK(hipMemcpy(focal, df.p, nf * sizeof(float), hipMemcpyDeviceToHost));
  });
}

int rt_dbg_classify(rt_tracer* t, uint32_t level, uint32_t forms, uint32_t slack_milli, const uint32_t* regions, uint32_t n_regions,
                    float* out, size_t capacity_floats) {
  if (!t || t->mg || !regions || !out || level > 4u) return RT_ERR_INVALID;
  std::lock_guard<std::mutex> lk(t->api_mu);
  return guarded(t, [&] {
    t->cancel_and_join();
    t->use_device();
    rtk::TraceParams p = t->params(1);
    p.macro_w = rt_tracer::kMacroW; p.macro_h = rt_tracer::kMacroH;
    p.super_f = rt_tracer::kSuperF;
    const uint32_t rw = level == 0u ? 8u : level == 2u ? p.macro_w : level == 4u ? p.macro_w * p.super_f : 32u;
    const uint32_t rh = level == 2u ? p.macro_h : level == 4u ? p.macro_h * p.super_f : level == 3u ? 16u : 8u;
    for (uint32_t i = 0; i < n_regions; ++i)
      if (regions[2u * i] % rw != 0u || regions[2u * i + 1u] % rh != 0u || regions[2u * i] >= t->W || regions[2u * i + 1u] >= t->rows)
        throw HipFail{fmt("region %u (%u, %u) is not a level-%u region of the %ux%u band", i, regions[2u * i], regions[2u * i + 1u], level, t->W, t->rows)};
    const size_t per = 16u + static_cast<size_t>(t->n_tris) * (forms ? 32u : 12u);
    if (per * n_regions > capacity_floats) throw HipFail{fmt("rt_dbg_classify needs %zu floats", per * n_regions)};
    DevBuf dr(static_cast<size_t>(n_regions) * 2u * sizeof(uint32_t)), dout(per * n_regions * sizeof(float));
    HIP_CHECK(hipMemcpyAsync(dr.p, regions, static_cast<size_t>(n_regions) * 2u * sizeof(uint32_t), hipMemcpyHostToDevice, t->main_stream()));
    HIP_CHECK(rtk::launch_dbg_classify(t->fma, forms != 0u, slack_milli, p, level, n_regions, dr.as<uint32_t>(), dout.as<float>(), t->main_stream()));
    HIP_CHECK(hipStreamSynchronize(t->main_stream()));
    HIP_CHECK(hipMemcpy(out, dout.p, per * n_regions * sizeof(float), hipMemcpyDeviceToHost));
  });
}

void rt_dbg_rng_init_host(uint64_t seed, uint64_t subsequence, uint32_t state[6]) {
  rth::init_state(jump_host(), seed, subsequence & 0xffffffffull, state);
}

}
```

Before: 582,600.

## Replace list-ready event wait with tagged per-word polling handoff in trace kernel

Tile-list words are now tagged with a per-build generation tag and written with relaxed agent-scope atomics. The trace kernel polls the tags for its own tile and only proceeds once they match, with a timeout that falls back to testing all triangles. This lets the host skip the stream wait on the list-build event in steady state, so list building on the side stream overlaps with tracing. In exchange every list read becomes an atomic load plus a tag mask, tiles may spin-wait, and a tile that times out does brute-force work. Debug counters and an API for the hand-off statistics are added.

```diff
diff --git a/include/rt_mi355x.h b/include/rt_mi355x.h
--- a/include/rt_mi355x.h
+++ b/include/rt_mi355x.h
@@ -135,6 +135,7 @@
 int rt_dbg_check_midrange(int device, uint64_t out[4]);
 int rt_dbg_wave_list_counts(rt_tracer* t, int half, uint32_t* dst, size_t capacity_tiles, uint32_t* n_tiles, uint32_t* capacity_per_tile);
 int rt_dbg_read_tile_lists(rt_tracer* t, uint32_t* dst, size_t capacity_words, uint32_t* words_per_tile);
+int rt_dbg_list_handoff_counts(rt_tracer* t, uint32_t counts[2], int reset);
 int rt_dbg_focal_boxes(rt_tracer* t, float curv_scale, float* boxes, size_t boxes_capacity, float* focal, size_t focal_capacity);
 int rt_dbg_classify(rt_tracer* t, uint32_t level, uint32_t forms, uint32_t slack_milli, const uint32_t* regions, uint32_t n_regions,
                     float* out, size_t capacity_floats);
diff --git a/raytracertest_amd/api.py b/raytracertest_amd/api.py
--- a/raytracertest_amd/api.py
+++ b/raytracertest_amd/api.py
@@ -35,7 +35,7 @@
     "rt_dbg_rng_init_host",
     "rt_tracer_create_multi", "rt_group_unique_id", "rt_tracer_join_group", "rt_tracer_leave_group",
     "rt_tracer_gather_time", "rt_tracer_band_count", "rt_tracer_band_info",
-    "rt_tracer_join_group_bands", "rt_balance_rows", "rt_tracer_rebalance", "rt_tracer_set_band", "rt_dbg_read_tile_lists", "rt_dbg_wave_list_counts", "rt_dbg_focal_boxes", "rt_dbg_classify",
+    "rt_tracer_join_group_bands", "rt_balance_rows", "rt_tracer_rebalance", "rt_tracer_set_band", "rt_dbg_read_tile_lists", "rt_dbg_list_handoff_counts", "rt_dbg_wave_list_counts", "rt_dbg_focal_boxes", "rt_dbg_classify",
     "rt_tracer_gather_only", "rt_tracer_group_info",
 ]
 
@@ -168,6 +168,7 @@
         L.rt_tracer_rebalance.argtypes = [vp]
         L.rt_tracer_set_band.argtypes = [vp, C.c_uint32, C.c_uint32]
         L.rt_dbg_read_tile_lists.argtypes = [vp, u32p, C.c_size_t, u32p]
+        L.rt_dbg_list_handoff_counts.argtypes = [vp, u32p, C.c_int]
         L.rt_dbg_wave_list_counts.argtypes = [vp, C.c_int, u32p, C.c_size_t, u32p, u32p]
         L.rt_dbg_focal_boxes.argtypes = [vp, C.c_float, f32p, C.c_size_t, f32p, C.c_size_t]
         L.rt_tracer_gather_only.argtypes = [vp]
@@ -436,6 +437,11 @@
         words = buf[:bx * by * 4 * w].reshape(by, bx * 4, w)[:, :, 0]
         return (words & 0x3FF).astype(np.int32), ((words >> 10) & 0x3FF).astype(np.int32), (words >> 31).astype(bool)
 
+    def DebugListHandoff(self, reset=False):
+        out = np.zeros(2, np.uint32)
+        self._check(self._lib.rt_dbg_list_handoff_counts(self._h, _u32p(out), int(reset)))
+        return int(out[0]), int(out[1])
+
     def DebugWaveListCounts(self, half=0):
         n, cap = np.zeros(1, np.uint32), np.zeros(1, np.uint32)
         buf = np.zeros(((self.width + 31) // 32) * ((self.rows + 7) // 8 + 1) * 4, np.uint32)
diff --git a/raytracertest_amd/csrc/rt_kernels.hpp b/raytracertest_amd/csrc/rt_kernels.hpp
--- a/raytracertest_amd/csrc/rt_kernels.hpp
+++ b/raytracertest_amd/csrc/rt_kernels.hpp
@@ -4,6 +4,7 @@
 
 namespace rtk {
 
+constexpr uint32_t kListTagShift = 20u, kListTags = 2047u, kListTagMask = 0x7FFu << kListTagShift, kListTagNever = 0x800u;
 constexpr uint32_t kSuperChunk = 1024u, kSuperMaxChunks = 64u;
 
 struct TraceParams {
@@ -41,6 +42,8 @@
   uint32_t  super_chunks, super_f, super_nx;
   float*    macro_bounds;
   uint32_t* tile_lists;
+  uint32_t  list_tag, list_poll_ticks;
+  uint32_t* list_counters;
   uint32_t  row_il, row_phase;
   uint32_t* half_cost;
   uint32_t  cost_split_brow;
diff --git a/raytracertest_amd/csrc/rt_lists.hpp b/raytracertest_amd/csrc/rt_lists.hpp
--- a/raytracertest_amd/csrc/rt_lists.hpp
+++ b/raytracertest_amd/csrc/rt_lists.hpp
@@ -156,6 +156,9 @@
   }, n, out, p.macro_cap, s_cnt);
 }
 
+__device__ __forceinline__ void store_list_word(uint32_t* w, uint32_t v) {
+  __hip_atomic_store((__attribute__((address_space(1))) uint32_t*)w, v, __ATOMIC_RELAXED, __HIP_MEMORY_SCOPE_AGENT);
+}
 template <int CTRL>
 __device__ __forceinline__ float dpp_f(float v) {
   return __builtin_bit_cast(float, __builtin_amdgcn_update_dpp(0, __builtin_bit_cast(int, v), CTRL, 0xF, 0xF, true));
@@ -257,6 +260,7 @@
 
   uint32_t* const saved = p.tile_lists + static_cast<size_t>(sl) * (1u + p.bin_list);
   const uint32_t n = p.n_tris;
+  const uint32_t tag = p.list_tag << kListTagShift;
   uint32_t count = 0;
   const float NEG = -__builtin_inff();
   bool haveA = false;
@@ -279,7 +283,7 @@
     const unsigned long long m = __builtin_amdgcn_ballot_w64(keep);
     const unsigned long long gm = G == 64 ? m : ((m >> gbase) & 0xFFFFFFFFull);
     const uint32_t pos = count + static_cast<uint32_t>(__builtin_popcountll(gm & ((1ull << gl) - 1ull)));
-    if (keep) saved[1u + pos] = tri;
+    if (keep) store_list_word(saved + 1u + pos, tri | tag);
     count += static_cast<uint32_t>(__builtin_popcountll(gm));
     const bool cand = keep && sure && fam.usable;
     const float Qs = group_max<G>(cand ? q[0] : NEG);
@@ -308,7 +312,7 @@
     const float R = (I1 == A) ? M2 : M1;
     sure_one = count <= 1u || (R < Q - 1e-4f * (__builtin_fabsf(R) + __builtin_fabsf(Q)));
   }
-  if (live && gl == 0u) saved[0] = count | (A << 10) | (sure_one ? 0x80000000u : 0u);
+  if (live && gl == 0u) store_list_word(saved, count | (A << 10) | tag | (sure_one ? 0x80000000u : 0u));
 }
 
 template <class SL>
@@ -380,6 +384,7 @@
   const bool tile_valid = mine.any;
   const TileFamily fam = make_family<SL>(p, mine);
   uint32_t* const saved = p.tile_lists + static_cast<size_t>(tile_valid ? tslot : 0u) * (1u + p.bin_list);
+  const uint32_t tag = p.list_tag << kListTagShift;
   const float NEG = -__builtin_inff();
   uint32_t count = 0;
   bool haveA = false;
@@ -402,7 +407,7 @@
     }
     const uint32_t gm = static_cast<uint32_t>(__builtin_amdgcn_ballot_w64(keep) >> gsh) & GM;
     const uint32_t pos = count + static_cast<uint32_t>(__builtin_popcount(gm & ((1u << j) - 1u)));
-    if (keep) saved[1u + pos] = tri;
+    if (keep) store_list_word(saved + 1u + pos, tri | tag);
     count += static_cast<uint32_t>(__builtin_popcount(gm));
     const bool cd = keep && sure && fam.usable;
     const float Qs = max_group<G2>(cd ? q[0] : NEG);
@@ -439,8 +444,8 @@
     if (one_pass) sure_one = sure_one || others_ok;
   }
   if (j == 0u) {
-    if (tile_valid) saved[0] = count | (A << 10) | (sure_one ? 0x80000000u : 0u);
-    else if (slot_live) p.tile_lists[static_cast<size_t>(tslot) * (1u + p.bin_list)] = 0u;
+    if (tile_valid) store_list_word(saved, count | (A << 10) | tag | (sure_one ? 0x80000000u : 0u));
+    else if (slot_live) store_list_word(p.tile_lists + static_cast<size_t>(tslot) * (1u + p.bin_list), tag);
   }
   if (p.half_cost != nullptr) {
     const bool rays = j == 0u && tile_valid && !sure_one;
diff --git a/raytracertest_amd/csrc/rt_trace.hpp b/raytracertest_amd/csrc/rt_trace.hpp
--- a/raytracertest_amd/csrc/rt_trace.hpp
+++ b/raytracertest_amd/csrc/rt_trace.hpp
@@ -101,6 +101,37 @@
       }
     }
   }
+}
+
+
+using gu32 = __attribute__((address_space(1))) uint32_t;
+__device__ __forceinline__ uint32_t load_list_word(const uint32_t* w) {
+  return __hip_atomic_load((gu32*)w, __ATOMIC_RELAXED, __HIP_MEMORY_SCOPE_AGENT);
+}
+__device__ __forceinline__ bool tile_list_tagged(const TraceParams& p, const uint32_t* words, uint32_t lane, uint32_t& h) {
+  const uint32_t want = p.list_tag << kListTagShift, L = p.bin_list;
+  h = static_cast<uint32_t>(__builtin_amdgcn_readfirstlane(static_cast<int>(load_list_word(words))));
+  const uint32_t ent = lane < L ? load_list_word(words + 1u + lane) : want;
+  const bool h_ok = (h & kListTagMask) == want;
+  const uint32_t cnt = h_ok ? ((h & 0x3FFu) < L ? (h & 0x3FFu) : L) : 0u;
+  bool bad = !h_ok || (lane < cnt && (ent & kListTagMask) != want);
+  for (uint32_t b = 64u; b < cnt; b += 64u)
+    if (b + lane < cnt) bad = bad || (load_list_word(words + 1u + b + lane) & kListTagMask) != want;
+  return __builtin_amdgcn_ballot_w64(bad) == 0ull;
+}
+__device__ __forceinline__ uint32_t fetch_tile_list(const TraceParams& p, const uint32_t* words, uint32_t lane, bool& all) {
+  uint32_t h;
+  all = false;
+  if (tile_list_tagged(p, words, lane, h)) return h;
+  if (lane == 0u && p.list_counters != nullptr) atomicAdd(p.list_counters, 1u);
+  const unsigned long long t0 = __builtin_amdgcn_s_memrealtime();
+  while (__builtin_amdgcn_s_memrealtime() - t0 < p.list_poll_ticks) {
+    __builtin_amdgcn_s_sleep(8);
+    if (tile_list_tagged(p, words, lane, h)) return h;
+  }
+  if (lane == 0u && p.list_counters != nullptr) atomicAdd(p.list_counters + 1, 1u);
+  all = true;
+  return p.n_tris;
 }
 
 
@@ -162,10 +193,11 @@
   const bool sure_ok = BIN && ONEPASS && (p.flags & (TRACE_NEAREST_HIT | TRACE_NO_SURE_HIT)) == 0u && p.n_spheres == 0u && p.tri_n == nullptr;
   bool loaded_sure = false;
   uint32_t list_word = 0u;
+  bool list_all = false;
   if constexpr (BIN && ONEPASS) {
     if (p.tile_lists != nullptr) {
       const size_t slot0 = (static_cast<size_t>(by) * gxb + bx) * 4u + wave;
-      list_word = static_cast<uint32_t>(__builtin_amdgcn_readfirstlane(static_cast<int>(p.tile_lists[slot0 * (1u + p.bin_list)])));
+      list_word = fetch_tile_list(p, p.tile_lists + slot0 * (1u + p.bin_list), lane, list_all);
       loaded_sure = sure_ok && (list_word >> 31) != 0u;
     }
   }
@@ -366,7 +398,7 @@
       for (uint32_t base = 0; base < (sure_hit_tile ? 0u : count); base += 64u) {
         const uint32_t e = base + lane;
         if (e < count) {
-          const uint32_t tri = saved[1u + e];
+          const uint32_t tri = (list_all ? e : load_list_word(saved + 1u + e)) & ~kListTagMask;
           cA[2u * e] = p.tri_a[2u * tri];
           cA[2u * e + 1u] = p.tri_a[2u * tri + 1u];
           cB[e] = p.tri_b[tri];
diff --git a/raytracertest_amd/csrc/rt_tracer.hip b/raytracertest_amd/csrc/rt_tracer.hip
--- a/raytracertest_amd/csrc/rt_tracer.hip
+++ b/raytracertest_amd/csrc/rt_tracer.hip
@@ -32,6 +32,8 @@
   bool no_sure_table;
   int row_interleave;
   long macro_cap;
+  bool list_wait;
+  bool list_fallback;
   static bool on(const char* name) { const char* e = getenv(name); return e && e[0] == '1'; }
   Env() {
     log = getenv("RT_MI355X_LOG") != nullptr;
@@ -42,6 +44,8 @@
     row_interleave = (ri && (ri[0] == '0' || ri[0] == '1') && ri[1] == 0) ? ri[0] - '0' : -1;
     const char* mc = getenv("RT_MI355X_MACRO_CAP");
     macro_cap = mc ? strtol(mc, nullptr, 10) : 0;
+    list_wait = on("RT_MI355X_LIST_WAIT");
+    list_fallback = on("RT_MI355X_LIST_FALLBACK");
   }
 };
 inline Env read_env() { return Env(); }
@@ -398,6 +402,8 @@
     p.tri_a = d_tri; p.tri_b = d_tri_b; p.tri_color = d_tri_color; p.n_tris = n_tris;
     p.tri_n = smooth_normals ? d_tri_n : nullptr;
     p.stats = nullptr;
+    p.list_tag = 0u; p.list_counters = d_list_counters;
+    p.list_poll_ticks = env.list_fallback ? 0u : kListPollTicks;
     p.spheres = d_spheres; p.n_spheres = n_spheres;
     p.chunk = chunk_req ? chunk_req : 1024u;
     if (p.chunk > 4096u) p.chunk = 4096u;
@@ -446,6 +452,7 @@
     p.image = d_image;
     bool have_lists = false;
     const bool build_lists = prepare_tile_lists(p, (flags & rtk::TRACE_ZERO_ACC) != 0u, have_lists);
+    const bool lists_wait = (build_lists && lists_from_idle.exchange(false)) || env.list_wait;
     attach_sure_table(p, have_lists);
     last_k = K; last_chunk = p.chunk;
     last_lds = rtk::trace_lds_bytes(p, bin);
@@ -456,9 +463,9 @@
     if (r0 == 0u) {
       (void)main_stream();
       if (build_lists) build_tile_lists_ahead(p);
-      attach_tile_lists(p, have_lists);
+      attach_tile_lists(p, have_lists, true);
       if (timed) HIP_CHECK(hipEventRecord(e.a, stream));
-      if (have_lists) wait_for_lists(stream, list_waited_a);
+      if (have_lists) wait_for_lists(stream, list_waited_a, lists_wait);
       attach_macro_lists(p, 0, stream, (flags & rtk::TRACE_ZERO_ACC) != 0u);
       HIP_CHECK(rtk::launch_trace(p, fma, filter, bin, K, stream));
       if (timed) HIP_CHECK(hipEventRecord(e.b, stream));
@@ -478,8 +485,8 @@
       hipStream_t st[2] = {stream, stream_b};
       if (timed) HIP_CHECK(hipEventRecord(e.a, stream));
       for (int h = 0; h < 2; ++h) {
-        attach_tile_lists(half[h], have_lists);
-        if (have_lists) wait_for_lists(st[h], h == 0 ? list_waited_a : list_waited_b);
+        attach_tile_lists(half[h], have_lists, true);
+        if (have_lists) wait_for_lists(st[h], h == 0 ? list_waited_a : list_waited_b, lists_wait);
         if (h == 1 && stagger) {
           const uint32_t us = static_cast<uint32_t>(last_half_ms.load() * 450.0f);
           if (us >= 5u) HIP_CHECK(rtk::launch_delay(us, stream_b));
@@ -601,6 +608,10 @@
   int list_cur = 0;
   uint64_t list_builds = 0;
   uint64_t list_waited_a = 0, list_waited_b = 0;
+  uint32_t list_tag_cur = rtk::kListTags;
+  std::atomic<bool> lists_from_idle{true};
+  static constexpr uint32_t kListPollTicks = 20000u;
+  uint32_t* d_list_counters = nullptr;
   hipStream_t stream_l = nullptr;
   std::atomic<bool> stagger_next{true};
   hipEvent_t stagger_event = nullptr;
@@ -664,11 +675,12 @@
     return true;
   }
 
-  void attach_tile_lists(rtk::TraceParams& p, bool have) {
+  void attach_tile_lists(rtk::TraceParams& p, bool have, bool trace = false) {
     p.tile_lists = nullptr;
     if (!have) return;
     const size_t slot_base = static_cast<size_t>((W + 31u) / 32u) * ((p.row0 - row0) / 8u) * 4u;
     p.tile_lists = tile_lists_now() + slot_base * (1u + p.bin_list);
+    p.list_tag = (trace && env.list_fallback) ? rtk::kListTagNever : list_tag_cur;
   }
 
   float4* d_sure_table = nullptr;
@@ -711,6 +723,7 @@
       }
     }
     list_cur = r;
+    list_tag_cur = static_cast<uint32_t>(m % rtk::kListTags) + 1u;
     rtk::TraceParams q = p_band;
     attach_tile_lists(q, true);
     const uint32_t sr = split_row(rows);
@@ -720,9 +733,9 @@
     if (q.half_cost != nullptr) HIP_CHECK(rtk::launch_publish_half_cost(d_half_cost, h_half_cost, stream_l));
     ++list_builds;
   }
-  void wait_for_lists(hipStream_t st, uint64_t& waited) {
+  void wait_for_lists(hipStream_t st, uint64_t& waited, bool need) {
     if (waited == list_builds) return;
-    HIP_CHECK(hipStreamWaitEvent(st, list_ready[list_cur], 0));
+    if (need) HIP_CHECK(hipStreamWaitEvent(st, list_ready[list_cur], 0));
     waited = list_builds;
   }
 
@@ -886,6 +899,7 @@
         clear_accumulators();
         if (!stopped) convert();
       }
+      lists_from_idle = true;
       if (stopped) { HIP_CHECK(hipStreamSynchronize(main_stream())); return; }
       if (cleared && i == iterationCount) {
         sync_polling(main_stream());
@@ -1079,6 +1093,8 @@
       HIP_CHECK(hipEventCreateWithFlags(&t->stagger_event, hipEventDisableTiming));
       HIP_CHECK(hipMalloc(&t->d_half_cost, 2 * sizeof(uint32_t)));
       HIP_CHECK(hipMemset(t->d_half_cost, 0, 2 * sizeof(uint32_t)));
+      HIP_CHECK(hipMalloc(&t->d_list_counters, 2 * sizeof(uint32_t)));
+      HIP_CHECK(hipMemset(t->d_list_counters, 0, 2 * sizeof(uint32_t)));
       HIP_CHECK(hipDeviceSynchronize());
       HIP_CHECK(hipHostMalloc(&t->h_half_cost, sizeof(unsigned long long), hipHostMallocDefault));
       *t->h_half_cost = 0ull;
@@ -1142,6 +1158,7 @@
   if (t->stream_l) (void)hipStreamDestroy(t->stream_l);
   if (t->stagger_event) (void)hipEventDestroy(t->stagger_event);
   if (t->d_half_cost) (void)hipFree(t->d_half_cost);
+  if (t->d_list_counters) (void)hipFree(t->d_list_counters);
   if (t->h_half_cost) (void)hipHostFree(t->h_half_cost);
   for (int h = 0; h < 2; ++h) if (t->d_macro_lists[h]) (void)hipFree(t->d_macro_lists[h]);
   for (int h = 0; h < 2; ++h) if (t->d_super_lists[h]) (void)hipFree(t->d_super_lists[h]);
@@ -1474,6 +1491,7 @@
     HIP_CHECK(hipStreamSynchronize(t->main_stream()));
     t->sync_list_stream();
     t->stagger_next = true;
+    t->lists_from_idle = true;
     t->drain_events_before(seen);
     if (t->grp) t->grp->sync();
   });
@@ -1804,7 +1822,20 @@
     if (!t->tile_lists_now() || !t->list_key_valid) throw HipFail{"no tile lists (small scenes build them ahead of their first trace launch)"};
     const size_t n = t->tile_lists_words < capacity_words ? t->tile_lists_words : capacity_words;
     HIP_CHECK(hipMemcpy(dst, t->tile_lists_now(), n * sizeof(uint32_t), hipMemcpyDeviceToHost));
+    for (size_t i = 0; i < n; ++i) dst[i] &= ~rtk::kListTagMask;
     if (words_per_tile) *words_per_tile = 1u + t->list_key.bin_list;
+  });
+}
+
+int rt_dbg_list_handoff_counts(rt_tracer* t, uint32_t counts[2], int reset) {
+  if (!t || t->mg || !counts) return RT_ERR_INVALID;
+  std::lock_guard<std::mutex> lk(t->api_mu);
+  return guarded(t, [&] {
+    t->cancel_and_join();
+    t->use_device();
+    HIP_CHECK(hipStreamSynchronize(t->main_stream()));
+    HIP_CHECK(hipMemcpy(counts, t->d_list_counters, 2 * sizeof(uint32_t), hipMemcpyDeviceToHost));
+    if (reset) HIP_CHECK(hipMemset(t->d_list_counters, 0, 2 * sizeof(uint32_t)));
   });
 }
 
```

New measurement: 563,900 (median of 6 runs). -3.2%, worse.
